# fogleman/sdf

Hardware: AMD Instinct MI355X
Metric: grid voxels/sec (sampled + meshed), canonical CSG example (higher is better)
Workload: dtype f64; 1 GPU; example @ samples=2**27 -> 512x512x512 grid, sparse=True, batch_size=32; batches=4096, skipped=2352, empty=120, nonempty=1624, triangles=2945152, parallelism=single GPU

## Files before the change

include/sdf_hip.h:

```cpp
#ifndef SDF_HIP_H
#define SDF_HIP_H

#include <stddef.h>
#include <stdint.h>

#ifdef __cplusplus
extern "C" {
#endif

#define SDF_ABI_VERSION 15

#define SDF_PRECISION_F64 0
#define SDF_PRECISION_F32 1

typedef struct sdf_ctx sdf_ctx;
typedef struct sdf_tape sdf_tape;
typedef struct sdf_mesh sdf_mesh;

typedef struct sdf_stats {
    int64_t n_batches;
    int64_t n_skipped;
    int64_t n_empty;
    int64_t n_nonempty;
    int64_t n_triangles;
    int64_t n_grid_voxels;
    int64_t n_eval_voxels;
    int64_t n_ambiguous_cells;
    int64_t n_work_begin;
    int64_t n_work_end;
    int64_t n_retries;
    double ms_prepass;
    double ms_mesh;
    double ms_emit;
    double ms_total;
    int64_t n_pruned_instrs;
    int64_t n_batch_instrs;
    int64_t n_sampled_voxels;
    double ms_mesh_device;
    double sclk_mhz;
    double t_mesh_first_us;
    double t_mesh_last_us;
    int64_t mesh_kernel;
} sdf_stats;

int sdf_abi_version(void);
const char *sdf_build_info(void);
const char *sdf_last_error(void);
int sdf_device_count(void);

int sdf_device_mem_info(int device, size_t *free_bytes, size_t *total_bytes);
int sdf_test_fail_alloc(int nth);

int sdf_ctx_create(int device, sdf_ctx **out);
int sdf_ctx_destroy(sdf_ctx *ctx);
int sdf_ctx_set_stream(sdf_ctx *ctx, void *hip_stream);
int sdf_ctx_set_prune(sdf_ctx *ctx, int enabled);
int sdf_ctx_set_cull(sdf_ctx *ctx, int enabled);
int sdf_ctx_set_twopass(sdf_ctx *ctx, int mode);
int sdf_ctx_set_defer(sdf_ctx *ctx, int on);
int sdf_ctx_set_cull_levels(sdf_ctx *ctx, int levels);
int sdf_ctx_set_tail_order(sdf_ctx *ctx, int on);
int sdf_ctx_synchronize(sdf_ctx *ctx);
int sdf_ctx_trim(sdf_ctx *ctx);

int sdf_tape_create(sdf_ctx *ctx, const uint32_t *code, uint32_t n_words, const double *consts,
                    uint32_t n_consts, uint32_t n_pslots, uint32_t n_dslots, sdf_tape **out);
int sdf_tape_set_prune_info(sdf_tape *tape, const uint16_t *rstart, const uint16_t *lstart, uint32_t n_instr);
int sdf_tape_destroy(sdf_tape *tape);

int sdf_eval_points(sdf_tape *tape, const void *d_points, int64_t n, int dim, void *d_out, int precision);
int sdf_eval_points_host(sdf_tape *tape, const double *h_points, int64_t n, int dim, double *h_out,
                         int precision);
int sdf_eval_grid_host(sdf_tape *tape, const double *X, int nx, const double *Y, int ny, const double *Z,
                       int nz, double *h_out, int precision);

int sdf_tape_extern_count(sdf_tape *tape);
int sdf_eval_extern_points_host(sdf_tape *tape, const double *h_points, int64_t n, int dim, double *h_ext_points,
                                int precision);
int sdf_eval_points_extern_host(sdf_tape *tape, const double *h_points, int64_t n, int dim, const double *h_ext_values,
                                double *h_out, int precision);
int sdf_mesh_level_set_host(sdf_ctx *ctx, const double *h_points, int64_t n_points, const int32_t *h_tris, int64_t n_tris,
                            double voxel_size, int half_width_voxels, int64_t out_ijk0[3], int64_t out_dims[3], float *h_out,
                            int64_t cap_voxels);
int sdf_distance_texture_host(sdf_ctx *ctx, const uint8_t *h_mask, int64_t rows, int64_t cols, double *h_out);
int sdf_render_host(sdf_tape *tape, const double *frame18, int width, int height, const double *params5, int max_steps, int refine,
                    double *h_depth, double *h_normal, int32_t *h_steps, uint8_t *h_status);
double sdf_render_last_kernel_ms(void);

typedef int (*sdf_field_fn)(void *user, const double *points, int64_t n, double *values);
int sdf_generate_field(sdf_ctx *ctx, sdf_field_fn field, void *user, const double *X, int nx, const double *Y, int ny,
                       const double *Z, int nz, int batch_size, int sparse, int64_t shard_index, int64_t shard_count,
                       sdf_mesh **out);

int sdf_estimate_bounds(sdf_tape *tape, double *h_out6, int precision);

int sdf_marching_cubes(sdf_ctx *ctx, const void *d_volume, int n0, int n1, int n2, void *d_out_tris,
                       int64_t cap_tris, int64_t *n_tris);
int sdf_marching_cubes_host(sdf_ctx *ctx, const float *h_volume, int n0, int n1, int n2, float *h_out_tris,
                            int64_t cap_tris, int64_t *n_tris);

int sdf_generate(sdf_tape *tape, const double *X, int nx, const double *Y, int ny, const double *Z, int nz,
                 int batch_size, int sparse, int64_t shard_index, int64_t shard_count, int precision,
                 sdf_mesh **out);
int sdf_generate_to_device(sdf_tape *tape, const double *X, int nx, const double *Y, int ny, const double *Z, int nz,
                           int batch_size, int sparse, int64_t shard_index, int64_t shard_count, int precision,
                           void *d_out, int64_t cap_tris, int *emitted, sdf_mesh **out);
int sdf_generate_to_device_async(sdf_tape *tape, const double *X, int nx, const double *Y, int ny, const double *Z, int nz,
                                 int batch_size, int sparse, int64_t shard_index, int64_t shard_count, int precision,
                                 void *d_out, int64_t cap_tris, sdf_mesh **out);
int sdf_mesh_wait(sdf_mesh *mesh, int *emitted);
int sdf_generate_records(sdf_tape *tape, const double *X, int nx, const double *Y, int ny, const double *Z, int nz,
                         int batch_size, int sparse, int precision, sdf_mesh **out);
size_t sdf_slab_bytes(int64_t cap_items, int64_t cap_tris);
int sdf_generate_compact_async(sdf_tape *tape, const double *X, int nx, const double *Y, int ny, const double *Z, int nz,
                               int batch_size, int sparse, int64_t shard_index, int64_t shard_count, int precision,
                               void *d_slab, int64_t cap_items, int64_t cap_tris, sdf_mesh **out);
int sdf_expand_slabs(sdf_ctx *ctx, const void *const *d_slabs, int n_slabs, int64_t cap_items, int64_t cap_tris,
                     void *d_out, int64_t cap_out_tris);
#define SDF_COMM_ID_BYTES 128
typedef struct sdf_comm sdf_comm;
typedef struct sdf_exchange sdf_exchange;
typedef struct sdf_exchange_stats {
    int64_t n_batches, n_skipped, n_empty, n_nonempty, n_triangles, n_grid_voxels, n_eval_voxels, n_ambiguous_cells,
        n_sampled_voxels, n_pruned_instrs;
    int64_t n_retries, chunks, world, slab_bytes;
    double ms_mesh, ms_exchange, ms_expand, ms_total;
    int64_t per_rank_triangles[64];
} sdf_exchange_stats;
int sdf_comm_available(void);
int sdf_comm_unique_id(void *out_id128);
int sdf_comm_create(sdf_ctx *ctx, const void *ids, int n_lanes, int rank, int world, sdf_comm **out);
int sdf_comm_destroy(sdf_comm *comm);
int sdf_generate_sharded_async(sdf_comm *comm, sdf_tape *tape, const double *X, int nx, const double *Y, int ny, const double *Z,
                               int nz, int batch_size, int sparse, int precision, int chunks, int lane, sdf_exchange **out);
int sdf_exchange_wait(sdf_exchange *x, void **d_soup, int64_t *n_tris);
int sdf_exchange_stats_get(sdf_exchange *x, sdf_exchange_stats *out);
int sdf_exchange_destroy(sdf_exchange *x);
int sdf_skip_kinds(sdf_tape *tape, const double *X, int nx, const double *Y, int ny, const double *Z, int nz, int batch_size,
                   int64_t b_begin, int64_t b_end, int precision, void *d_kinds);
int sdf_generate_from_kinds(sdf_tape *tape, const double *X, int nx, const double *Y, int ny, const double *Z, int nz,
                            int batch_size, int64_t shard_index, int64_t shard_count, int precision, const void *d_kinds,
                            sdf_mesh **out);
int sdf_memcpy_to_host(sdf_ctx *ctx, void *h_dst, const void *d_src, size_t bytes);
// ... 37 lines not shown
```

sdf_amd/csrc/sdf_device.h:

```cpp
#pragma once
#include <hip/hip_runtime.h>
#include <stdint.h>
#include <type_traits>

#include "sdf_interp.h"
#include "sdf_mc33.h"
#include "sdf_interval.h"
#include "sdf_slab.h"

namespace sdfk {

struct McTables {
    unsigned char ntri[256];
    unsigned char amb[256];
    signed char tri[256][16];
    signed char mc33[MC33_FLAT_SIZE];
};

struct MeshCounters {
    unsigned long long n_pruned;
    unsigned long long n_eval;
    unsigned int work_counter;
    unsigned int overflow;
    unsigned int n_empty, n_nonempty;
// ... 258 lines not shown
                                                           unsigned max_spins, unsigned long long first) {
    const int lane = threadIdx.x & 63;
    if (w == w_begin) return 0;
    unsigned long long acc = 0;
    int idx = w - 1;
    bool use_first = true;
    for (unsigned spins = 0; spins < max_spins;) {
        constexpr int NW = 4;
        unsigned long long sw[NW];
        const int nwin = use_first ? 1 : NW;
        if (use_first) sw[0] = first;
        else {
#pragma unroll
            for (int k = 0; k < NW; k++) {
                const int j = idx - 64 * k - lane;
                sw[k] = j >= w_begin ? __hip_atomic_load(&status[j], __ATOMIC_RELAXED, __HIP_MEMORY_SCOPE_AGENT)
                                     : MESH_FLAG_PFX;
            }
        }
        use_first = false;
        bool wait = false;
#pragma unroll
        for (int k = 0; k < NW; k++) {
            if (k >= nwin || wait) break;
            const unsigned flag = (unsigned)(sw[k] >> 62);
            const unsigned long long pending = __ballot(flag == 0), is_pfx = __ballot(flag == 2);
            if (is_pfx) {
                const int p = __ffsll((long long)is_pfx) - 1;
                if (pending & ((1ull << p) - 1ull)) { wait = true; break; }
                acc += lane <= p ? (sw[k] & MESH_VAL_MASK) : 0ull;
                const unsigned long long excl = wave_sum_u64(acc);
                if (lane == 0) __hip_atomic_store(&status[w], MESH_FLAG_PFX | (excl + total), __ATOMIC_RELAXED, __HIP_MEMORY_SCOPE_AGENT);
                return excl;
            }
            if (pending) { wait = true; break; }
            acc += sw[k] & MESH_VAL_MASK;
            idx -= 64;
        }
        if (wait) { __builtin_amdgcn_s_sleep(1); spins++; }
    }
    return max_spins < (1u << 24) ? MESH_NOT_READY : ~0ull;
}
#define MESH_SPIN_FOREVER (1u << 24)

__device__ __noinline__ void mc33_triangle(const float *corner, int s0, int s1, int i0, int i1, int i2,
                                           const signed char *tab, int j, float *o) {
    double lv[8];
    int off;
    mc33_load_cell(corner, s0, s1, lv);
    const int n = mc33_cell(lv, tab, &off);
    if (j >= n) { for (int q = 0; q < 9; q++) o[q] = 0.0f; return; }
    const signed char lew_edge[12] = {8, 5, 9, 4, 10, 7, 11, 6, 0, 1, 3, 2};
    for (int q = 0; q < 3; q++) {
        const int e = tab[off + 3 * j + 2 - q];
        if (e == 12) mc33_centre_vertex(lv, i0, i1, i2, o + 3 * q);
        else mc_vertex(corner, s0, s1, i0, i1, i2, lew_edge[e], o + 3 * q);
    }
}

struct TileTasks {
    int lx, ly, lz, lyz, nvox;
    float inv_lyz, inv_lz;
    bool regular;
    int ntask;
    __device__ __forceinline__ TileTasks(int lx_, int ly_, int lz_) : lx(lx_), ly(ly_), lz(lz_) {
        lyz = ly * lz; nvox = lx * lyz;
        inv_lyz = 1.0f / (float)lyz; inv_lz = 1.0f / (float)lz;
        regular = lx == 33 && ly == 33 && lz == 33;
        ntask = regular ? 563 : (nvox + 63) >> 6;
    }
    __device__ __forceinline__ bool sample(int task, int lane, int &ix, int &iy, int &iz) const {
        if (!regular) {
            const int i = min(task * 64 + lane, nvox - 1);
            ix = fast_div(i, inv_lyz); const int r = i - ix * lyz; iy = fast_div(r, inv_lz); iz = r - iy * lz;
            return task * 64 + lane < nvox;
        }
        if (task < 512) { ix = 4 * (task >> 6) + (lane >> 4); iy = 4 * ((task >> 3) & 7) + ((lane >> 2) & 3); iz = 4 * (task & 7) + (lane & 3); return true; }
        if (task < 530) { const int p = min((task - 512) * 64 + lane, 1088); ix = 32; iy = fast_div(p, 1.0f / 33.0f); iz = p - 33 * iy; return (task - 512) * 64 + lane < 1089; }
        if (task < 547) { const int p = min((task - 530) * 64 + lane, 1055); iy = 32; ix = fast_div(p, 1.0f / 33.0f); iz = p - 33 * ix; return (task - 530) * 64 + lane < 1056; }
        const int p = (task - 547) * 64 + lane; iz = 32; ix = p >> 5; iy = p & 31; return true;
    }
};

enum { CULL_UNIT_CAP = 3072, CULL_ULIST = 8, CULL_SBYTES = CULL_ULIST, CULL_SSTATE = CULL_ULIST + 2 * CULL_UNIT_CAP, CULL_COLINFO = CULL_SSTATE + 1024,
       CULL_RECORD = CULL_COLINFO + 1160,
       CULL_MSTATE = CULL_RECORD, CULL_GSTATE = CULL_MSTATE + 64, CULL_ELIST = CULL_GSTATE + 512, CULL_PACC = CULL_ELIST + 1024,
       CULL_SCRATCH = CULL_PACC + 64 };
static_assert(CULL_RECORD % 8 == 0 && CULL_SSTATE % 8 == 0 && CULL_COLINFO % 8 == 0, "the record is copied in words; its state rows are read as u64");
__device__ __forceinline__ bool cull_sample(const unsigned short *units, int task, int lane, int lx, int ly, int lz, int &ix, int &iy, int &iz) {
    const unsigned u = units[8 * task + (lane >> 3)];
    const int x = (int)((u >> 9) & 62u) + ((lane >> 2) & 1), y = (int)((u >> 4) & 62u) + ((lane >> 1) & 1), z = (int)((u << 1) & 62u) + (lane & 1);
    const bool ok = x < lx && y < ly && z < lz;
    ix = ok ? x : 0; iy = ok ? y : 0; iz = ok ? z : 0;
    return ok;
}
template <int BLOCK, bool FULL, bool RARE>
__device__ __forceinline__ int cull_tasks(const uint32_t *wcode, const double *consts, int n_instr_w, int lx, int ly, int lz,
                                       const double *axes, double *ia_state, int ia_bytes, unsigned char *scratch, int *wave_sums,
                                       int ia_np, int ia_nd, unsigned long long *prof = nullptr, int levels = 3) {
    const int tid = threadIdx.x;
    long long tprev = prof ? clock64() : 0;
    unsigned *pacc = reinterpret_cast<unsigned *>(scratch + CULL_PACC);
    if (prof && tid == 0) for (int k = 0; k < 12; k++) pacc[k] = 0;
#define SDF_CULL_PROF(K) do { if (prof && tid == 0) { const long long tn = clock64(); pacc[(K) - 16] += (unsigned)(tn - tprev); tprev = tn; } } while (0)
    const int c0 = lx - 1, c1 = ly - 1, c2 = lz - 1;
    const int per_pass = min(BLOCK, ia_bytes / ((6 * ia_np + 2 * ia_nd) * 8)) & ~63;
    if (c0 <= 0 || c1 <= 0 || c2 <= 0 || per_pass < 64) return -1;
    unsigned short *ulist = reinterpret_cast<unsigned short *>(scratch + CULL_ULIST);
    unsigned char *sstate = scratch + CULL_SBYTES;
    static_assert(2 * CULL_UNIT_CAP >= 4096, "the byte states lie over the unit list");
    unsigned char *mstate = scratch + CULL_MSTATE;
    unsigned char *gstate = scratch + CULL_GSTATE;
    unsigned short *elist = reinterpret_cast<unsigned short *>(scratch + CULL_ELIST);
    auto box_state = [&](int x0, int x1, int y0, int y1, int z0, int z1) -> unsigned char {
        Ival bx{axes[x0], axes[min(x1, c0)]}, by{axes[33 + y0], axes[33 + min(y1, c1)]}, bz{axes[66 + z0], axes[66 + min(z1, c2)]};
        if (bx.lo > bx.hi) { const double t = bx.lo; bx.lo = bx.hi; bx.hi = t; }
        if (by.lo > by.hi) { const double t = by.lo; by.lo = by.hi; by.hi = t; }
        if (bz.lo > bz.hi) { const double t = bz.lo; bz.lo = bz.hi; bz.hi = t; }
        if (ia::bad(bx) || ia::bad(by) || ia::bad(bz)) { bx = by = bz = ia::top(); }
        const Ival v = ia_run_tape<false, FULL, RARE>(wcode, consts, nullptr, nullptr, n_instr_w, bx, by, bz, true,
                                          IaShared{ia_state, ia_np, per_pass}, ia_nd, nullptr);
        return v.lo > 1e-30 ? 1 : (v.hi < -1e-30 ? 2 : 0);
    };
    int phase = 0, e0 = 0, nev = 0;
    for (;;) {
        if (phase == 1 && e0 >= nev) {
            __syncthreads();
            SDF_CULL_PROF(19);
            int nund = 0;
            for (int g0 = 0; levels >= 3 && g0 < 512; g0 += BLOCK) {
                const int gi = g0 + tid;
                const bool und = gi < 512 && gstate[gi] == 0;
                int n;
                const int pos = nund + block_exclusive_count<BLOCK>(und, wave_sums, n);
                if (und) elist[pos] = (unsigned short)gi;
                nund += n;
            }
            for (int h = tid; h < 4096; h += BLOCK) {
                const int h0 = h >> 8, h1 = (h >> 4) & 15, h2 = h & 15;
                const bool exists = 2 * h0 < c0 && 2 * h1 < c1 && 2 * h2 < c2;
                sstate[h] = exists ? gstate[((h0 >> 1) * 8 + (h1 >> 1)) * 8 + (h2 >> 1)] : 1;
            }
            __syncthreads();
            phase = 2; e0 = 0; nev = 8 * nund;
        }
        if (phase == 2 && e0 >= nev) break;
        const bool run = phase == 0 ? tid < 64 : (tid < per_pass && e0 + (tid & ~63) < nev);
        int target = 0, x0, y0, z0, ext;
        bool live;
        if (phase == 0) {
            const int m0 = tid >> 4, m1 = (tid >> 2) & 3, m2 = tid & 3;
            live = 8 * m0 < c0 && 8 * m1 < c1 && 8 * m2 < c2;
            x0 = live ? 8 * m0 : 0; y0 = live ? 8 * m1 : 0; z0 = live ? 8 * m2 : 0; ext = 8;
        } else if (phase == 1) {
            live = e0 + tid < nev;
            target = run ? (int)elist[min(e0 + tid, nev - 1)] : 0;
            x0 = 4 * (target >> 6); y0 = 4 * ((target >> 3) & 7); z0 = 4 * (target & 7); ext = 4;
        } else {
            const int e = min(e0 + tid, nev - 1);
            const int gq = run ? (int)elist[e >> 3] : 0, ch = e & 7;
            const int h0 = 2 * (gq >> 6) + (ch >> 2), h1 = 2 * ((gq >> 3) & 7) + ((ch >> 1) & 1), h2 = 2 * (gq & 7) + (ch & 1);
            live = e0 + tid < nev && 2 * h0 < c0 && 2 * h1 < c1 && 2 * h2 < c2;
            target = (h0 * 16 + h1) * 16 + h2;
            x0 = live ? 2 * h0 : 0; y0 = live ? 2 * h1 : 0; z0 = live ? 2 * h2 : 0; ext = 2;
        }
        if (run) {
            const unsigned char st = box_state(x0, x0 + ext, y0, y0 + ext, z0, z0 + ext);
            if (phase == 0) mstate[tid & 63] = live ? st : 1;
            else if (live) (phase == 1 ? gstate : sstate)[target] = st;
        }
        if (phase != 0) { if (prof && tid == 0) pacc[7]++; e0 += per_pass; continue; }
        SDF_CULL_PROF(17);
        __syncthreads();
        for (int g0 = 0; g0 < 512; g0 += BLOCK) {
            const int gi = g0 + tid;
            const int a0 = gi >> 6, a1 = (gi >> 3) & 7, a2 = gi & 7;
            const bool exists = gi < 512 && 4 * a0 < c0 && 4 * a1 < c1 && 4 * a2 < c2;
            const unsigned char ms = exists ? mstate[((a0 >> 1) * 4 + (a1 >> 1)) * 4 + (a2 >> 1)] : 1;
            if (gi < 512) gstate[gi] = ms;
            int n;
            const int pos = nev + block_exclusive_count<BLOCK>(ms == 0, wave_sums, n);
            if (ms == 0) elist[pos] = (unsigned short)gi;
            nev += n;
        }
        __syncthreads();
        SDF_CULL_PROF(18);
        if (prof && tid == 0) pacc[6] = (unsigned)nev;
        phase = 1; e0 = 0;
    }
    __syncthreads();
    SDF_CULL_PROF(20);
    unsigned short *ub = reinterpret_cast<unsigned short *>(scratch + CULL_GSTATE);
    for (int r = tid; r < 256; r += BLOCK) {
        const unsigned long long lo8 = *reinterpret_cast<const unsigned long long *>(sstate + 16 * r);
        const unsigned long long hi8 = *reinterpret_cast<const unsigned long long *>(sstate + 16 * r + 8);
        unsigned m = 0, pk = 0;
        SDF_UNROLL for (int k = 0; k < 8; k++) { m |= ((lo8 >> (8 * k)) & 255ull) == 0ull ? 1u << k : 0u; pk |= (unsigned)((lo8 >> (8 * k)) & 3ull) << (2 * k); }
        SDF_UNROLL for (int k = 0; k < 8; k++) { m |= ((hi8 >> (8 * k)) & 255ull) == 0ull ? 256u << k : 0u; pk |= (unsigned)((hi8 >> (8 * k)) & 3ull) << (2 * k + 16); }
        ub[r] = (unsigned short)m;
        reinterpret_cast<unsigned *>(scratch + CULL_SSTATE)[r] = pk;
    }
    __syncthreads();
    const int nu0 = (lx + 1) >> 1, nu1 = (ly + 1) >> 1, nu2 = (lz + 1) >> 1;
    int nlisted = 0;
    unsigned *colinfo = reinterpret_cast<unsigned *>(scratch + CULL_COLINFO);
    for (int q0 = 0; q0 < 17 * 17; q0 += BLOCK) {
        const int q = q0 + tid, u0 = q / 17, u1 = q - 17 * u0;
        unsigned um = 0;
        if (q < 17 * 17 && u0 < nu0 && u1 < nu1) {
            unsigned m = 0;
            for (int d0 = 0; d0 < 2; d0++)
                for (int d1 = 0; d1 < 2; d1++) {
                    const int h0 = u0 - d0, h1 = u1 - d1;
                    if (h0 >= 0 && h0 < 16 && h1 >= 0 && h1 < 16) m |= ub[h0 * 16 + h1];
                }
            um = (m | (m << 1)) & ((1u << nu2) - 1u);
        }
        int n;
        int pos = nlisted + block_exclusive_scan<BLOCK>(__popc(um), wave_sums, n);
        nlisted += n;
        if (q < 17 * 17) colinfo[q] = um | ((unsigned)min(pos, 32767) << 17);
        if (nlisted <= CULL_UNIT_CAP) {
            while (um) {
                const int u2 = __ffs((int)um) - 1;
                um &= um - 1u;
                ulist[pos++] = (unsigned short)((u0 << 10) | (u1 << 5) | u2);
            }
        }
    }
    SDF_CULL_PROF(24);
    if (nlisted > CULL_UNIT_CAP) { __syncthreads(); return -1; }
    if (tid < 8 && nlisted + tid < ((nlisted + 7) & ~7)) ulist[nlisted + tid] = 0xFFFFu;
    if (tid == 0) reinterpret_cast<unsigned short *>(scratch)[0] = (unsigned short)nlisted;
    __syncthreads();
    SDF_CULL_PROF(25);
#undef SDF_CULL_PROF
    return (nlisted + 7) >> 3;
}

#ifndef SDF_SOUP_NT
#define SDF_SOUP_NT 0
#endif
#if SDF_SOUP_NT
#define SDF_SOUP_STORE(PTR, VAL) __builtin_nontemporal_store((VAL), (PTR))
#else
#define SDF_SOUP_STORE(PTR, VAL) (*(PTR) = (VAL))
#endif

enum { MESH_SLOT_HDR = 1232, MESH_SLOT_COLINFO = 64, MESH_STAGE_BYTES = 32 * 9 * 4 };

template <typename T, bool FULL, int NP, int ND, int NS, int BLOCK, bool TWOPASS = false>
__global__ __launch_bounds__(BLOCK) void k_mesh(const uint32_t *__restrict__ code, const T *__restrict__ consts, MeshArgs a_byval) {
    typedef __attribute__((address_space(4))) const MeshArgs KArgs;
    static_assert(sizeof(const uint32_t *) + sizeof(const T *) == 16 && alignof(MeshArgs) <= 16, "MeshArgs sits at byte 16 of the kernel arguments");
    KArgs *ap = (KArgs *)((__attribute__((address_space(4))) const char *)__builtin_amdgcn_kernarg_segment_ptr() + 16);
    (void)a_byval;
#define KA (*ap)
#define SDF_SINK (Tri16Sink{KA.out, KA.raw, KA.raw_cap, &KA.ctr->n_raw})
    typedef Vec<T, NS> V;
    constexpr int RPT = 1024 / BLOCK;
    constexpr int MESH_CELL_CHUNKS = 2;
    extern __shared__ __attribute__((aligned(16))) unsigned char smem[];
    int *wave_sums = reinterpret_cast<int *>(smem);
    int *bcast = wave_sums + 16;
    unsigned char *ntri_lds = smem + MESH_LDS_NTRI;
    double *axes = reinterpret_cast<double *>(smem + MESH_LDS_AXES);
    float *vol = reinterpret_cast<float *>(smem + MESH_LDS_VOL);
    unsigned long long *bits = reinterpret_cast<unsigned long long *>(smem + KA.bits_off);
    unsigned *wlist = reinterpret_cast<unsigned *>(smem + KA.list_off);
    int tid = threadIdx.x;
#define SDF_FRESH() asm volatile("" : "+v"(tid))
    const GridDesc g = a_byval.g;
    unsigned short *tri_lds = reinterpret_cast<unsigned short *>(smem + MESH_LDS_TRI);

    if (tid < 256) ntri_lds[tid] = (unsigned char)(KA.mc->ntri[tid] | (KA.mc->amb[tid] << 7));
    if (!TWOPASS)
        for (int i = tid; i < 256 * 5; i += BLOCK) {
            const int cfg = i / 5, j = i - 5 * cfg;
            const signed char *t3 = &KA.mc->tri[cfg][3 * j];
            tri_lds[i] = (unsigned short)(((unsigned)t3[0] & 15u) | (((unsigned)t3[1] & 15u) << 4) | (((unsigned)t3[2] & 15u) << 8));
        }

    for (int i = tid; i < (int)((KA.list_off - KA.bits_off) >> 3); i += BLOCK) bits[i] = 0ull;
    const int work_begin = KA.ctr->work_begin, work_end = KA.ctr->work_end;
    if (KA.prof && tid == 0) KA.prof[64 + 4 * blockIdx.x] = wall_clock64();
// ... 683 lines not shown
```

sdf_amd/csrc/sdf_hip.hip:

```cpp
#include <hip/hip_runtime.h>

#include <algorithm>
#include <cmath>
#include <cstdio>
#include <cstdlib>
#include <cstring>

#include "mc_table.h"
#include "sdf_prune.h"
#include "sdf_plain.h"
#include "sdf_bounds.h"
#include "sdf_internal.h"

using namespace sdfk;


template <typename T, bool FULL>
__global__ __launch_bounds__(256) void k_eval_points(const uint32_t *__restrict__ code, const T *__restrict__ consts,
                                                     const double *__restrict__ pts, long long n, int dim,
                                                     double *__restrict__ out) {
    const long long i = (long long)blockIdx.x * blockDim.x + threadIdx.x;
    if (i >= n) return;
    const T x = (T)pts[i * dim], y = (T)pts[i * dim + 1], z = dim > 2 ? (T)pts[i * dim + 2] : T(0);
    out[i] = (double)run_tape1<T, FULL>(code, consts, x, y, z);
// ... 22 lines not shown
    const int iz = (int)(i % tl.n2), iy = (int)((i / tl.n2) % tl.n1), ix = (int)(i / ((long long)tl.n2 * tl.n1));
    const int *o = org + 3 * blockIdx.y;
    vol[tl.vol_off + i] = (float)run_tape1<T, FULL>(code, consts, (T)X[o[0] + ix], (T)Y[o[1] + iy], (T)Z[o[2] + iz]);
}

template <typename T, bool FULL>
__global__ __launch_bounds__(256) void k_eval_points_ext(const uint32_t *__restrict__ code, const T *__restrict__ consts,
                                                         const double *__restrict__ pts, long long n, int dim,
                                                         double *__restrict__ ext, int dump, double *__restrict__ out) {
    const long long i = (long long)blockIdx.x * blockDim.x + threadIdx.x;
    if (i >= n) return;
    const T x = (T)pts[i * dim], y = (T)pts[i * dim + 1], z = dim > 2 ? (T)pts[i * dim + 2] : T(0);
    const T v = run_tape1_ext<T, FULL>(code, consts, x, y, z, ExtIO{ext, n, i, dump != 0});
    if (!dump) out[i] = (double)v;
}


enum { SKIP_BATCHES_PER_BLOCK = 7 * (256 / 64) };
template <typename T, bool FULL, bool RARE>
__device__ __forceinline__ void skip_body(const uint32_t *__restrict__ code, const T *__restrict__ consts, GridDesc g,
                                              int nbatches, unsigned char *__restrict__ kinds, const PruneArgs &pa,
                                              const double *__restrict__ c64, const uint16_t *__restrict__ rstart,
                                              const uint16_t *__restrict__ lstart, double *prune_lds, int skip_b0) {
    if ((int)blockIdx.x >= pa.first_block) {
        prune_block<FULL, RARE>(code, c64, rstart, lstart, pa, g, nbatches, (int)blockIdx.x - pa.first_block, prune_lds);
        return;
    }
    const int lane = threadIdx.x & 63, slot = min(lane / 9, 6), l = lane - 9 * slot;
    const int b = skip_b0 + ((int)blockIdx.x * (256 / 64) + (int)(threadIdx.x >> 6)) * 7 + slot;
    const bool live = b < nbatches && l < 9;
    int ox = 0, oy = 0, oz = 0, lx = 1, ly = 1, lz = 1;
    if (b < nbatches) batch_origin(g, b, ox, oy, oz, lx, ly, lz);
    double x0 = 0, x1 = 0, y0 = 0, y1 = 0, z0 = 0, z1 = 0;
    if (b < nbatches) {
        x0 = g.X[ox]; x1 = g.X[ox + lx - 1]; y0 = g.Y[oy]; y1 = g.Y[oy + ly - 1]; z0 = g.Z[oz]; z1 = g.Z[oz + lz - 1];
    }
    const double cx = (x0 + x1) / 2, cy = (y0 + y1) / 2, cz = (z0 + z1) / 2;
    double px = cx, py = cy, pz = cz;
    if (l >= 1) { const int k = l - 1; px = (k & 4) ? x1 : x0; py = (k & 2) ? y1 : y0; pz = (k & 1) ? z1 : z0; }
    T v = T(0);
    if (live) v = run_tape1<T, FULL>(code, consts, (T)px, (T)py, (T)pz);
    const int base = 9 * slot;
    const T vc = __shfl(v, base, 64);
    const T v1 = __shfl(v, base + 1, 64);
    const bool pos = v1 > T(0);
    const bool ok = pos ? (v > T(0)) : (v < T(0));
    const unsigned long long m = __ballot(ok);
    const bool all_same = ((m >> (base + 1)) & 0xFFull) == 0xFFull;
    if (b < nbatches && l == 0) {
        const double r = fabs((double)vc);
        const double d = sqrt(((cx - x0) * (cx - x0) + (cy - y0) * (cy - y0)) + (cz - z0) * (cz - z0));
        const bool skip = !(r <= d) && all_same;
        kinds[b] = skip ? 0 : 255;
    }
}

template <typename T, bool FULL>
__global__ __launch_bounds__(256) void k_skip(const uint32_t *__restrict__ code, const T *__restrict__ consts, GridDesc g,
                                              int nbatches, unsigned char *__restrict__ kinds, PruneArgs pa,
                                              const double *__restrict__ c64, const uint16_t *__restrict__ rstart, const uint16_t *__restrict__ lstart,
                                              int skip_b0) {
    extern __shared__ double prune_lds[];
    skip_body<T, FULL, false>(code, consts, g, nbatches, kinds, pa, c64, rstart, lstart, prune_lds, skip_b0);
}
template <typename T, bool FULL>
__global__ __launch_bounds__(256) void k_skip_rare(const uint32_t *__restrict__ code, const T *__restrict__ consts, GridDesc g,
                                                   int nbatches, unsigned char *__restrict__ kinds, PruneArgs pa,
                                                   const double *__restrict__ c64, const uint16_t *__restrict__ rstart, const uint16_t *__restrict__ lstart,
                                                   int skip_b0) {
    extern __shared__ double prune_lds[];
    skip_body<T, FULL, true>(code, consts, g, nbatches, kinds, pa, c64, rstart, lstart, prune_lds, skip_b0);
}

template <bool FULL, bool RARE>
__global__ __launch_bounds__(PRUNE_BLOCK) void k_prune_list(const uint32_t *__restrict__ code, GridDesc g, int nbatches, PruneArgs pa,
                                                               const double *__restrict__ c64, const uint16_t *__restrict__ rstart,
                                                               const uint16_t *__restrict__ lstart) {
    extern __shared__ double prune_list_lds[];
    if ((long long)blockIdx.x * (PRUNE_BLOCK / 8) >= (long long)(pa.ctr->work_end - pa.ctr->work_begin)) return;
    prune_block<FULL, RARE>(code, c64, rstart, lstart, pa, g, nbatches, (int)blockIdx.x, prune_list_lds);
}

#define CULL_BLOCK 256
template <bool FULL, bool RARE, int CB = CULL_BLOCK>
__device__ __forceinline__ void cull_body(const uint32_t *__restrict__ code, const double *__restrict__ consts, GridDesc g,
                                                     const int *__restrict__ worklist, const MeshCounters *__restrict__ ctr,
                                                     int tape_stride, int n_instr, int ia_np, int ia_nd, int ia_bytes,
                                                     unsigned char *__restrict__ out, unsigned char *cull_smem, unsigned long long *prof,
                                                     int *__restrict__ order, int tail_max, int levels) {
    int *wave_sums = reinterpret_cast<int *>(cull_smem);
    double *axes = reinterpret_cast<double *>(cull_smem + 64);
    unsigned char *scratch = cull_smem + 896;
    double *ia_state = reinterpret_cast<double *>(cull_smem + 896 + CULL_SCRATCH);
    const int tid = threadIdx.x;
    const long long tstart = prof ? clock64() : 0;
    asm volatile("" :: "s"(g.X), "s"(g.Y), "s"(g.Z), "s"(g.nx), "s"(g.ny), "s"(g.nz), "s"(g.nby), "s"(g.nbz), "s"(g.bs));
    const int w = ctr->work_begin + (int)blockIdx.x;
    if (w >= ctr->work_end) return;
    long long t_ctr = 0, t_b = 0;
    if (prof) asm volatile("s_memtime %0\n\ts_waitcnt lgkmcnt(0)" : "=s"(t_ctr) : "s"(w) : "memory");
    const int b = __builtin_amdgcn_readfirstlane(worklist[w]);
    if (prof) asm volatile("s_memtime %0\n\ts_waitcnt lgkmcnt(0)" : "=s"(t_b) : "s"(b) : "memory");
    int ox, oy, oz, lx, ly, lz;
    batch_origin(g, b, ox, oy, oz, lx, ly, lz);
    long long t_org = 0;
    if (prof) asm volatile("s_memtime %0\n\ts_waitcnt lgkmcnt(0)" : "=s"(t_org) : "s"(ox), "s"(oy), "s"(oz), "s"(lx) : "memory");
    for (int i = tid; i < 99; i += CB) {
        const int ax = i < 33 ? 0 : (i < 66 ? 1 : 2), k = i - 33 * ax;
        const double *src = ax == 0 ? g.X + ox : (ax == 1 ? g.Y + oy : g.Z + oz);
        if (k < (ax == 0 ? lx : (ax == 1 ? ly : lz))) axes[i] = src[k];
    }
    long long t_ax = 0, t_bar = 0;
    if (prof) asm volatile("s_waitcnt vmcnt(0) lgkmcnt(0)\n\ts_memtime %0\n\ts_waitcnt lgkmcnt(0)" : "=s"(t_ax) : "s"(b) : "memory");
    __syncthreads();
    if (prof) asm volatile("s_memtime %0\n\ts_waitcnt lgkmcnt(0)" : "=s"(t_bar) : "s"(b) : "memory");
    const uint32_t *wcode = code + (size_t)b * (size_t)tape_stride * 2;
    const int n_instr_w = tape_stride ? (int)reinterpret_cast<const unsigned long long *>(wcode)[tape_stride - 1] : n_instr;
    long long tstart1 = 0;
    if (prof) asm volatile("s_waitcnt vmcnt(0) lgkmcnt(0)\n\ts_memtime %0\n\ts_waitcnt lgkmcnt(0)" : "=s"(tstart1) : "s"(n_instr_w) : "memory");
    const int ntl = cull_tasks<CB, FULL, RARE>(wcode, consts, n_instr_w, lx, ly, lz, axes, ia_state, ia_bytes, scratch, wave_sums, ia_np, ia_nd, prof, levels);
    const long long tw = prof ? clock64() : 0;
    if (tid == 0 && ntl < 0) reinterpret_cast<unsigned short *>(scratch)[0] = (unsigned short)0xFFFF;
    __syncthreads();
    {
        unsigned *rec = reinterpret_cast<unsigned *>(out + (size_t)w * CULL_RECORD);
        const unsigned *src = reinterpret_cast<const unsigned *>(scratch);
        const int nwords = ntl < 0 ? 1 : (CULL_ULIST + 16 * ntl + 3) >> 2;
        for (int i = tid; i < nwords; i += CB) rec[i] = src[i];
        if (ntl >= 0) for (int i = tid; i < (CULL_RECORD - CULL_SSTATE) / 4; i += CB) rec[CULL_SSTATE / 4 + i] = src[CULL_SSTATE / 4 + i];
    }
    if (order && tid == 0) {
        const int tail = min(tail_max, ctr->work_end - ctr->work_begin), tpos = w - (ctr->work_end - tail);
        if (tpos >= 0) order[tpos] = (ntl < 0 ? 563 : ntl) * max(n_instr_w, 1);
    }
    if (prof && tid == 0) {
        const unsigned *pacc = reinterpret_cast<const unsigned *>(scratch + CULL_PACC);
        atomicAdd(&prof[32 + (ntl < 0 ? 9 : min(ntl >> 6, 8))], 1ull);
        atomicAdd(&prof[16], (unsigned long long)(tstart1 - tstart));
        atomicAdd(&prof[26], (unsigned long long)(t_ctr - tstart));
        atomicAdd(&prof[27], (unsigned long long)(t_b - t_ctr));
        atomicAdd(&prof[28], (unsigned long long)(t_ax - t_org));
        atomicAdd(&prof[30], (unsigned long long)(t_org - t_b));
        atomicAdd(&prof[29], (unsigned long long)(t_bar - t_ax));
        atomicAdd(&prof[21], (unsigned long long)(clock64() - tw));
        for (int k = 1; k < 10; k++) if (k != 5) atomicAdd(&prof[16 + k], (unsigned long long)pacc[k]);
    }
}

template <bool FULL, bool RARE, int CB = CULL_BLOCK>
__global__ __launch_bounds__(CB) void k_cull(const uint32_t *__restrict__ code, const double *__restrict__ consts, GridDesc g,
                                                     const int *__restrict__ worklist, const MeshCounters *__restrict__ ctr,
                                                     int tape_stride, int n_instr, int ia_np, int ia_nd, int ia_bytes,
                                                     unsigned char *__restrict__ out, unsigned long long *prof,
                                                     int *__restrict__ order, int tail_max, int levels) {
    extern __shared__ __attribute__((aligned(16))) unsigned char cull_smem[];
    cull_body<FULL, RARE, CB>(code, consts, g, worklist, ctr, tape_stride, n_instr, ia_np, ia_nd, ia_bytes, out, cull_smem, prof, order, tail_max, levels);
}
__global__ __launch_bounds__(CULL_BLOCK) __attribute__((amdgpu_waves_per_eu(6, 8))) void k_cull_lean(const uint32_t *__restrict__ code, const double *__restrict__ consts, GridDesc g,
                                                     const int *__restrict__ worklist, const MeshCounters *__restrict__ ctr,
                                                     int tape_stride, int n_instr, int ia_np, int ia_nd, int ia_bytes,
                                                     unsigned char *__restrict__ out, unsigned long long *prof,
                                                     int *__restrict__ order, int tail_max, int levels) {
    extern __shared__ __attribute__((aligned(16))) unsigned char cull_smem[];
    cull_body<false, false>(code, consts, g, worklist, ctr, tape_stride, n_instr, ia_np, ia_nd, ia_bytes, out, cull_smem, prof, order, tail_max, levels);
}
__global__ __launch_bounds__(128) __attribute__((amdgpu_waves_per_eu(6, 8))) void k_cull_lean128(const uint32_t *__restrict__ code, const double *__restrict__ consts, GridDesc g,
                                                     const int *__restrict__ worklist, const MeshCounters *__restrict__ ctr,
                                                     int tape_stride, int n_instr, int ia_np, int ia_nd, int ia_bytes,
                                                     unsigned char *__restrict__ out, unsigned long long *prof,
                                                     int *__restrict__ order, int tail_max, int levels) {
    extern __shared__ __attribute__((aligned(16))) unsigned char cull_smem[];
    cull_body<false, false, 128>(code, consts, g, worklist, ctr, tape_stride, n_instr, ia_np, ia_nd, ia_bytes, out, cull_smem, prof, order, tail_max, levels);
}



static bool tape_needs_full(const uint32_t *code, uint32_t n_words, const double *consts) {
    auto trig_ease = [](int id) {
        return id == EASE_in_sine || id == EASE_out_sine || id == EASE_in_out_sine || id == EASE_in_expo ||
               id == EASE_out_expo || id == EASE_in_out_expo || id == EASE_in_elastic || id == EASE_out_elastic ||
               id == EASE_in_out_elastic;
    };
    for (uint32_t i = 0; i + 1 < n_words; i += 2) {
        const uint32_t op = code[i] & 255u;
        const double *c = consts + (code[i + 1] & 0xFFFFFFu) + 1;
        switch (op) {
        case OP_TWIST: case OP_BEND: case OP_BEND_RADIAL: case OP_WRAP_AROUND: case OP_CIRC_PREP: case OP_CIRC_SET:
        case OP_TRANS_RAD_PRE:
            return true;
        case OP_BEND_LINEAR: if (trig_ease((int)c[10])) return true; break;
        case OP_TRANS_LIN_PRE: if (trig_ease((int)c[7])) return true; break;
        case OP_EXTTO_PRE: if (trig_ease((int)c[1])) return true; break;
        default: break;
        }
    }
    return false;
}

static int validate_tape(const uint32_t *code, uint32_t n_words, uint32_t n_consts, uint32_t n_p, uint32_t n_d) {
    if (n_words < 2 || (n_words & 1)) return fail("tape: code must be a non-empty list of 2-word instructions");
    if (n_p > SDF_NP_SLOTS || n_d > SDF_ND_SLOTS) return fail("tape: model needs more register slots than this build provides");
    if ((code[n_words - 2] & 255u) != OP_END) return fail("tape: missing END");
    for (uint32_t i = 0; i < n_words; i += 2) {
        const uint32_t w0 = code[i], w1 = code[i + 1], op = w0 & 255u, post = (w0 >> 8) & 7u, sa = w0 >> 24, sb = w1 >> 24;
        if (op >= OP_COUNT) return fail("tape: unknown opcode");
        if (post > POST_BLEND) return fail("tape: unknown post-combine");
        if (w0 & 0x800000u) return fail("tape: reserved bit set");
        if ((w0 & 0x000800u) && ((w0 >> 12) & 7u) >= std::max(n_p, 1u)) return fail("tape: reload slot out of range");
        if ((w0 & 0x008000u) && ((w0 >> 16) & 7u) >= std::max(n_p, 1u)) return fail("tape: save slot out of range");
        if ((w0 & 0x080000u) && ((w0 >> 20) & 7u) >= std::max(n_d, 1u)) return fail("tape: push slot out of range");
        if (sa >= SDF_NP_SLOTS || sb >= SDF_NP_SLOTS) return fail("tape: slot out of range");
        if ((w1 & 0xFFFFFFu) >= n_consts) return fail("tape: constant offset out of range");
        if (op == OP_END && i != n_words - 2) return fail("tape: END before the last instruction");
    }
    return 0;
}

static int ctx_init(sdf_ctx *c);

extern "C" {

int sdf_abi_version(void) { return SDF_ABI_VERSION; }

#ifndef SDF_BUILD_INFO
#define SDF_BUILD_INFO "unknown toolchain (not built by csrc/build.sh)"
#endif
const char *sdf_build_info(void) { return SDF_BUILD_INFO; }

int sdf_device_count(void) {
    int n = 0;
    hipError_t e = hipGetDeviceCount(&n);
    if (e != hipSuccess) { g_err = std::string("hipGetDeviceCount: ") + hipGetErrorString(e); return 0; }
    return n;
}


int sdf_device_mem_info(int device, size_t *free_bytes, size_t *total_bytes) {
    if (!free_bytes || !total_bytes) return fail("sdf_device_mem_info: NULL argument");
    HIPCHK(set_device(device));
    HIPCHK(hipMemGetInfo(free_bytes, total_bytes));
    return 0;
}

int sdf_ctx_create(int device, sdf_ctx **out) {
    if (!out) return fail("sdf_ctx_create: out is NULL");
    int n = 0;
    HIPCHK(hipGetDeviceCount(&n));
    if (device < 0 || device >= n) return fail("sdf_ctx_create: no such device");
    HIPCHK(set_device(device));
    hipDeviceProp_t prop;
    HIPCHK(hipGetDeviceProperties(&prop, device));
    if (std::string(prop.gcnArchName).rfind("gfx950", 0) != 0)
        return fail(std::string("sdf_ctx_create: this library is built for gfx950 only, device is ") + prop.gcnArchName);
    sdf_ctx *c = new sdf_ctx();
    c->device = device;
    c->n_cu = prop.multiProcessorCount;
    c->lds_max = prop.sharedMemPerBlock;
    if (ctx_init(c)) {
        const std::string keep = g_err;
        sdf_ctx_destroy(c);
        g_err = keep;
        return 1;
    }
    *out = c;
    return 0;
}

static int ctx_init(sdf_ctx *c) {
    HIPCHK(hipStreamCreateWithFlags(&c->own_stream, hipStreamNonBlocking));
    c->stream = c->own_stream;
    for (auto &e : c->ev) HIPCHK(hipEventCreate(&e));
    HIPCHK(host_malloc(&c->h_stage, (size_t)SDF_CALL_SLOTS * SDF_STAGE_BYTES + 4096));
    for (auto &cs : c->slots) {
        HIPCHK(hipEventCreate(&cs.e0)); HIPCHK(hipEventCreate(&cs.e2)); HIPCHK(hipEventCreate(&cs.e3)); HIPCHK(hipEventCreate(&cs.e4));
        HIPCHK(hipEventCreateWithFlags(&cs.done, hipEventDisableTiming));
        HIPCHK(hipStreamCreateWithFlags(&cs.stream, hipStreamNonBlocking));
    }
    if (const char *e = getenv("SDF_SLOT_STREAMS")) c->slot_streams = atoi(e);
    if (const char *e = getenv("SDF_CULL_BLOCK")) c->cull_block = atoi(e);
    if (const char *e = getenv("SDF_TAIL_ORDER")) c->tail_order = atoi(e);
    if (const char *e = getenv("SDF_MESH_TWOPASS")) c->twopass = atoi(e);
    McTables t;
    memcpy(t.ntri, MC_NTRI, 256);
    memcpy(t.amb, MC_AMBIGUOUS, 256);
    memcpy(t.tri, MC_TRI, sizeof(t.tri));
    memcpy(t.mc33, MC33_FLAT, sizeof(t.mc33));
    if (c->mc.ensure(sizeof(t))) return 1;
    HIPCHK(hipMemcpy(c->mc.p, &t, sizeof(t), hipMemcpyHostToDevice));
    if (const char *e = getenv("SDF_BOUNDS_TAG0")) c->bounds_tag0 = (unsigned)atoi(e) & 0xFFFFu;
    if (const char *e = getenv("SDF_MESH_SLOTS")) c->mesh_slots = atoi(e);
    if (const char *e = getenv("SDF_PRUNE")) c->prune = atoi(e);
    if (const char *e = getenv("SDF_PARK")) c->parking = atoi(e);
    if (const char *e = getenv("SDF_PRUNE_LIST_MIN")) c->prune_list_min = std::max(atoi(e), 0);
    if (const char *e = getenv("SDF_CULL")) c->cull = atoi(e);
    if (const char *e = getenv("SDF_DEFER")) c->defer = atoi(e) ? 1 : 0;
    if (const char *e = getenv("SDF_CULL_LEVELS")) c->cull_levels = atoi(e);
    if (const char *e = getenv("SDF_PARK_SPINS")) c->park_spins = std::max(atoi(e), 1);
    if (const char *e = getenv("SDF_MESH_PROF")) { if (atoi(e) && c->prof.ensure(512 + 4096 * 32)) return 1; }
    return 0;
}

int sdf_ctx_destroy(sdf_ctx *c) {
    if (!c) return 0;
    (void)hipSetDevice(c->device);
    (void)stream_wait(c->stream);
    for (auto &cs : c->slots) { if (cs.stream) (void)stream_wait(cs.stream); cs.park.release(); }
    for (DevBuf *b : {&c->scratch_in, &c->scratch_out, &c->rows, &c->rows_off, &c->mc, &c->prof, &c->park, &c->ext, &c->field_vals,
                      &c->field_vol, &c->field_tiles, &c->bounds_work})
        b->release();
    for (auto &b : c->arena_pool) b.release();
    for (auto &b : c->counter_pool) b.release();
    g_pool.drop_device(c->device);
    for (auto &e : c->ev) if (e) (void)hipEventDestroy(e);
    for (auto &cs : c->slots) for (hipEvent_t e : {cs.e0, cs.e2, cs.e3, cs.e4, cs.done}) if (e) (void)hipEventDestroy(e);
    for (auto &cs : c->slots) if (cs.stream) (void)hipStreamDestroy(cs.stream);
    if (c->h_stage) (void)hipHostFree(c->h_stage);
    if (c->h_rec) (void)hipHostFree(c->h_rec);
    for (hipEvent_t e : c->rec_ev) if (e) (void)hipEventDestroy(e);
    if (c->own_stream) (void)hipStreamDestroy(c->own_stream);
    delete c;
    return 0;
}

int sdf_ctx_set_stream(sdf_ctx *c, void *s) {
    if (!c) return fail("sdf_ctx_set_stream: ctx is NULL");
    c->stream = s ? (hipStream_t)s : c->own_stream;
    return 0;
}

int sdf_ctx_set_prune(sdf_ctx *c, int enabled) {
    if (!c) return fail("sdf_ctx_set_prune: ctx is NULL");
    c->prune = enabled ? 1 : 0;
    return 0;
}

int sdf_ctx_set_cull(sdf_ctx *c, int enabled) {
    if (!c) return fail("sdf_ctx_set_cull: ctx is NULL");
    c->cull = enabled ? 1 : 0;
    return 0;
}

int sdf_ctx_set_defer(sdf_ctx *c, int on) {
    if (!c) return fail("sdf_ctx_set_defer: ctx is NULL");
    c->defer = on ? 1 : 0;
    return 0;
}
int sdf_ctx_set_cull_levels(sdf_ctx *c, int levels) {
    if (!c) return fail("sdf_ctx_set_cull_levels: ctx is NULL");
    if (levels != 0 && levels != 2 && levels != 3) return fail("sdf_ctx_set_cull_levels: 0 (the library's choice), 2 or 3");
    c->cull_levels = levels;
    return 0;
}

int sdf_ctx_set_tail_order(sdf_ctx *c, int on) {
    if (!c) return fail("sdf_ctx_set_tail_order: ctx is NULL");
    c->tail_order = on ? 1 : 0;
    return 0;
}
int sdf_ctx_set_twopass(sdf_ctx *c, int mode) {
    if (!c) return fail("sdf_ctx_set_twopass: ctx is NULL");
    c->twopass = mode < 0 ? -1 : (mode ? 1 : 0);
    return 0;
}

int sdf_ctx_trim(sdf_ctx *c) {
    if (!c) return fail("sdf_ctx_trim: ctx is NULL");
    HIPCHK(set_device(c->device));
    HIPCHK(stream_wait(c->stream));
    for (auto &cs : c->slots) if (cs.stream) HIPCHK(stream_wait(cs.stream));
    for (auto &b : c->arena_pool) b.release();
    c->arena_pool.clear();
    g_pool.drop_device(c->device);
    return 0;
}

int sdf_ctx_synchronize(sdf_ctx *c) {
    if (!c) return fail("sdf_ctx_synchronize: ctx is NULL");
    HIPCHK(set_device(c->device));
    HIPCHK(stream_wait(c->stream));
    for (auto &cs : c->slots) if (cs.stream) HIPCHK(stream_wait(cs.stream));
    return 0;
}

int sdf_tape_create(sdf_ctx *c, const uint32_t *code, uint32_t n_words, const double *consts, uint32_t n_consts,
                    uint32_t n_p, uint32_t n_d, sdf_tape **out) {
    if (!c || !code || !consts || !out) return fail("sdf_tape_create: NULL argument");
    if (validate_tape(code, n_words, n_consts, n_p, n_d)) return 1;
    HIPCHK(set_device(c->device));
    sdf_tape *t = new sdf_tape();
    struct Guard { sdf_tape *t; ~Guard() { if (t) { const std::string keep = g_err; sdf_tape_destroy(t); g_err = keep; } } } guard{t};
    t->ctx = c; t->n_words = n_words; t->n_consts = n_consts;
    t->full = tape_needs_full(code, n_words, consts);
    {
        unsigned long long h = 1469598103934665603ull;
        auto mix = [&](const void *p, size_t n) { const unsigned char *b = (const unsigned char *)p; for (size_t i = 0; i < n; i++) { h ^= b[i]; h *= 1099511628211ull; } };
        mix(code, (size_t)n_words * 4); mix(consts, (size_t)n_consts * 8); mix(&n_p, 4); mix(&n_d, 4);
        t->content_hash = h;
    }
    t->ia_complete = true;
    for (uint32_t i = 0; i < n_words; i += 2) {
        t->ia_complete = t->ia_complete && ia_has_form(code[i] & 255u);
        t->ia_rare = t->ia_rare || ia_is_rare_leaf(code[i] & 255u);
        if ((code[i] & 255u) == OP_L_EXTERN) {
            if ((code[i + 1] & 0xFFFFFFu) + 1 >= n_consts) return fail("tape: closure index out of the constant pool");
            const double k = consts[(code[i + 1] & 0xFFFFFFu) + 1];
            if (!(k >= 0.0 && k < 65536.0 && k == (double)(uint32_t)k)) return fail("tape: bad closure index");
            t->n_extern = std::max(t->n_extern, (uint32_t)k + 1u);
        }
    }
    t->n_p = n_p; t->n_d = n_d;
    std::vector<double> c64(consts, consts + n_consts);
    c64.push_back(0.0); c64.push_back(0.0);
    std::vector<float> c32(c64.size());
    for (size_t i = 0; i < c64.size(); i++) c32[i] = (float)c64[i];
    std::vector<uint32_t> pcode(code, code + n_words);
    pcode.push_back(code[n_words - 2]); pcode.push_back(code[n_words - 1]);
    HIPCHK(dev_malloc((void **)&t->d_code, pcode.size() * sizeof(uint32_t)));
    HIPCHK(dev_malloc((void **)&t->d_c64, c64.size() * sizeof(double)));
    HIPCHK(dev_malloc((void **)&t->d_c32, c32.size() * sizeof(float)));
    HIPCHK(hipMemcpy(t->d_code, pcode.data(), pcode.size() * sizeof(uint32_t), hipMemcpyHostToDevice));
    HIPCHK(hipMemcpy(t->d_c64, c64.data(), c64.size() * sizeof(double), hipMemcpyHostToDevice));
    HIPCHK(hipMemcpy(t->d_c32, c32.data(), c32.size() * sizeof(float), hipMemcpyHostToDevice));
    guard.t = nullptr;
    *out = t;
    return 0;
}

int sdf_tape_set_prune_info(sdf_tape *t, const uint16_t *rstart, const uint16_t *lstart, uint32_t n_instr) {
    if (!t || !rstart || !lstart) return fail("sdf_tape_set_prune_info: NULL argument");
    if (n_instr * 2 != t->n_words) return fail("sdf_tape_set_prune_info: one entry per instruction expected");
    for (uint32_t i = 0; i < n_instr; i++) {
        const bool none = rstart[i] == 0xFFFF || lstart[i] == 0xFFFF;
        if (!none && !(lstart[i] <= rstart[i] && rstart[i] <= i)) return fail("sdf_tape_set_prune_info: operand range out of order");
// ... 338 lines not shown
    return 0;
}

static int stage_axes(const GenCall &call, char *stage, double *dX, hipStream_t st) {
    const double *X = call.X, *Y = call.Y, *Z = call.Z;
    const int nx = call.nx, ny = call.ny, nz = call.nz;
    double *dY = dX + nx, *dZ = dY + ny;
    const size_t axis_bytes = (size_t)(nx + ny + nz) * 8;
    if (call.collected && axis_bytes > SDF_STAGE_BYTES - 256) return fail("sdf_generate_to_device_async: axes too long for the staging slot");
    if (axis_bytes <= SDF_STAGE_BYTES - 256) {
        double *hs = (double *)stage;
        memcpy(hs, X, (size_t)nx * 8); memcpy(hs + nx, Y, (size_t)ny * 8); memcpy(hs + nx + ny, Z, (size_t)nz * 8);
        HIPCHK(hipMemcpyAsync(dX, hs, axis_bytes, hipMemcpyHostToDevice, st));
    } else {
        HIPCHK(hipMemcpyAsync(dX, X, (size_t)nx * 8, hipMemcpyHostToDevice, st));
        HIPCHK(hipMemcpyAsync(dY, Y, (size_t)ny * 8, hipMemcpyHostToDevice, st));
        HIPCHK(hipMemcpyAsync(dZ, Z, (size_t)nz * 8, hipMemcpyHostToDevice, st));
    }
    return 0;
}

static int enqueue_prepass(const GenCall &call, sdf_mesh *m, int nb, int tape_stride, hipStream_t st) {
    sdf_tape *t = call.tape;
    sdf_ctx *c = t->ctx;
    const GridDesc &g = m->g;
    const int sparse = call.sparse, precision = call.precision;
    const bool pruning = tape_stride != 0;
    const uint32_t n_instr = t->n_words / 2;
    PruneArgs pa = {};
    pa.first_block = 0x7fffffff;
    const bool prune_listed = pruning && sparse && (nb >= c->prune_list_min || call.shard_count > 1);
    unsigned skip_blocks = (sparse && !call.d_kinds) ? (unsigned)((nb + SKIP_BATCHES_PER_BLOCK - 1) / SKIP_BATCHES_PER_BLOCK) : 0u, prune_blocks = 0;
    size_t prune_lds = 0;
    if (pruning) {
        if (m->prune.ensure((size_t)nb * 64) || m->tapes.ensure((size_t)nb * tape_stride * 8)) return 1;
        pa.n_instr = (int)n_instr; pa.n_p = std::max(t->n_p, 1u); pa.n_d = std::max(t->n_d, 1u);
        pa.masks_out = (uint32_t *)m->prune.p; pa.tapes_out = (unsigned long long *)m->tapes.p; pa.tape_stride = tape_stride;
        pa.zero_off = t->n_consts;
        prune_lds = prune_lds_bytes(pa.n_p, pa.n_d);
        if (!prune_listed) {
            pa.first_block = (int)skip_blocks;
            prune_blocks = (unsigned)(((long long)nb * 8 + PRUNE_BLOCK - 1) / PRUNE_BLOCK);
        }
    }
    if (skip_blocks + prune_blocks) {
        if (prune_lds > 32768 && prune_blocks) {
            const void *fn = t->ia_rare ? (t->full ? reinterpret_cast<const void *>(k_skip_rare<double, true>) : reinterpret_cast<const void *>(k_skip_rare<double, false>))
                                        : (t->full ? reinterpret_cast<const void *>(k_skip<double, true>) : reinterpret_cast<const void *>(k_skip<double, false>));
            HIPCHK(hipFuncSetAttribute(fn, hipFuncAttributeMaxDynamicSharedMemorySize, (int)prune_lds));
        }
        const size_t skip_lds = prune_blocks ? prune_lds : 0;
        if (t->ia_rare) LAUNCH_TAPE_ON(st, k_skip_rare, dim3(skip_blocks + prune_blocks), dim3(256), skip_lds, t, precision, g, nb, (unsigned char *)m->kinds.p, pa,
                                       (const double *)t->d_c64, (const uint16_t *)t->d_rstart, (const uint16_t *)t->d_lstart, 0);
        else LAUNCH_TAPE_ON(st, k_skip, dim3(skip_blocks + prune_blocks), dim3(256), skip_lds, t, precision, g, nb, (unsigned char *)m->kinds.p, pa,
                            (const double *)t->d_c64, (const uint16_t *)t->d_rstart, (const uint16_t *)t->d_lstart, 0);
    }
    if (!sparse) HIPCHK(hipMemsetAsync(m->kinds.p, 255, (size_t)nb, st));
    else if (call.d_kinds) HIPCHK(hipMemcpyAsync(m->kinds.p, call.d_kinds, (size_t)nb, hipMemcpyDeviceToDevice, st));
    launch_k_compact(dim3(1), dim3(1024), st, (const unsigned char *)m->kinds.p, nb, (int *)m->worklist.p,
                       (MeshCounters *)m->counters.p, (unsigned long long *)m->status.p, (long long)call.shard_index,
                       (long long)call.shard_count);
    HIPCHK(hipGetLastError());
    if (prune_listed) {
        pa.worklist = (const int *)m->worklist.p; pa.ctr = (const MeshCounters *)m->counters.p;
        auto kp = t->full ? (t->ia_rare ? k_prune_list<true, true> : k_prune_list<true, false>) : (t->ia_rare ? k_prune_list<false, true> : k_prune_list<false, false>);
        if (prune_lds > 32768) HIPCHK(hipFuncSetAttribute(reinterpret_cast<const void *>(kp), hipFuncAttributeMaxDynamicSharedMemorySize, (int)prune_lds));
        hipLaunchKernelGGL(kp, dim3((unsigned)(((long long)nb * 8 + PRUNE_BLOCK - 1) / PRUNE_BLOCK)), dim3(PRUNE_BLOCK), prune_lds, st,
                           (const uint32_t *)t->d_code, g, nb, pa, (const double *)t->d_c64, (const uint16_t *)t->d_rstart,
                           (const uint16_t *)t->d_lstart);
        HIPCHK(hipGetLastError());
    }
    return 0;
}

static int enqueue_cull(sdf_tape *t, sdf_mesh *m, int nb, int tape_stride, bool tail_order, int tail_max, hipStream_t st) {
    sdf_ctx *c = t->ctx;
    const GridDesc &g = m->g;
    const bool pruning = tape_stride != 0;
    const uint32_t n_instr = t->n_words / 2;
    if (c->prof.p) HIPCHK(hipMemsetAsync((unsigned char *)c->prof.p + 128, 0, 384, st));
    if (m->cull.ensure((size_t)nb * CULL_RECORD) || (tail_order && m->order.ensure(MESH_TAIL_MAX * sizeof(int)))) return 1;
    const int ia_np = (int)std::max(t->n_p, 1u), ia_nd = (int)std::max(t->n_d, 1u);
    auto kc = t->full ? (t->ia_rare ? k_cull<true, true> : k_cull<true, false>) : (t->ia_rare ? k_cull<false, true> : k_cull_lean);
    int cull_block = CULL_BLOCK;
    if (c->cull_block == 128 && kc == k_cull_lean) { kc = k_cull_lean128; cull_block = 128; }
    if (t->full && !t->ia_rare && c->cull_block != 256) {
        cull_block = c->cull_block == 64 ? 64 : 128;
        kc = cull_block == 64 ? k_cull<true, false, 64> : k_cull<true, false, 128>;
    }
    const int cull_levels = c->cull_levels ? c->cull_levels : (kc == k_cull_lean || kc == k_cull_lean128 ? 3 : 2);
    const size_t ia_bytes = std::min<size_t>((size_t)cull_block * (6 * ia_np + 2 * ia_nd) * 8, c->lds_max - 896 - CULL_SCRATCH);
    const size_t lds = 896 + CULL_SCRATCH + ia_bytes;
    if (lds > 32768) HIPCHK(hipFuncSetAttribute(reinterpret_cast<const void *>(kc), hipFuncAttributeMaxDynamicSharedMemorySize, (int)lds));
    hipLaunchKernelGGL(kc, dim3(nb), dim3(cull_block), lds, st,
                       pruning ? (const uint32_t *)m->tapes.p : (const uint32_t *)t->d_code, (const double *)t->d_c64, g,
                       (const int *)m->worklist.p, (const MeshCounters *)m->counters.p, pruning ? tape_stride : 0, (int)n_instr,
                       ia_np, ia_nd, (int)ia_bytes, (unsigned char *)m->cull.p, (unsigned long long *)c->prof.p,
                       tail_order ? (int *)m->order.p : (int *)nullptr, tail_max, cull_levels);
    HIPCHK(hipGetLastError());
    return 0;
}

static int first_soup_cap(sdf_tape *t, sdf_mesh *m, unsigned long long key, hipStream_t st, unsigned long long &cap, bool &quiet) {
    if (t->hint_key == key && t->hint_total_tris) {
        cap = t->hint_total_tris + t->hint_total_tris / 4 + 4096;
        return 0;
    }
    MeshCounters h;
    quiet = false;
    HIPCHK(hipMemcpyAsync(&h, m->counters.p, sizeof(h), hipMemcpyDeviceToHost, st));
    HIPCHK(stream_wait(st));
    const unsigned long long nshard0 = (unsigned long long)std::max(h.work_end - h.work_begin, 1);
    cap = std::max<unsigned long long>(4096ull * nshard0, 1ull << 16);
    size_t free_b = 0, total_b = 0;
    if (hipMemGetInfo(&free_b, &total_b) == hipSuccess)
        cap = std::min<unsigned long long>(cap, std::max<unsigned long long>(free_b / 2 / (72 + 40), 1ull << 16));
    return 0;
}

static int soup_target(const GenCall &call, sdf_mesh *m, int attempt, unsigned long long cap, bool &quiet, MeshArgs &a) {
    sdf_ctx *c = m->ctx;
    a.compact = 0; a.xf = nullptr; a.xf_cap = 0; a.raw = nullptr; a.raw_cap = 0;
    if (cap) {
        if (!m->out.p && !c->arena_pool.empty()) { m->out = c->arena_pool.back(); c->arena_pool.pop_back(); }
        if (m->out.bytes < (size_t)cap * 72) quiet = false;
        if (m->out.ensure((size_t)cap * 72)) {
            bool ok = false;
            for (int k = 0; k < 6 && !ok && attempt == 0 && cap > (1ull << 16); k++) {
                cap = std::max<unsigned long long>(cap / 4, 1ull << 16);
                ok = m->out.ensure((size_t)cap * 72) == 0;
            }
            if (!ok) return 1;
        }
        a.out = (double *)m->out.p; a.out_cap = m->out.bytes / 72;
    } else if (call.dest == GenCall::SLAB) {
        unsigned char *d_slab = (unsigned char *)call.d_out;
        const SlabLayout L(call.cap_items, call.cap_tris);
        a.out = reinterpret_cast<double *>(d_slab + L.tris_off); a.out_cap = (unsigned long long)call.cap_tris;
        a.compact = 1; a.xf = reinterpret_cast<double *>(d_slab + L.xf_off);
        a.raw = reinterpret_cast<float *>(d_slab + L.raw_off); a.raw_cap = L.raw_cap;
        a.xf_cap = (int)std::min<int64_t>(call.cap_items, 0x7fffffff);
    } else {
        a.out = (double *)call.d_out; a.out_cap = (unsigned long long)call.cap_tris;
    }
    return 0;
}

static int mesh_attempt(const GenCall &call, sdf_mesh *m, CallState &s, hipStream_t st, int attempt, unsigned long long soup_cap, bool quiet,
                        bool culling, int tail, int tape_stride) {
    sdf_tape *t = call.tape;
    sdf_ctx *c = t->ctx;
    CallSlot &cs = c->slots[s.slot];
    const int nb = s.nb;
    const uint32_t n_instr = s.n_instr;
    MeshArgs a;
    a.twopass = 0; a.desc = nullptr; a.cells = nullptr; a.tlist = nullptr; a.cells_cap = a.tlist_cap = 0; a.block_item = nullptr;
    a.order = tail ? (const int *)m->order.p : nullptr; a.tail = tail;
    if (soup_target(call, m, attempt, soup_cap, quiet, a)) return 1;
    if (attempt) {
        HIPCHK(hipMemsetAsync(m->counters.p, 0, MESH_COUNTERS_RESET_BYTES, st));
        HIPCHK(hipMemsetAsync(m->status.p, 0, (size_t)nb * 8, st));
    }
    a.g = m->g; a.worklist = (const int *)m->worklist.p;
    a.kinds = (unsigned char *)m->kinds.p; a.status = (unsigned long long *)m->status.p;
    a.ctr = (MeshCounters *)m->counters.p;
    a.mc = (const McTables *)c->mc.p;
    a.prof = (unsigned long long *)c->prof.p;
    const bool twopass = c->twopass >= 0 ? c->twopass != 0 : n_instr > 96;
    DevBuf &park = call.collected ? cs.park : c->park;
    const bool parks = c->parking && !twopass;
    if (parks && !park.p) { quiet = false; if (park.ensure((size_t)c->n_cu * MESH_PARK_DEPTH * SDF_PARK_TRIS * 36)) return 1; }
    a.park = parks ? (float *)park.p : nullptr; a.park_cap = a.park ? SDF_PARK_TRIS : 0;
    a.park_spins = (unsigned)c->park_spins;
    a.cull = culling ? (const unsigned char *)m->cull.p : nullptr;
    a.tape_stride = tape_stride;
    a.n_instr = (int)n_instr;
    if (twopass) {
        const size_t cap_t = (size_t)a.out_cap;
        if (m->desc.bytes < (size_t)nb * sizeof(ItemDesc) || m->cellrecs.bytes < cap_t * 36 || m->trilist.bytes < cap_t * 4) quiet = false;
        if (m->desc.ensure((size_t)nb * sizeof(ItemDesc)) || m->cellrecs.ensure(cap_t * 36) || m->trilist.ensure(cap_t * 4) ||
            m->blockidx.ensure(((cap_t + 255) / 256 + 2) * sizeof(int)))
            return 1;
        a.twopass = 1; a.desc = (ItemDesc *)m->desc.p; a.cells = (unsigned *)m->cellrecs.p; a.tlist = (unsigned *)m->trilist.p;
        a.block_item = (const int *)m->blockidx.p;
        a.cells_cap = a.tlist_cap = (unsigned long long)cap_t;
    }
    if (a.prof) {
        HIPCHK(hipMemsetAsync(a.prof, 0, 128, st));
        HIPCHK(hipMemsetAsync((unsigned char *)a.prof + 512, 0, 4096 * 32, st));
    }
    const int grid = std::min(nb, c->n_cu);
    s.own_start = attempt > 0 || a.prof || !quiet;
    if (s.own_start) HIPCHK(hipEventRecord(cs.e3, st));
    if (launch_mesh(t, tape_stride ? m->tapes.p : (const void *)t->d_code, call.precision, a, grid, call.bs, st)) return 1;
    if (a.twopass) {
        const unsigned long long emit_blocks = (a.out_cap + 255ull) / 256ull;
        if (emit_blocks > 0x7fffffffull) return fail("sdf_generate: soup capacity too large for one k_emit2 launch");
        launch_k_scan_items(dim3(1), dim3(1024), st, (const ItemDesc *)m->desc.p, (MeshCounters *)m->counters.p,
                           (unsigned long long *)m->status.p, (int *)m->blockidx.p, emit_blocks + 1ull);
        launch_k_emit2(dim3((unsigned)std::max<unsigned long long>(emit_blocks, 1ull)), dim3(256), st, a);
        HIPCHK(hipGetLastError());
    }
    HIPCHK(hipEventRecord(cs.e4, st));
    if (call.dest == GenCall::SLAB) {
        const unsigned pack_blocks = (unsigned)std::min<int64_t>(std::max<int64_t>((call.cap_items + 255) / 256, 1), 1024);
        HIPCHK((hipError_t)sdf_launch_pack_slab(pack_blocks, st, (const MeshCounters *)m->counters.p, (const unsigned long long *)m->status.p,
                                                (unsigned char *)call.d_out, (long long)call.cap_items, (long long)call.cap_tris));
    }
    MeshCounters *hp = (MeshCounters *)((char *)c->h_stage + (size_t)s.slot * SDF_STAGE_BYTES + SDF_STAGE_BYTES - 256);
    HIPCHK(hipMemcpyAsync(hp, m->counters.p, sizeof(MeshCounters), hipMemcpyDeviceToHost, st));
    return 0;
}

static int mesh_prof_report(sdf_ctx *c, int grid, float ms) {
    unsigned long long pc[64];
    HIPCHK(hipMemcpy(pc, c->prof.p, 512, hipMemcpyDeviceToHost));
    {
        std::vector<unsigned long long> tl((size_t)4 * grid);
        HIPCHK(hipMemcpy(tl.data(), (unsigned char *)c->prof.p + 512, tl.size() * 8, hipMemcpyDeviceToHost));
        unsigned long long t0 = ~0ull, t_end = 0;
        double s_out = 0, s_done = 0, mn_out = 1e30, mx_out = 0;
        for (int i = 0; i < grid; i++) t0 = std::min(t0, tl[4 * i]);
        for (int i = 0; i < grid; i++) {
            const double o = (double)(tl[4 * i + 1] - t0) * 0.01, d = (double)(tl[4 * i + 2] - t0) * 0.01;
            s_out += o; s_done += d; mn_out = std::min(mn_out, o); mx_out = std::max(mx_out, o); t_end = std::max(t_end, tl[4 * i + 2]);
        }
        double first_hi = 0;
        for (int i = 0; i < grid; i++) first_hi = std::max(first_hi, (double)(tl[4 * i] - t0) * 0.01);
        fprintf(stderr, "[k_mesh prof] %d workgroups (1 per CU), last of them started after %.1f us; out of work after min %.1f avg %.1f max %.1f us; done after avg %.1f, last %.1f us\n",
                grid, first_hi, mn_out, s_out / grid, mx_out, s_done / grid, (double)(t_end - t0) * 0.01);
    }
    fprintf(stderr, "[k_cull prof] work items by listed tasks (of 563; bins of 64, last: not culled): %llu %llu %llu %llu %llu %llu %llu %llu %llu | %llu\n",
            pc[32], pc[33], pc[34], pc[35], pc[36], pc[37], pc[38], pc[39], pc[40], pc[41]);
    fprintf(stderr, "[k_cull prof] cycles of thread 0, summed over the workgroups: start %llu boxes %llu list %llu groups %llu (%llu passes, %llu groups) tasks %llu record %llu\n",
            pc[16], pc[17], pc[18], pc[19], pc[23], pc[22], pc[20], pc[21]);
    fprintf(stderr, "[k_cull prof] task listing: which tasks %llu, scans %llu; start: range %llu batch %llu origin %llu axes %llu barrier %llu (rest: tape length)\n", pc[24], pc[25], pc[26], pc[27], pc[30], pc[28], pc[29]);
    fprintf(stderr, "[k_mesh prof] sampling: intervals %llu task list %llu interpreter %llu sign bits %llu\n", pc[8], pc[9], pc[10], pc[11]);
    fprintf(stderr, "[k_mesh prof] fine: atomic %llu barrier+rank %llu header %llu | rows %llu cells %llu | placing %llu look-back %llu | round end %llu\n",
            pc[42], pc[43], pc[44], pc[45], pc[46], pc[47], pc[48], pc[49]);
    fprintf(stderr, "[k_mesh prof] %.3f ms; cycles/WG-sum: grab %llu sample %llu count %llu (of which placing the parked batch %llu) list %llu emit %llu tail %llu; %llu batches parked, %llu written one batch later from their slot\n",
            ms, pc[0], pc[1], pc[2], pc[6], pc[3], pc[4], pc[5], pc[7], pc[12]);
    return 0;
}

int generate_impl(sdf_mesh *m, const GenCall &call) {
    sdf_tape *t = call.tape;
    sdf_ctx *c = t->ctx;
    const bool slab = call.dest == GenCall::SLAB;
    const int nx = call.nx, ny = call.ny, nz = call.nz;
    CallState s;
    if (take_slot(c, s.slot)) return 1;
    CallSlot &cs = c->slots[s.slot];
    const bool own_lane = call.collected && !slab && c->stream == c->own_stream && c->slot_streams;
    hipStream_t st = call.lane ? call.lane : (own_lane ? cs.stream : c->stream);
    m->stream = (own_lane || call.lane) ? st : nullptr;
    if (grid_batches(nx, ny, nz, call.bs, "sdf_generate", m->g, s.nb)) return 1;
    const int nb = s.nb;
    m->st.n_batches = nb;
    m->st.n_grid_voxels = (int64_t)nx * ny * nz;
    if (nb == 0) {
        if (slab) HIPCHK(hipMemsetAsync(call.d_out, 0, sizeof(SlabHeader), st));
        return 0;
    }

    if (m->axes.ensure((size_t)(nx + ny + nz) * 8) || m->kinds.ensure((size_t)nb) || m->worklist.ensure((size_t)nb * 4) ||
        m->status.ensure((size_t)nb * 8))
        return 1;
    if (!m->counters.p && !c->counter_pool.empty()) { m->counters = c->counter_pool.back(); c->counter_pool.pop_back(); }
    if (m->counters.ensure(sizeof(MeshCounters))) return 1;
    double *dX = (double *)m->axes.p;
    m->g.X = dX; m->g.Y = dX + nx; m->g.Z = dX + nx + ny;
    HIPCHK(hipEventRecord(cs.e0, st));
    if (stage_axes(call, (char *)c->h_stage + (size_t)s.slot * SDF_STAGE_BYTES, dX, st)) return 1;

    auto monotone = [](const double *a, int n) {
        bool up = true, down = true;
        for (int i = 1; i < n; i++) { up &= a[i - 1] <= a[i]; down &= a[i - 1] >= a[i]; }
        return up || down;
    };
    s.n_instr = t->n_words / 2;
    const bool intervals_ok = call.precision == SDF_PRECISION_F64 && monotone(call.X, nx) && monotone(call.Y, ny) && monotone(call.Z, nz);
    s.pruning = c->prune && t->d_rstart && s.n_instr <= 256 && intervals_ok && t->n_consts < 0xFFFFF0u;
    const int tape_stride = s.pruning ? (int)((s.n_instr + 2 + 7) & ~7u) : 0;
    if (enqueue_prepass(call, m, nb, tape_stride, st)) return 1;
    const bool culling = c->cull && intervals_ok && t->ia_complete && mesh_lds(call.bs, c->lds_max).list_off + CULL_RECORD <= c->lds_max;
    const int tail_max = std::min<int>(MESH_TAIL_MAX, std::min(nb, c->n_cu) - 1);
    const bool tail_order = culling && c->tail_order && tail_max >= 2 && !call.collected;
    s.key = grid_key(nx, ny, nz, call.bs, call.sparse, call.shard_index, call.shard_count);
    if (culling && enqueue_cull(t, m, nb, tape_stride, tail_order, tail_max, st)) return 1;
    HIPCHK(hipEventRecord(cs.e2, st));

    unsigned long long soup_cap = 0;
    bool quiet = true;
    if (call.dest == GenCall::SOUP && first_soup_cap(t, m, s.key, st, soup_cap, quiet)) return 1;
    for (int attempt = 0;; attempt++) {
        if (mesh_attempt(call, m, s, st, attempt, soup_cap, quiet, culling, tail_order ? tail_max : 0, tape_stride)) return 1;
        if (call.collected) {
            HIPCHK(hipEventRecord(cs.done, st));
            cs.busy = true; cs.owner = m;
            sdf_mesh::Pending &pd = m->pend;
            pd.active = true; pd.call = call; pd.got = s;
            pd.axes.assign(call.X, call.X + nx); pd.axes.insert(pd.axes.end(), call.Y, call.Y + ny); pd.axes.insert(pd.axes.end(), call.Z, call.Z + nz);
            pd.call.X = pd.axes.data(); pd.call.Y = pd.call.X + nx; pd.call.Z = pd.call.Y + ny;
            return 0;
        }
        HIPCHK(stream_wait(st));
        MeshCounters h;
        const int rc = finish_call(m, call, s, slab, h);
        if (c->prof.p && mesh_prof_report(c, std::min(nb, c->n_cu), m->st.ms_mesh)) return 1;
        m->st.n_retries = attempt;
        if (rc) return 1;
        if (slab) {
            const SlabLayout L(call.cap_items, call.cap_tris);
            const bool raw_over = (long long)h.n_raw > L.raw_cap;
            m->n_raw = (long long)h.n_raw;
            m->rec_overflow = (h.overflow & 1u) != 0 || raw_over || (long long)(h.work_end - h.work_begin) > (long long)call.cap_items;
            m->rec_need_tris = std::max<long long>((long long)h.total, raw_over ? (long long)h.n_raw * SLAB_RAW_DIV : 0ll);
            m->emitted_to = nullptr;
            return 0;
// ... 378 lines not shown
```

sdf_amd/csrc/sdf_internal.h:

```cpp
#pragma once
#include <cstdint>
#include <map>

#include "../../include/sdf_hip.h"
#include "sdf_device.h"
#include "sdf_runtime.h"

using sdfk::DevBuf;
using sdfk::GridDesc;

#define SDF_STAGE_BYTES (1u << 20)
#ifndef SDF_CALL_SLOTS
#define SDF_CALL_SLOTS 8
#endif
struct CallSlot {
    hipEvent_t e0 = nullptr, e2 = nullptr, e3 = nullptr, e4 = nullptr;
    hipEvent_t done = nullptr;
    bool busy = false;
    struct sdf_mesh *owner = nullptr;
    hipStream_t stream = nullptr;
    DevBuf park;
};
#define SDF_BATCH_SIZE_MAX 512
#define SDF_PARK_TRIS 8192

struct sdf_ctx {
    int device = 0;
    hipStream_t own_stream = nullptr, stream = nullptr;
    hipEvent_t ev[8] = {};
    int n_cu = 256;
    size_t lds_max = 0;
    DevBuf scratch_in, scratch_out, rows, rows_off, mc;
    DevBuf ext;
    DevBuf field_vals, field_vol, field_tiles;
    DevBuf prof;
    int prune = 1;
    int parking = 1;
    int cull = 1;
    int prune_list_min = 8192;
    int park_spins = 1;
    DevBuf park;
    int mesh_slots = -1;
    std::vector<DevBuf> arena_pool;
    std::vector<DevBuf> counter_pool;
    void *h_stage = nullptr;
    CallSlot slots[SDF_CALL_SLOTS];
    unsigned slot_seq = 0;
    int slot_streams = 1;
    int cull_block = 0;
    int tail_order = 1;
    int twopass = -1;
    int defer = 1;
    int cull_levels = 0;
    DevBuf bounds_work;
    unsigned bounds_tag = 0, bounds_tag0 = 0;
    struct RecHint { unsigned long long tris = 0, raw = 0; };
    std::map<std::pair<unsigned long long, unsigned long long>, RecHint> rec_hints;
    void *h_rec = nullptr;
    size_t h_rec_bytes = 0;
    std::vector<hipEvent_t> rec_ev;
};

struct sdf_tape {
    sdf_ctx *ctx = nullptr;
    uint32_t *d_code = nullptr;
    double *d_c64 = nullptr;
    float *d_c32 = nullptr;
    uint32_t n_words = 0, n_consts = 0;
    bool full = false;
    uint32_t n_p = 0, n_d = 0;
    uint16_t *d_rstart = nullptr, *d_lstart = nullptr;
    bool ia_complete = false;
    bool ia_rare = false;
    uint32_t n_extern = 0;
    unsigned long long hint_key = 0, hint_total_tris = 0;
    unsigned long long content_hash = 0;
};

struct GenCall {
    sdf_tape *tape = nullptr;
    const double *X = nullptr, *Y = nullptr, *Z = nullptr;
    int nx = 0, ny = 0, nz = 0, bs = 0, sparse = 0, precision = 0;
    int64_t shard_index = 0, shard_count = 1;
    enum Dest { SOUP, CALLER, SLAB } dest = SOUP;
    void *d_out = nullptr;
    int64_t cap_tris = 0, cap_items = 0;
    bool collected = false;
    hipStream_t lane = nullptr;
    const unsigned char *d_kinds = nullptr;
};
struct CallState { int slot = 0, nb = 0; bool pruning = false, own_start = false; uint32_t n_instr = 0; unsigned long long key = 0; };

struct sdf_mesh {
    sdf_ctx *ctx = nullptr;
    sdf_stats st = {};
    GridDesc g = {};
    DevBuf axes, kinds, worklist, status, out, prune, tapes, cull, order;
    DevBuf desc, cellrecs, trilist;
    DevBuf blockidx;
    bool pruned = false;
    hipStream_t stream = nullptr;
    DevBuf counters;
    int work_begin = 0, work_end = 0;
    void *emitted_to = nullptr;
    struct Pending {
        bool active = false;
        GenCall call;
        std::vector<double> axes;
        CallState got;
    } pend;
    double *weld_pts = nullptr;
    long long *weld_inv = nullptr;
    long long weld_n = -1;
    double *nrm = nullptr;
    bool nrm_valid = false;
    unsigned long long nrm_model = 0;
    double nrm_eps = 0.0;
    long long nrm_flat = 0;
    bool records = false;
    DevBuf slab;
    long long slab_items = 0, slab_tris = 0, n_raw = 0;
    bool rec_overflow = false;
    long long rec_need_tris = 0;
};

inline long long grid_desc(int nx, int ny, int nz, int bs, GridDesc &g) {
    g = GridDesc{};
    g.nx = nx; g.ny = ny; g.nz = nz; g.bs = bs;
    if (bs < 1) return 0;
    g.nbx = (nx + bs - 1) / bs; g.nby = (ny + bs - 1) / bs; g.nbz = (nz + bs - 1) / bs;
    return (long long)g.nbx * g.nby * g.nbz;
}

inline GenCall gen_call(sdf_tape *t, const double *X, int nx, const double *Y, int ny, const double *Z, int nz, int bs, int sparse,
                        int64_t shard_index, int64_t shard_count, int precision) {
// ... 16 lines not shown
```

sdf_amd/csrc/sdf_interval.h:

```cpp
#pragma once
#include <hip/hip_runtime.h>
#include <stdint.h>

#include "opcodes.h"

#define SDF_IA __host__ __device__ __forceinline__

namespace sdfk {

#if defined(__HIP_DEVICE_COMPILE__)
__device__ __forceinline__ void ia_sincos(double x, double *s, double *c) { sincos64(x, *s, *c); }
__device__ __forceinline__ double ia_atan2(double y, double x) { return atan2_64(y, x); }
#else
inline void ia_sincos(double x, double *s, double *c) { *s = sin(x); *c = cos(x); }
inline double ia_atan2(double y, double x) { return atan2(y, x); }
#endif

struct Ival {
    double lo, hi;
};

namespace ia {

SDF_IA Ival top() { return Ival{-__builtin_inf(), __builtin_inf()}; }
// ... 100 lines not shown
    d = a = top();
    if (!finite_(x) || !finite_(y) || !(da > 0.0) || !(da < 7.0)) return;
    d = pad(len2(x, y), 1e-12, 1e-300);
    if (bad(d)) { d = top(); return; }
    d.lo = fmax(d.lo, 0.0);
    a = Ival{0.0, da};
    if (x.lo <= 0.0 && y.lo <= 0.0 && y.hi >= 0.0) return;
    const double t0 = ia_atan2(y.lo, x.lo), t1 = ia_atan2(y.lo, x.hi), t2 = ia_atan2(y.hi, x.lo), t3 = ia_atan2(y.hi, x.hi);
    const double tl = fmin(fmin(t0, t1), fmin(t2, t3)) - 1e-12, th = fmax(fmax(t0, t1), fmax(t2, t3)) + 1e-12;
    if (!(tl <= th)) return;
    const double kl = floor(tl / da), kh = floor(th / da);
    if (kl != kh) return;
    const double lo = tl - kl * da, hi = th - kl * da;
    if (!(lo > 1e-9) || !(da - hi > 1e-9)) return;
    a = Ival{lo - 1e-12, hi + 1e-12};
}
SDF_IA Ival atan2_range(const Ival &x, const Ival &y) {
    const double pi = 3.141592653589793;
    if (!finite_(x) || !finite_(y)) return top();
    if (x.lo <= 0.0 && y.lo <= 0.0 && y.hi >= 0.0) return Ival{-pi, pi};
    const double t0 = ia_atan2(y.lo, x.lo), t1 = ia_atan2(y.lo, x.hi), t2 = ia_atan2(y.hi, x.lo), t3 = ia_atan2(y.hi, x.hi);
    const double tl = fmin(fmin(t0, t1), fmin(t2, t3)) - 1e-12, th = fmax(fmax(t0, t1), fmax(t2, t3)) + 1e-12;
    if (!(tl <= th)) return Ival{-pi, pi};
    return Ival{fmax(tl, -pi), fmin(th, pi)};
}
SDF_IA void circ_set(const Ival &d, const Ival &a, double delta, Ival &x, Ival &y) {
    x = y = top();
    if (!finite_(d) || !finite_(a) || delta != delta) return;
    Ival sn, cs;
    sincos_range(subc(a, delta), sn, cs);
    x = mul(cs, d);
    y = mul(sn, d);
}
SDF_IA double ease_value(int id, double t, bool &known) {
    double u, v;
    known = true;
    switch (id) {
    case EASE_linear: return t;
    case EASE_in_quad: return t * t;
    case EASE_out_quad: return -t * (t - 2.0);
    case EASE_in_out_quad: u = 2.0 * t - 1.0; return t < 0.5 ? 2.0 * t * t : -0.5 * (u * (u - 2.0) - 1.0);
    case EASE_in_cubic: return t * t * t;
    case EASE_out_cubic: u = t - 1.0; return u * u * u + 1.0;
    case EASE_in_out_cubic: u = t * 2.0; v = u - 2.0; return u < 1.0 ? 0.5 * u * u * u : 0.5 * (v * v * v + 2.0);
    case EASE_in_quart: return t * t * t * t;
    case EASE_out_quart: u = t - 1.0; return -(u * u * u * u - 1.0);
    case EASE_in_out_quart: u = t * 2.0; v = u - 2.0; return u < 1.0 ? 0.5 * u * u * u * u : -0.5 * (v * v * v * v - 2.0);
    case EASE_in_quint: return t * t * t * t * t;
    case EASE_out_quint: u = t - 1.0; return u * u * u * u * u + 1.0;
    case EASE_in_out_quint: u = t * 2.0; v = u - 2.0; return u < 1.0 ? 0.5 * u * u * u * u * u : 0.5 * (v * v * v * v * v + 2.0);
    case EASE_in_circ: return -1.0 * (sqrt(fmax(1.0 - t * t, 0.0)) - 1.0);
    case EASE_out_circ: u = t - 1.0; return sqrt(fmax(1.0 - u * u, 0.0));
    case EASE_in_out_circ:
        u = t * 2.0; v = u - 2.0;
        return u < 1.0 ? -0.5 * (sqrt(fmax(1.0 - u * u, 0.0)) - 1.0) : 0.5 * (sqrt(fmax(1.0 - v * v, 0.0)) + 1.0);
    case EASE_in_square: return t < 1.0 ? 0.0 : 1.0;
    case EASE_out_square: return t > 0.0 ? 1.0 : 0.0;
    case EASE_in_out_square: return t < 0.5 ? 0.0 : 1.0;
    default: known = false; return 0.0;
    }
}
SDF_IA Ival ease01(int id, const Ival &t) {
    if (bad(t) || t.lo < 0.0 || t.hi > 1.0) return top();
    bool k0, k1;
    const double a = ease_value(id, t.lo, k0), b = ease_value(id, t.hi, k1);
    if (!k0 || !k1 || a != a || b != b) return top();
    return Ival{fmin(a, b) - 1e-12, fmax(a, b) + 1e-12};
}

}

enum { PRUNE_BLOCK = 256 };
struct IaShared {
    double *base;
    int n_p;
    int stride;
#if defined(__HIP_DEVICE_COMPILE__)
    __device__ __forceinline__ static int lane_slot() { return (int)threadIdx.x; }
#elif defined(SDF_HOST_SIMT)
    static int lane_slot() { return sdf_host_simt_tid(); }
#else
    static int lane_slot() { return 0; }
#endif
    SDF_IA double &ps(uint32_t slot, int k) { return base[(slot * 6 + k) * stride + lane_slot()]; }
    SDF_IA double &ds(uint32_t slot, int k) { return base[(n_p * 6 + slot * 2 + k) * stride + lane_slot()]; }
};
__host__ __device__ inline size_t prune_lds_bytes(int n_p, int n_d) { return (size_t)(6 * n_p + 2 * n_d) * PRUNE_BLOCK * 8; }


__host__ __device__ inline bool ia_has_form(uint32_t op) {
    switch (op) {
    case OP_END: case OP_L_SPHERE: case OP_L_PLANE: case OP_L_BOX: case OP_L_ROUNDED_BOX: case OP_L_TORUS: case OP_L_CYLINDER:
    case OP_L_ROUNDED_CYLINDER: case OP_L_CAPSULE: case OP_L_OCTAHEDRON: case OP_L_CIRCLE: case OP_L_LINE: case OP_L_RECTANGLE:
    case OP_L_WIREFRAME_BOX: case OP_L_CAPPED_CYLINDER: case OP_L_ROUNDED_CONE: case OP_L_ELLIPSOID: case OP_L_TETRAHEDRON:
    case OP_L_DODECAHEDRON: case OP_L_ICOSAHEDRON: case OP_L_ROUNDED_RECTANGLE: case OP_L_EQUILATERAL_TRIANGLE: case OP_L_HEXAGON:
    case OP_L_ROUNDED_X: case OP_L_VESICA: case OP_L_CAPPED_CONE: case OP_L_PYRAMID: case OP_L_POLYGON: case OP_L_TEXTURE2D:
    case OP_L_GRID3D:
    case OP_COMB: case OP_TRANSLATE: case OP_SCALE: case OP_ROTATE: case OP_ELONGATE: case OP_TRANSLATE2: case OP_SCALE2:
    case OP_ROTATE2: case OP_ELONGATE2: case OP_REVOLVE: case OP_SETZ0: case OP_SAVE_P: case OP_LOAD_P: case OP_PUSH_D: case OP_NOP:
    case OP_NEG: case OP_ADDC: case OP_SUBC: case OP_MULC: case OP_SHELL: case OP_ADD_DS: case OP_EXT_PRE: case OP_EXT_POST:
    case OP_REP_PREP: case OP_REP_SET: case OP_CIRC_PREP: case OP_CIRC_SET: case OP_BEND_LINEAR:
    case OP_TWIST: case OP_BEND: case OP_BEND_RADIAL: case OP_TRANS_LIN_PRE: case OP_TRANS_RAD_PRE: case OP_TRANS_MIX:
    case OP_EXTTO_PRE: case OP_EXTTO_MIX: case OP_SLICE_POST: case OP_WRAP_AROUND:
        return true;
    default: return false;
    }
}

SDF_IA Ival ia_box_like(const Ival &qx, const Ival &qy, const Ival &qz) {
    using namespace ia;
    const Ival mx = max_(max_(qx, qy), qz);
    return add(len3(maxc(qx, 0.0), maxc(qy, 0.0), maxc(qz, 0.0)), minc(mx, 0.0));
}

SDF_IA Ival ia_leaf(uint32_t op, const double *c, const Ival &x, const Ival &y, const Ival &z) {
    using namespace ia;
    switch (op) {
    case OP_L_SPHERE: return subc(len3(subc(x, c[1]), subc(y, c[2]), subc(z, c[3])), c[0]);
    case OP_L_PLANE: return dot3c(csub(c[3], x), csub(c[4], y), csub(c[5], z), c[0], c[1], c[2]);
    case OP_L_BOX:
        return ia_box_like(subc(abs_(subc(x, c[0])), c[3]), subc(abs_(subc(y, c[1])), c[4]), subc(abs_(subc(z, c[2])), c[5]));
    case OP_L_ROUNDED_BOX:
        return subc(ia_box_like(addc(subc(abs_(x), c[0]), c[3]), addc(subc(abs_(y), c[1]), c[3]), addc(subc(abs_(z), c[2]), c[3])), c[3]);
    case OP_L_TORUS: return subc(len2(subc(len2(x, y), c[0]), z), c[1]);
    case OP_L_CYLINDER: return subc(len2(x, y), c[0]);
    case OP_L_ROUNDED_CYLINDER: {
        const Ival d0 = addc(subc(len2(x, y), c[0]), c[1]), d1 = addc(subc(abs_(z), c[2]), c[1]);
        return subc(add(minc(max_(d0, d1), 0.0), len2(maxc(d0, 0.0), maxc(d1, 0.0))), c[1]);
    }
    case OP_L_CAPSULE: {
        const Ival pax = subc(x, c[0]), pay = subc(y, c[1]), paz = subc(z, c[2]);
        const Ival h = clip01(divc(dot3c(pax, pay, paz, c[3], c[4], c[5]), c[6]));
        return subc(len3(sub(pax, mulc(h, c[3])), sub(pay, mulc(h, c[4])), sub(paz, mulc(h, c[5]))), c[7]);
    }
    case OP_L_OCTAHEDRON: return mulc(subc(add(add(abs_(x), abs_(y)), abs_(z)), c[0]), c[1]);
    case OP_L_CIRCLE: return subc(len2(subc(x, c[1]), subc(y, c[2])), c[0]);
    case OP_L_LINE: return dot2c(csub(c[2], x), csub(c[3], y), c[0], c[1]);
    case OP_L_RECTANGLE: {
        const Ival qx = subc(abs_(subc(x, c[0])), c[2]), qy = subc(abs_(subc(y, c[1])), c[3]);
        return add(len2(maxc(qx, 0.0), maxc(qy, 0.0)), minc(max_(qx, qy), 0.0));
    }
    default: return top();

    }
}

SDF_IA bool ia_is_rare_leaf(uint32_t op) {
    switch (op) {
    case OP_L_WIREFRAME_BOX: case OP_L_CAPPED_CYLINDER: case OP_L_ROUNDED_CONE: case OP_L_ELLIPSOID: case OP_L_TETRAHEDRON:
    case OP_L_DODECAHEDRON: case OP_L_ICOSAHEDRON: case OP_L_ROUNDED_RECTANGLE: case OP_L_EQUILATERAL_TRIANGLE: case OP_L_HEXAGON:
    case OP_L_ROUNDED_X: case OP_L_VESICA: case OP_L_CAPPED_CONE: case OP_L_PYRAMID: case OP_L_POLYGON: case OP_L_TEXTURE2D:
    case OP_L_GRID3D:
        return true;
    default: return false;
    }
}
__host__ __device__ __attribute__((noinline)) inline Ival ia_leaf_rare(uint32_t op, const double *c, const Ival &x, const Ival &y, const Ival &z) {
    using namespace ia;
    switch (op) {
    case OP_L_WIREFRAME_BOX: {
        const double t2 = c[3];
        const Ival px = subc(subc(abs_(x), c[0]), t2), py = subc(subc(abs_(y), c[1]), t2), pz = subc(subc(abs_(z), c[2]), t2);
        const Ival qx = subc(abs_(addc(px, t2)), t2), qy = subc(abs_(addc(py, t2)), t2), qz = subc(abs_(addc(pz, t2)), t2);
        const Ival g0 = add(len3(maxc(px, 0.0), maxc(qy, 0.0), maxc(qz, 0.0)), minc(max_(px, max_(qy, qz)), 0.0));
        const Ival g1 = add(len3(maxc(qx, 0.0), maxc(py, 0.0), maxc(qz, 0.0)), minc(max_(qx, max_(py, qz)), 0.0));
        const Ival g2 = add(len3(maxc(qx, 0.0), maxc(qy, 0.0), maxc(pz, 0.0)), minc(max_(qx, max_(qy, pz)), 0.0));
        return min_(min_(g0, g1), g2);
    }
    case OP_L_CAPPED_CYLINDER: {
        const double bax = c[3], bay = c[4], baz = c[5], baba = c[6];
        if (!(baba > 0.0)) return top();
        const Ival pax = subc(x, c[0]), pay = subc(y, c[1]), paz = subc(z, c[2]);
        const Ival paba = dot3c(pax, pay, paz, bax, bay, baz);
        const Ival xx = subc(len3(sub(mulc(pax, baba), mulc(paba, bax)), sub(mulc(pay, baba), mulc(paba, bay)),
                                  sub(mulc(paz, baba), mulc(paba, baz))), c[8]);
        const Ival yy = subc(abs_(subc(paba, c[9])), c[9]);
        const Ival x2 = sqr(xx), y2 = mulc(sqr(yy), baba);
        const Ival zero = pt(0.0);
        const Ival din = neg(min_(x2, y2));
        const Ival dout = add(sel_gt(xx, zero, x2, zero), sel_gt(yy, zero, y2, zero));
        const Ival d = sel_gt(zero, max_(xx, yy), din, dout);
        if (bad(d)) return top();
        const double lo = (d.lo > 0.0 ? 1.0 : (d.lo < 0.0 ? -1.0 : 0.0)) * sqrt(fabs(d.lo)) / baba;
        const double hi = (d.hi > 0.0 ? 1.0 : (d.hi < 0.0 ? -1.0 : 0.0)) * sqrt(fabs(d.hi)) / baba;
        return wide(lo, hi);
    }
    case OP_L_ROUNDED_CONE: {
        const double r1 = c[0], r2 = c[1], h = c[2], b = c[3], a = c[4], ah = c[5];
        const Ival qx = len2(x, y), qy = z;
        const Ival k = dot2c(qx, qy, -b, a);
        const Ival c1 = subc(len2(qx, qy), r1), c2 = subc(len2(qx, subc(qy, h)), r2), c3 = subc(dot2c(qx, qy, a, b), r1);
        if (bad(k) || ah != ah) return top();
        Ival r{0.0, 0.0};
        bool any = false;
        if (k.lo < 0.0) { r = c1; any = true; }
        if (k.hi >= 0.0) {
            if (k.hi > ah) { r = any ? hull(r, c2) : c2; any = true; }
            if (fmax(k.lo, 0.0) <= ah) { r = any ? hull(r, c3) : c3; any = true; }
        }
        return any ? fix(r) : top();
    }
    case OP_L_ELLIPSOID: {
        const Ival k0 = len3(divc(x, c[0]), divc(y, c[1]), divc(z, c[2]));
        const Ival k1 = len3(divc(x, c[3]), divc(y, c[4]), divc(z, c[5]));
        return div_pos(mul(k0, subc(k0, 1.0)), k1);
    }
    case OP_L_TETRAHEDRON:
        return divc(subc(max_(sub(abs_(add(x, y)), z), add(abs_(sub(x, y)), z)), c[0]), c[1]);
    case OP_L_DODECAHEDRON: case OP_L_ICOSAHEDRON: {
        const double r = c[0], X = c[1], Y = c[2], Z = c[3];
        const Ival ax = abs_(divc(x, r)), ay = abs_(divc(y, r)), az = abs_(divc(z, r));
        const Ival a = dot3c(ax, ay, az, X, Y, Z), b = dot3c(ax, ay, az, Z, X, Y), cc = dot3c(ax, ay, az, Y, Z, X);
        const Ival m = subc(max_(max_(a, b), cc), X);
        if (op == OP_L_DODECAHEDRON) return mulc(m, r);
        return mulc(max_(m, subc(dot3c(ax, ay, az, c[4], c[4], c[4]), X)), r);
    }
    case OP_L_ROUNDED_RECTANGLE: {
        if (bad(x) || bad(y)) return top();
        const bool xt = x.hi > 0.0, xf = !(x.lo > 0.0), yt = y.hi > 0.0, yf = !(y.lo > 0.0);
        double rl = __builtin_inf(), rh = -__builtin_inf();
        if (xt && yt) { rl = fmin(rl, c[2]); rh = fmax(rh, c[2]); }
        if (xt && yf) { rl = fmin(rl, c[3]); rh = fmax(rh, c[3]); }
        if (xf && yf) { rl = fmin(rl, c[4]); rh = fmax(rh, c[4]); }
        if (xf && yt) { rl = fmin(rl, c[5]); rh = fmax(rh, c[5]); }
        if (!(rl <= rh)) return top();
        const Ival r{rl, rh};
        const Ival qx = add(subc(abs_(x), c[0]), r), qy = add(subc(abs_(y), c[1]), r);
// ... 75 lines not shown
        const Ival ti = addc(mulc(u, c[4]), c[6]), tj = addc(mulc(vv, c[5]), c[7]);
        const Ival qx = subc(abs_(subc(x, c[10])), c[12]), qy = subc(abs_(subc(y, c[11])), c[13]);
        const Ival q = add(len2(maxc(qx, 0.0), maxc(qy, 0.0)), minc(max_(qx, qy), 0.0));
        if (bad(ti) || bad(tj) || !finite_(ti) || !finite_(tj)) return top();
        const double wi = (double)(tw - 1), hj = (double)(th - 1);
        if (ti.hi < 0.0 || ti.lo >= wi || tj.hi < 0.0 || tj.lo >= hj) return q;
        const int i0 = (int)floor(fmax(ti.lo, 0.0)), i1 = (int)fmin(floor(fmin(ti.hi, wi)) + 1.0, wi);
        const int j0 = (int)floor(fmax(tj.lo, 0.0)), j1 = (int)fmin(floor(fmin(tj.hi, hj)) + 1.0, hj);
        if ((long long)(i1 - i0 + 1) * (long long)(j1 - j0 + 1) > 1024) return top();
        double lo = __builtin_inf(), hi = -__builtin_inf();
        for (int j = j0; j <= j1; j++)
            for (int i = i0; i <= i1; i++) { const double p = tex[(size_t)j * tw + i]; lo = fmin(lo, p); hi = fmax(hi, p); if (p != p) return top(); }
        if (!(lo <= hi)) return top();
        const Ival d = pad(Ival{lo, hi}, 1e-12, 1e-300);
        const bool all_inside = ti.lo >= 0.0 && ti.hi < wi && tj.lo >= 0.0 && tj.hi < hj;
        return all_inside ? d : hull(d, q);
    }
    case OP_L_GRID3D: {
        const int n[3] = {(int)c[0], (int)c[1], (int)c[2]};
        const double bg = c[3];
        if (n[0] < 2 || n[1] < 2 || n[2] < 2 || bad(x) || bad(y) || bad(z) || !(bg == bg)) return top();
        const Ival e = ia_box_like(subc(abs_(subc(x, c[4])), c[7]), subc(abs_(subc(y, c[5])), c[8]), subc(abs_(subc(z, c[6])), c[9]));
        if (bad(e)) return top();
        if (e.lo > bg) return e;
        const double *g[3] = {c + 10, c + 10 + n[0], c + 10 + n[0] + n[1]};
        const double *vox = c + 10 + n[0] + n[1] + n[2];
        const Ival *pv[3] = {&x, &y, &z};
        int i0[3], i1[3];
        bool oob = false;
        for (int a = 0; a < 3; a++) {
            const double plo = pv[a]->lo, phi = pv[a]->hi;
            int lo = 0, hi = n[a];
            while (lo < hi) { const int mid = (lo + hi) >> 1; if (g[a][mid] < plo) lo = mid + 1; else hi = mid; }
            i0[a] = lo - 1 < 0 ? 0 : (lo - 1 > n[a] - 2 ? n[a] - 2 : lo - 1);
            lo = 0; hi = n[a];
            while (lo < hi) { const int mid = (lo + hi) >> 1; if (g[a][mid] < phi) lo = mid + 1; else hi = mid; }
            i1[a] = (lo - 1 < 0 ? 0 : (lo - 1 > n[a] - 2 ? n[a] - 2 : lo - 1)) + 1;
            oob = oob || plo < g[a][0] || phi > g[a][n[a] - 1];
        }
        if ((long long)(i1[0] - i0[0] + 1) * (long long)(i1[1] - i0[1] + 1) * (long long)(i1[2] - i0[2] + 1) > 4096) return top();
        double lo = __builtin_inf(), hi = -__builtin_inf();
        for (int i = i0[0]; i <= i1[0]; i++)
            for (int j = i0[1]; j <= i1[1]; j++)
                for (int k = i0[2]; k <= i1[2]; k++) {
                    const double p = vox[((size_t)i * n[1] + j) * n[2] + k];
                    if (p != p) return top();
                    lo = fmin(lo, p); hi = fmax(hi, p);
                }
        if (!(lo <= hi)) return top();
        Ival d = pad(Ival{lo, hi}, 1e-12, 1e-300);
        if (oob) d = hull(d, pt(bg));
        return e.hi <= bg ? d : hull(e, d);
    }
    case OP_L_POLYGON: {
        const int np_ = (int)c[0];
        const double *pv = c + 1;
        if (np_ < 1 || bad(x) || bad(y) || !finite_(x) || !finite_(y)) return top();
        Ival d = add(sqr(subc(x, pv[0])), sqr(subc(y, pv[1])));
        double sgn = 1.0;
        double scale2 = x.hi * x.hi + y.hi * y.hi + x.lo * x.lo + y.lo * y.lo;
        for (int i = 0; i < np_; i++) {
            const int j = (i + np_ - 1) % np_;
            const double vix = pv[2 * i], viy = pv[2 * i + 1], vjx = pv[2 * j], vjy = pv[2 * j + 1];
            const double ex = vjx - vix, ey = vjy - viy;
            const Ival wx = subc(x, vix), wy = subc(y, viy);
            const double ee = fma(ey, ey, ex * ex);
            const Ival cl = clip01(divc(dot2c(wx, wy, ex, ey), ee));
            const Ival bx = sub(wx, mulc(cl, ex)), by = sub(wy, mulc(cl, ey));
            d = min_(d, add(sqr(bx), sqr(by)));
            const double pwx = x.lo - vix, pwy = y.lo - viy;
            const bool c1 = y.lo >= viy, c2 = y.lo < vjy, c3 = ex * pwy > ey * pwx;
            if ((c1 && c2 && c3) || (!c1 && !c2 && !c3)) sgn = -sgn;
            scale2 += vix * vix + viy * viy;
        }
        const Ival r = sqrt_(d);
        if (bad(d) || bad(r) || !(scale2 == scale2)) return top();
        if (d.lo > 1e-24 * (1.0 + scale2)) return sgn > 0.0 ? r : neg(r);
        return Ival{-r.hi, r.hi};
    }
    default: return top();
    }
}

SDF_IA Ival ia_post(uint32_t post, const Ival &d1, const Ival &d2, double K) {
    using namespace ia;
    switch (post) {
    case POST_SET: return d2;
    case POST_UNION: return min_(d1, d2);
    case POST_DIFF: return max_(d1, neg(d2));
    case POST_INTER: return max_(d1, d2);
    case POST_BLEND: return add(mulc(d2, K), mulc(d1, 1.0 - K));
    default: break;
    }
    if (!(K > 0.0) || bad(d1) || bad(d2)) return top();
    const Ival e = post == POST_SDIFF ? neg(d2) : d2;
    const Ival ad = abs_(sub(e, d1));
    const double tmin = fmin(ad.lo / K, 1.0), tmax = fmin(ad.hi / K, 1.0);
    const double cmax = 0.25 * K * (1.0 - tmin) * (1.0 - tmin), cmin = 0.25 * K * (1.0 - tmax) * (1.0 - tmax);
    Ival r = post == POST_SUNION ? min_(d1, e) : max_(d1, e);
    if (post == POST_SUNION) { r.lo -= cmax; r.hi -= cmin; } else { r.lo += cmin; r.hi += cmax; }
    const double m = 1e-9 * (fabs(r.lo) + fabs(r.hi) + K);
    return fix(Ival{r.lo - m, r.hi + m});
}

SDF_IA int ia_decide(uint32_t post, const Ival &left, const Ival &right, double K) {
    using namespace ia;
    switch (post) {
    case POST_UNION: return right.lo > left.hi ? 1 : (left.lo > right.hi ? 2 : 0);
    case POST_INTER: return right.hi < left.lo ? 1 : (left.hi < right.lo ? 2 : 0);
    case POST_DIFF: return -right.lo < left.lo ? 1 : (left.hi < -right.hi ? 2 : 0);
    case POST_SUNION: case POST_SINTER: case POST_SDIFF: {
        if (!(K > 0.0) || !finite_(left) || !finite_(right)) return 0;
        Ival e;
        if (post == POST_SUNION) e = addc(divc(mulc(sub(right, left), 0.5), K), 0.5);
        else if (post == POST_SINTER) e = csub(0.5, divc(mulc(sub(right, left), 0.5), K));
        else e = csub(0.5, divc(mulc(add(right, left), 0.5), K));
        if (bad(e) || !(e.hi <= 0.0)) return 0;
        return post == POST_SDIFF ? 1 : 2;
    }
    default: return 0;
    }
}

__device__ __forceinline__ void mask_set_range(uint32_t *m, int a, int b) {
    for (int k = 0; k < 8; k++) {
        const int lo = a - 32 * k, hi = b - 32 * k;
        if (hi < 0 || lo > 31) continue;
        m[k] |= (0xFFFFFFFFu >> (31 - (hi > 31 ? 31 : hi))) & (0xFFFFFFFFu << (lo < 0 ? 0 : lo));
    }
}

__device__ __forceinline__ void mask_set_bit(uint32_t *m, int i) {
    for (int k = 0; k < 8; k++) if ((i >> 5) == k) m[k] |= 1u << (i & 31);
}
__device__ __forceinline__ uint32_t mask_word(const uint32_t *m, int idx) {
    uint32_t r = 0;
    for (int k = 0; k < 8; k++) r = idx == k ? m[k] : r;
    return r;
}

SDF_IA void ia_keep_bit(uint32_t *m, int i) {
    for (int k = 0; k < 8; k++) if ((i >> 5) == k) m[k] |= 1u << (i & 31);
}

template <bool DECIDE, bool FULL, bool RARE>
SDF_IA Ival ia_run_tape(const uint32_t *__restrict__ code, const double *__restrict__ consts,
                        const uint16_t *__restrict__ rstart, const uint16_t *__restrict__ lstart, int n_instr,
                        Ival x, Ival y, Ival z, bool live, IaShared sh, int n_d, uint32_t *masks) {
    using namespace ia;
#if defined(__HIP_DEVICE_COMPILE__)
    const int lane = threadIdx.x & 63, gbase = lane & ~7;
#endif
    Ival acc = pt(0.0);
    for (int i = 0; i < sh.n_p; i++)
        for (int k = 0; k < 6; k++) sh.ps(i, k) = 0.0;
    for (int i = 0; i < n_d; i++) { sh.ds(i, 0) = 0.0; sh.ds(i, 1) = 0.0; }
    uint32_t keep[8] = {0, 0, 0, 0, 0, 0, 0, 0};
    auto psave = [&](uint32_t k) {
        sh.ps(k, 0) = x.lo; sh.ps(k, 1) = x.hi; sh.ps(k, 2) = y.lo; sh.ps(k, 3) = y.hi; sh.ps(k, 4) = z.lo; sh.ps(k, 5) = z.hi;
    };
    auto pload = [&](uint32_t k) {
        x = Ival{sh.ps(k, 0), sh.ps(k, 1)}; y = Ival{sh.ps(k, 2), sh.ps(k, 3)}; z = Ival{sh.ps(k, 4), sh.ps(k, 5)};
    };
    auto dsave = [&](uint32_t k, const Ival &v) { sh.ds(k, 0) = v.lo; sh.ds(k, 1) = v.hi; };
    auto dload = [&](uint32_t k) { return Ival{sh.ds(k, 0), sh.ds(k, 1)}; };
    for (int ip = 0; ip < n_instr; ip++) {
        const uint32_t w0 = code[2 * ip], w1 = code[2 * ip + 1];
        const uint32_t op = w0 & 255u, post = (w0 >> 8) & 7u, sa = (w0 >> 24) & 7u;
        const double *c = consts + (w1 & 0xFFFFFFu) + 1;
        if (op == OP_END) break;
        if (w0 & 0x000800u) pload((w0 >> 12) & 7u);
        if (w0 & 0x008000u) psave((w0 >> 16) & 7u);
        if (w0 & 0x080000u) dsave((w0 >> 20) & 7u, acc);
        const bool is_leaf = op >= OP_L_SPHERE && op < OP_COMB;
        if (is_leaf || op == OP_COMB) {
            const Ival left = is_leaf ? acc : dload(sa);
            Ival right = acc;
            if (is_leaf) {
                if (RARE && ia_is_rare_leaf(op)) right = ia_leaf_rare(op, c, x, y, z);
                else right = ia_leaf(op, c, x, y, z);
            }
            int rs = 0xFFFF, ls = 0xFFFF;
            if constexpr (DECIDE) { rs = rstart[ip]; ls = lstart[ip]; }
#if defined(__HIP_DEVICE_COMPILE__)
            if (DECIDE && rs != 0xFFFF && ls != 0xFFFF && rs <= ip && ls <= rs) {
                const int d = live ? ia_decide(post, left, right, c[-1]) : 3;
                const unsigned long long b1 = __ballot(d == 1 || d == 3), b2 = __ballot(d == 2 || d == 3);
                if (((b1 >> gbase) & 0xFFull) == 0xFFull) {
                    if (post < POST_SUNION) mask_set_range(masks, rs, ip);
                    else {
                        if (rs < ip) mask_set_range(masks, rs, ip - 1);
                        mask_set_bit(masks + 8, ip);
                    }
                } else if (((b2 >> gbase) & 0xFFull) == 0xFFull && rs > ls) {
                    mask_set_range(masks, ls, rs - 1);
                    mask_set_bit(masks + 8, ip);
                }
            }
#endif
            acc = ia_post(post, left, right, c[-1]);
            continue;
        }
        switch (op) {
        case OP_TRANSLATE: x = subc(x, c[0]); y = subc(y, c[1]); z = subc(z, c[2]); break;
        case OP_SCALE: x = divc(x, c[0]); y = divc(y, c[1]); z = divc(z, c[2]); break;
        case OP_ROTATE: {
            const Ival nx = dot3c(x, y, z, c[0], c[3], c[6]);
            const Ival ny = dot3c(x, y, z, c[1], c[4], c[7]);
            const Ival nz = dot3c(x, y, z, c[2], c[5], c[8]);
            x = nx; y = ny; z = nz; break; }
        case OP_ELONGATE: {
            const Ival qx = subc(abs_(x), c[0]), qy = subc(abs_(y), c[1]), qz = subc(abs_(z), c[2]);
            dsave(sa, minc(max_(qx, max_(qy, qz)), 0.0));
            x = maxc(qx, 0.0); y = maxc(qy, 0.0); z = maxc(qz, 0.0); break; }
        case OP_TRANSLATE2: x = subc(x, c[0]); y = subc(y, c[1]); break;
        case OP_SCALE2: x = divc(x, c[0]); y = divc(y, c[1]); break;
        case OP_ROTATE2: {
            const Ival nx = dot2c(x, y, c[0], c[2]), ny = dot2c(x, y, c[1], c[3]);
            x = nx; y = ny; break; }
        case OP_ELONGATE2: {
            const Ival qx = subc(abs_(x), c[0]), qy = subc(abs_(y), c[1]);
            dsave(sa, minc(max_(qx, qy), 0.0));
            x = maxc(qx, 0.0); y = maxc(qy, 0.0); break; }
        case OP_REVOLVE: { const Ival nx = subc(len2(x, y), c[0]); y = z; x = nx; z = pt(0.0); break; }
        case OP_SETZ0: z = pt(0.0); break;
        case OP_SAVE_P: psave(sa); if constexpr (DECIDE) ia_keep_bit(keep, ip); break;
        case OP_LOAD_P: pload(sa); if constexpr (DECIDE) ia_keep_bit(keep, ip); break;
        case OP_PUSH_D: dsave(sa, acc); break;
        case OP_NOP: break;
        case OP_NEG: acc = neg(acc); break;
        case OP_ADDC: acc = addc(acc, c[0]); break;
        case OP_SUBC: acc = subc(acc, c[0]); break;
        case OP_MULC: acc = mulc(acc, c[0]); break;
        case OP_SHELL: acc = subc(abs_(acc), c[0]); break;
        case OP_ADD_DS: acc = add(acc, dload(sa)); break;
        case OP_EXT_PRE: dsave(sa, subc(abs_(z), c[0])); break;
        case OP_EXT_POST: {
            const Ival w = dload(sa);
            acc = add(minc(max_(acc, w), 0.0), len2(maxc(acc, 0.0), maxc(w, 0.0))); break; }
        case OP_BEND_LINEAR: {
            const Ival tt = ease01((int)c[10], clip01(divc(dot3c(subc(x, c[0]), subc(y, c[1]), subc(z, c[2]), c[3], c[4], c[5]), c[6])));
            x = add(x, mulc(tt, c[7])); y = add(y, mulc(tt, c[8])); z = add(z, mulc(tt, c[9])); break; }
        case OP_REP_PREP: {
            const int dim = (int)c[0];
            Ival idx[3] = {pt(0.0), pt(0.0), pt(0.0)};
            const Ival pp[3] = {x, y, z};
            for (int i = 0; i < 3; i++) {
                if (i >= dim) continue;
                const double s = c[1 + i];
                Ival r = s != 0.0 ? rint_(divc(pp[i], s)) : pt(0.0);
                if (c[4] != 0.0) r = clipc(r, -c[5 + i], c[5 + i]);
                idx[i] = r;
            }
            sh.ps(sa, 0) = idx[0].lo; sh.ps(sa, 1) = idx[0].hi; sh.ps(sa, 2) = idx[1].lo; sh.ps(sa, 3) = idx[1].hi;
            sh.ps(sa, 4) = idx[2].lo; sh.ps(sa, 5) = idx[2].hi; break; }
        case OP_REP_SET: {
            const uint32_t sb = (w1 >> 24) & 7u;
            const Ival ax{sh.ps(sa, 0), sh.ps(sa, 1)}, ay{sh.ps(sa, 2), sh.ps(sa, 3)}, az{sh.ps(sa, 4), sh.ps(sa, 5)};
            const Ival bx{sh.ps(sb, 0), sh.ps(sb, 1)}, by{sh.ps(sb, 2), sh.ps(sb, 3)}, bz{sh.ps(sb, 4), sh.ps(sb, 5)};
            x = sub(ax, mulc(addc(bx, c[3]), c[0]));
            y = sub(ay, mulc(addc(by, c[4]), c[1]));
            z = sub(az, mulc(addc(bz, c[5]), c[2])); break; }
        case OP_TRANS_LIN_PRE:
            dsave(sa, ease01((int)c[7], clip01(divc(dot3c(subc(x, c[0]), subc(y, c[1]), subc(z, c[2]), c[3], c[4], c[5]), c[6])))); break;
        case OP_TRANS_MIX: {
            const uint32_t sb = (w1 >> 24) & 7u;
            const Ival tt = dload(sa), dd = dload(sb);
            acc = add(mul(tt, acc), mul(csub(1.0, tt), dd)); break; }
        case OP_EXTTO_PRE:
            dsave(sa, ease01((int)c[1], addc(clipc(divc(z, c[0]), -0.5, 0.5), 0.5))); break;
        case OP_EXTTO_MIX: {
            const uint32_t sb = (w1 >> 24) & 7u;
            const Ival dd1 = dload(sb), tt = dload(sa);
            acc = add(dd1, mul(sub(acc, dd1), tt)); break; }
        case OP_SLICE_POST: {
            const Ival A = dload(sa), B = neg(acc);
            if (bad(A) || bad(B)) acc = top();
            else if (A.hi <= 0.0) acc = B;
            else if (A.lo > 0.0) acc = A;
            else acc = Ival{fmin(A.lo, B.lo), fmax(A.hi, B.hi)};
            break; }
        case OP_TWIST: case OP_BEND: case OP_BEND_RADIAL: case OP_TRANS_RAD_PRE: case OP_WRAP_AROUND:
            if constexpr (FULL) {
                if (op == OP_WRAP_AROUND) {
                    const double pi = 3.141592653589793;
                    Ival r = finite_(x) && finite_(y) ? pad(len2(x, y), 1e-12, 1e-300) : top();
                    if (!bad(r)) r.lo = fmax(r.lo, 0.0);
                    const Ival d = subc(r, c[9]);
                    const Ival u = divc(addc(atan2_range(x, y), pi), 2.0 * pi);
                    const Ival tt = bad(u) ? top() : ease01((int)c[10], Ival{fmax(u.lo, 0.0), fmin(u.hi, 1.0)});
                    const Ival nx = add(addc(mulc(tt, c[3]), c[0]), mulc(d, c[6])), ny = add(addc(mulc(tt, c[4]), c[1]), mulc(d, c[7]));
                    x = nx; y = ny;
                } else
                if (op == OP_TWIST || op == OP_BEND) {
                    Ival sn, cs;
                    sincos_range(mulc(op == OP_TWIST ? z : x, c[0]), sn, cs);
                    const Ival nx = sub(mul(cs, x), mul(sn, y)), ny = add(mul(sn, x), mul(cs, y));
                    x = nx; y = ny;
                } else {
                    Ival r = finite_(x) && finite_(y) ? pad(len2(x, y), 1e-12, 1e-300) : top();
                    if (!bad(r)) r.lo = fmax(r.lo, 0.0);
                    const Ival tt = clip01(divc(subc(r, c[0]), c[1]));
                    if (op == OP_BEND_RADIAL) z = sub(z, mulc(ease01((int)c[3], tt), c[2]));
                    else dsave(sa, ease01((int)c[2], tt));
                }
                break;
            }
            [[fallthrough]];
        case OP_CIRC_PREP: case OP_CIRC_SET:
            if constexpr (FULL) {
                if (op == OP_CIRC_PREP) {
                    Ival d, a;
                    circ_prep(x, y, c[0], d, a);
                    sh.ps(sa, 0) = d.lo; sh.ps(sa, 1) = d.hi; sh.ps(sa, 2) = a.lo; sh.ps(sa, 3) = a.hi;
                    sh.ps(sa, 4) = z.lo; sh.ps(sa, 5) = z.hi;
                } else {
                    const Ival d{sh.ps(sa, 0), sh.ps(sa, 1)}, a{sh.ps(sa, 2), sh.ps(sa, 3)};
                    circ_set(d, a, c[0], x, y);
                    z = Ival{sh.ps(sa, 4), sh.ps(sa, 5)};
                }
                break;
            }
            [[fallthrough]];
        default:
            x = y = z = top(); acc = top();
            for (int k = 0; k < n_d; k++) dsave(k, top());
            if (op == OP_REP_PREP || op == OP_CIRC_PREP) psave(sa);
            break;
        }
    }
    if constexpr (DECIDE)
        for (int k = 0; k < 8; k++) masks[k] &= ~keep[k];
    return acc;
}

__device__ __forceinline__ int compact_tape(const unsigned long long *__restrict__ code64, int n_instr, const uint32_t *masks,
                                            unsigned long long *__restrict__ out, bool store, uint32_t zero_off) {
    const unsigned long long PREFIX = 0x00FFF800ull, POSTM = 0x700ull;
    const unsigned long long ADD0 = ((unsigned long long)zero_off << 32) | OP_ADDC;
    int n = 0;
    auto put = [&](unsigned long long w) { if (store) out[n] = w; n++; };
    uint32_t skip_w = 0, force_w = 0;
    for (int ip = 0; ip < n_instr; ip++) {
        const unsigned long long w = code64[ip];
        const uint32_t op = (uint32_t)w & 255u, post = ((uint32_t)w >> 8) & 7u;
        if ((ip & 31) == 0) { skip_w = mask_word(masks, ip >> 5); force_w = mask_word(masks + 8, ip >> 5); }
        const bool skip = skip_w & 1u, forced = force_w & 1u;
        skip_w >>= 1; force_w >>= 1;
        if (skip) {
            if (w & PREFIX) put((w & PREFIX) | OP_NOP);
        } else if (!forced) {
            put(w);
        } else if (post == POST_SDIFF) {
            put((w & PREFIX) | ADD0);
        } else if (op == OP_COMB) {
            if (post == POST_DIFF) put((w & PREFIX) | OP_NEG);
            else if (post >= POST_SUNION) put((w & PREFIX) | ADD0);
            else if (w & PREFIX) put((w & PREFIX) | OP_NOP);
        } else {
            put(w & ~POSTM);
            if (post == POST_DIFF) put(OP_NEG);
            else if (post >= POST_SUNION) put(ADD0);
        }
    }
    return n;
}

}
```

sdf_amd/engine.py:

```python
import ctypes
import os
import threading
import weakref

import numpy as np

from . import tape as _tape

_HERE = os.path.dirname(os.path.abspath(__file__))
LIB_PATH = os.environ.get('SDF_HIP_LIB') or os.path.join(_HERE, 'csrc', 'libsdf_hip.so')

PRECISION_F64 = 0
PRECISION_F32 = 1

_c_i64 = ctypes.c_int64
_vp = ctypes.c_void_p
_f64p = ctypes.POINTER(ctypes.c_double)
_f32p = ctypes.POINTER(ctypes.c_float)
_u32p = ctypes.POINTER(ctypes.c_uint32)
_u8p = ctypes.POINTER(ctypes.c_uint8)


class SdfExchangeStats(ctypes.Structure):
    _fields_ = [(k, ctypes.c_int64) for k in ('n_batches', 'n_skipped', 'n_empty', 'n_nonempty', 'n_triangles', 'n_grid_voxels',
                                               'n_eval_voxels', 'n_ambiguous_cells', 'n_sampled_voxels', 'n_pruned_instrs',
                                               'n_retries', 'chunks', 'world', 'slab_bytes')] + \
               [(k, ctypes.c_double) for k in ('ms_mesh', 'ms_exchange', 'ms_expand', 'ms_total')] + \
               [('per_rank_triangles', ctypes.c_int64 * 64)]


class SdfMoments(ctypes.Structure):
    _fields_ = [('sums', ctypes.c_double * 11), ('origin', ctypes.c_double * 3), ('box_lo', ctypes.c_double * 3),
                ('box_hi', ctypes.c_double * 3), ('n_triangles', _c_i64), ('n_zero_area', _c_i64), ('n_nonfinite', _c_i64)]


CENSUS_FIELDS = ('vertices', 'faces', 'collapsed', 'edges', 'paired', 'boundary', 'misoriented', 'nonmanifold', 'euler', 'closed',
                 'oriented')


class SdfEdgeCensus(ctypes.Structure):
    _fields_ = [(k, _c_i64) for k in CENSUS_FIELDS]


class SdfStats(ctypes.Structure):
    _fields_ = [
        ('n_batches', _c_i64), ('n_skipped', _c_i64), ('n_empty', _c_i64), ('n_nonempty', _c_i64),
        ('n_triangles', _c_i64), ('n_grid_voxels', _c_i64), ('n_eval_voxels', _c_i64),
        ('n_ambiguous_cells', _c_i64), ('n_work_begin', _c_i64), ('n_work_end', _c_i64),
        ('n_retries', _c_i64),
        ('ms_prepass', ctypes.c_double), ('ms_mesh', ctypes.c_double), ('ms_emit', ctypes.c_double),
        ('ms_total', ctypes.c_double), ('n_pruned_instrs', _c_i64), ('n_batch_instrs', _c_i64),
        ('n_sampled_voxels', _c_i64), ('ms_mesh_device', ctypes.c_double), ('sclk_mhz', ctypes.c_double),
        ('t_mesh_first_us', ctypes.c_double), ('t_mesh_last_us', ctypes.c_double), ('mesh_kernel', ctypes.c_int64),
    ]


ABI = {
    'sdf_abi_version': (ctypes.c_int, []),
    'sdf_build_info': (ctypes.c_char_p, []),
    'sdf_last_error': (ctypes.c_char_p, []),
    'sdf_device_count': (ctypes.c_int, []),
    'sdf_device_mem_info': (ctypes.c_int, [ctypes.c_int, ctypes.POINTER(ctypes.c_size_t), ctypes.POINTER(ctypes.c_size_t)]),
    'sdf_test_fail_alloc': (ctypes.c_int, [ctypes.c_int]),
    'sdf_ctx_create': (ctypes.c_int, [ctypes.c_int, ctypes.POINTER(_vp)]),
    'sdf_ctx_destroy': (ctypes.c_int, [_vp]),
    'sdf_ctx_set_stream': (ctypes.c_int, [_vp, _vp]),
    'sdf_ctx_set_prune': (ctypes.c_int, [_vp, ctypes.c_int]),
    'sdf_ctx_set_cull': (ctypes.c_int, [_vp, ctypes.c_int]),
    'sdf_ctx_set_twopass': (ctypes.c_int, [_vp, ctypes.c_int]),
    'sdf_ctx_set_tail_order': (ctypes.c_int, [_vp, ctypes.c_int]),
    'sdf_ctx_set_defer': (ctypes.c_int, [_vp, ctypes.c_int]),
    'sdf_ctx_set_cull_levels': (ctypes.c_int, [_vp, ctypes.c_int]),
    'sdf_ctx_synchronize': (ctypes.c_int, [_vp]),
    'sdf_ctx_trim': (ctypes.c_int, [_vp]),
    'sdf_tape_create': (ctypes.c_int, [_vp, _u32p, ctypes.c_uint32, _f64p, ctypes.c_uint32,
                                       ctypes.c_uint32, ctypes.c_uint32, ctypes.POINTER(_vp)]),
    'sdf_tape_set_prune_info': (ctypes.c_int, [_vp, ctypes.POINTER(ctypes.c_uint16), ctypes.POINTER(ctypes.c_uint16),
                                               ctypes.c_uint32]),
    'sdf_tape_destroy': (ctypes.c_int, [_vp]),
    'sdf_eval_points': (ctypes.c_int, [_vp, _vp, _c_i64, ctypes.c_int, _vp, ctypes.c_int]),
    'sdf_eval_points_host': (ctypes.c_int, [_vp, _f64p, _c_i64, ctypes.c_int, _f64p, ctypes.c_int]),
    'sdf_eval_grid_host': (ctypes.c_int, [_vp, _f64p, ctypes.c_int, _f64p, ctypes.c_int, _f64p,
                                          ctypes.c_int, _f64p, ctypes.c_int]),
    'sdf_estimate_bounds': (ctypes.c_int, [_vp, _f64p, ctypes.c_int]),
    'sdf_tape_extern_count': (ctypes.c_int, [_vp]),
    'sdf_eval_extern_points_host': (ctypes.c_int, [_vp, _f64p, _c_i64, ctypes.c_int, _f64p, ctypes.c_int]),
    'sdf_eval_points_extern_host': (ctypes.c_int, [_vp, _f64p, _c_i64, ctypes.c_int, _f64p, _f64p, ctypes.c_int]),
    'sdf_generate_field': (ctypes.c_int, [_vp, _vp, _vp, _f64p, ctypes.c_int, _f64p, ctypes.c_int, _f64p, ctypes.c_int,
                                          ctypes.c_int, ctypes.c_int, _c_i64, _c_i64, ctypes.POINTER(_vp)]),
    'sdf_marching_cubes': (ctypes.c_int, [_vp, _vp, ctypes.c_int, ctypes.c_int, ctypes.c_int, _vp,
                                          _c_i64, ctypes.POINTER(_c_i64)]),
    'sdf_marching_cubes_host': (ctypes.c_int, [_vp, _f32p, ctypes.c_int, ctypes.c_int, ctypes.c_int,
                                               _f32p, _c_i64, ctypes.POINTER(_c_i64)]),
    'sdf_mesh_level_set_host': (ctypes.c_int, [_vp, _f64p, _c_i64, ctypes.POINTER(ctypes.c_int32), _c_i64, ctypes.c_double,
                                               ctypes.c_int, ctypes.POINTER(_c_i64), ctypes.POINTER(_c_i64), _f32p, _c_i64]),
    'sdf_distance_texture_host': (ctypes.c_int, [_vp, _u8p, _c_i64, _c_i64, _f64p]),
    'sdf_render_host': (ctypes.c_int, [_vp, _f64p, ctypes.c_int, ctypes.c_int, _f64p, ctypes.c_int, ctypes.c_int, _f64p, _f64p,
                                       ctypes.POINTER(ctypes.c_int32), _u8p]),
    'sdf_render_last_kernel_ms': (ctypes.c_double, []),
    'sdf_generate': (ctypes.c_int, [_vp, _f64p, ctypes.c_int, _f64p, ctypes.c_int, _f64p, ctypes.c_int,
                                    ctypes.c_int, ctypes.c_int, _c_i64, _c_i64, ctypes.c_int,
                                    ctypes.POINTER(_vp)]),
    'sdf_generate_to_device': (ctypes.c_int, [_vp, _f64p, ctypes.c_int, _f64p, ctypes.c_int, _f64p, ctypes.c_int,
                                              ctypes.c_int, ctypes.c_int, _c_i64, _c_i64, ctypes.c_int, _vp, _c_i64,
                                              ctypes.POINTER(ctypes.c_int), ctypes.POINTER(_vp)]),
    'sdf_generate_to_device_async': (ctypes.c_int, [_vp, _f64p, ctypes.c_int, _f64p, ctypes.c_int, _f64p, ctypes.c_int,
                                                    ctypes.c_int, ctypes.c_int, ctypes.c_int64, ctypes.c_int64,
                                                    ctypes.c_int, _vp, ctypes.c_int64, ctypes.POINTER(_vp)]),
    'sdf_mesh_wait': (ctypes.c_int, [_vp, ctypes.POINTER(ctypes.c_int)]),
    'sdf_generate_records': (ctypes.c_int, [_vp, _f64p, ctypes.c_int, _f64p, ctypes.c_int, _f64p, ctypes.c_int,
                                            ctypes.c_int, ctypes.c_int, ctypes.c_int, ctypes.POINTER(_vp)]),
    'sdf_slab_bytes': (ctypes.c_size_t, [_c_i64, _c_i64]),
    'sdf_generate_compact_async': (ctypes.c_int, [_vp, _f64p, ctypes.c_int, _f64p, ctypes.c_int, _f64p, ctypes.c_int,
                                                  ctypes.c_int, ctypes.c_int, _c_i64, _c_i64, ctypes.c_int, _vp, _c_i64,
                                                  _c_i64, ctypes.POINTER(_vp)]),
    'sdf_expand_slabs': (ctypes.c_int, [_vp, ctypes.POINTER(_vp), ctypes.c_int, _c_i64, _c_i64, _vp, _c_i64]),
    'sdf_comm_available': (ctypes.c_int, []),
    'sdf_comm_unique_id': (ctypes.c_int, [_vp]),
    'sdf_comm_create': (ctypes.c_int, [_vp, _vp, ctypes.c_int, ctypes.c_int, ctypes.c_int, ctypes.POINTER(_vp)]),
    'sdf_comm_destroy': (ctypes.c_int, [_vp]),
    'sdf_generate_sharded_async': (ctypes.c_int, [_vp, _vp, _f64p, ctypes.c_int, _f64p, ctypes.c_int, _f64p, ctypes.c_int,
                                                  ctypes.c_int, ctypes.c_int, ctypes.c_int, ctypes.c_int, ctypes.c_int,
                                                  ctypes.POINTER(_vp)]),
    'sdf_exchange_wait': (ctypes.c_int, [_vp, ctypes.POINTER(_vp), ctypes.POINTER(_c_i64)]),
    'sdf_exchange_stats_get': (ctypes.c_int, [_vp, ctypes.POINTER(SdfExchangeStats)]),
    'sdf_exchange_destroy': (ctypes.c_int, [_vp]),
    'sdf_skip_kinds': (ctypes.c_int, [_vp, _f64p, ctypes.c_int, _f64p, ctypes.c_int, _f64p, ctypes.c_int, ctypes.c_int, _c_i64,
                                      _c_i64, ctypes.c_int, _vp]),
    'sdf_generate_from_kinds': (ctypes.c_int, [_vp, _f64p, ctypes.c_int, _f64p, ctypes.c_int, _f64p, ctypes.c_int, ctypes.c_int,
                                               _c_i64, _c_i64, ctypes.c_int, _vp, ctypes.POINTER(_vp)]),
    'sdf_memcpy_to_host': (ctypes.c_int, [_vp, _vp, _vp, ctypes.c_size_t]),
    'sdf_mesh_stats': (ctypes.c_int, [_vp, ctypes.POINTER(SdfStats)]),
    'sdf_mesh_triangles': (_c_i64, [_vp]),
    'sdf_mesh_emit_device': (ctypes.c_int, [_vp, _vp]),
    'sdf_mesh_emit_host': (ctypes.c_int, [_vp, _f64p]),
    'sdf_mesh_emit_host_workers': (ctypes.c_int, [_vp, _f64p, ctypes.c_int]),
    'sdf_mesh_emit_host_range': (ctypes.c_int, [_vp, _c_i64, _c_i64, _f64p]),
    'sdf_mesh_batch_offsets': (ctypes.c_int, [_vp, ctypes.POINTER(_c_i64)]),
    'sdf_mesh_emit_stl_host': (ctypes.c_int, [_vp, _vp]),
    'sdf_mesh_adopt_soup': (ctypes.c_int, [_vp, _vp, _c_i64, ctypes.POINTER(_vp)]),
    'sdf_mesh_weld': (ctypes.c_int, [_vp, ctypes.POINTER(ctypes.c_int64)]),
    'sdf_mesh_weld_fetch': (ctypes.c_int, [_vp, _f64p, ctypes.POINTER(ctypes.c_int64)]),
    'sdf_mesh_vertex_normals': (ctypes.c_int, [_vp, _vp, ctypes.c_double, _f64p, ctypes.POINTER(ctypes.c_int64)]),
    'sdf_mesh_normals_last_kernel_ms': (ctypes.c_double, []),
    'sdf_mesh_emit_ply_host': (ctypes.c_int, [_vp, ctypes.c_int, _vp, _vp]),
    'sdf_mesh_moments': (ctypes.c_int, [_vp, _f64p, ctypes.POINTER(SdfMoments)]),
    'sdf_mesh_edge_census': (ctypes.c_int, [_vp, ctypes.POINTER(SdfEdgeCensus)]),
    'sdf_mesh_measure_last_kernel_ms': (ctypes.c_double, []),
    'sdf_host_alloc': (ctypes.c_int, [ctypes.c_size_t, ctypes.POINTER(_vp)]),
    'sdf_host_free': (ctypes.c_int, [_vp]),
    'sdf_mesh_kinds': (ctypes.c_int, [_vp, _u8p]),
    'sdf_mesh_prune_masks': (ctypes.c_int, [_vp, _u32p]),
    'sdf_mesh_destroy': (ctypes.c_int, [_vp]),
}
ABI_VERSION = 15


def build_info():
    return load_library().sdf_build_info().decode()


def _strip_c_comments(text):
    out, i, n = [], 0, len(text)
    while i < n:
        ch = text[i]
        if ch in '"\'':
            j = i + 1
            while j < n and text[j] != ch:
                j += 2 if text[j] == '\\' else 1
            out.append(text[i:j + 1]); i = j + 1
        elif text.startswith('//', i):
            j = text.find('\n', i)
            i = n if j < 0 else j
        elif text.startswith('/*', i):
            j = text.find('*/', i + 2)
            i = n if j < 0 else j + 2
        else:
            out.append(ch); i += 1
    return ''.join(out)


def source_id():
    import glob
    import hashlib
    import re
    h = hashlib.sha256()
    here = os.path.dirname(os.path.abspath(__file__))
    d = os.path.join(here, 'csrc')
    files = sorted(glob.glob(os.path.join(d, '*'))) + [os.path.join(os.path.dirname(here), 'include', 'sdf_hip.h')]
    for f in files:
        ext = f.rsplit('.', 1)[-1]
        if os.path.isfile(f) and ext in ('h', 'hip', 'inc', 'sh'):
            text = open(f, encoding='utf-8', errors='replace').read()
            if ext == 'sh':
                text = re.sub(r'(?m)^\s*#(?!!).*$', '', text)
            else:
                text = _strip_c_comments(text)
            text = '\n'.join(ln.rstrip() for ln in text.split('\n') if ln.strip())
            h.update(os.path.basename(f).encode()); h.update(text.encode())
    return h.hexdigest()[:16]

_lib = None
_lib_lock = threading.Lock()


class SdfHipError(RuntimeError):
    pass


FIELD_FN = ctypes.CFUNCTYPE(ctypes.c_int, _vp, _f64p, _c_i64, _f64p)


def call_closure(fn, P):
    v = np.asarray(fn(P), dtype=np.float64).reshape(-1)
    if v.shape[0] != len(P):
        raise ValueError('a user SDF returned %d values for %d points' % (v.shape[0], len(P)))
    return v


def load_library(path=None):
    global _lib
    with _lib_lock:
        if _lib is not None and path is None:
            return _lib
        p = path or LIB_PATH
        if not os.path.exists(p):
            raise SdfHipError(
                '%s is missing: build the HIP extension first '
                '(python -c "import __graft_entry__ as g; g.build()"); sdf_amd has no CPU path' % p)
        lib = ctypes.CDLL(p)
        for name, (rt, at) in ABI.items():
            fn = getattr(lib, name)
            fn.restype = rt
            fn.argtypes = at
        if lib.sdf_abi_version() != ABI_VERSION:
            raise SdfHipError('libsdf_hip.so ABI %d != binding %d' % (lib.sdf_abi_version(), ABI_VERSION))
        if path is None:
            _lib = lib
# ... 239 lines not shown
        d.update(batches=st.n_batches, skipped=st.n_skipped, empty=st.n_empty, nonempty=st.n_nonempty, triangles=st.n_triangles,
                 payload='16-byte triangle records (local coordinates) + per-batch transform', exchange='rccl (native)')
        return DeviceSoup(self.comm.engine, p.value, n.value, keep=self), d

    def close(self):
        self._fin()


class Comm:

    @staticmethod
    def available(lib):
        if lib.sdf_comm_available():
            return True, ''
        return False, (lib.sdf_last_error() or b'').decode(errors='replace')

    @staticmethod
    def unique_ids(lib, n_lanes=2):
        buf = ctypes.create_string_buffer(COMM_ID_BYTES * n_lanes)
        for l in range(n_lanes):
            _check(lib, lib.sdf_comm_unique_id(ctypes.cast(ctypes.byref(buf, COMM_ID_BYTES * l), _vp)))
        return buf.raw

    def __init__(self, eng, ids, rank, world):
        self.engine, self.rank, self.world = eng, int(rank), int(world)
        self.n_lanes = len(ids) // COMM_ID_BYTES
        self.handle = _vp()
        raw = ctypes.create_string_buffer(bytes(ids), len(ids))
        _check(eng.lib, eng.lib.sdf_comm_create(eng.ctx, ctypes.cast(raw, _vp), self.n_lanes, self.rank, self.world,
                                                ctypes.byref(self.handle)))
        self._fin = weakref.finalize(self, eng.lib.sdf_comm_destroy, self.handle)
        self._live = weakref.WeakSet()

    def submit(self, sdf, X, Y, Z, batch_size=32, sparse=True, chunks=1, lane=0):
        eng = self.engine
        dt = eng.tape_for(sdf)
        if dt.tape.externs:
            raise ValueError('a model with user closures is sharded through the host protocol (sdf_amd.dist with HostCodec)')
        X, Y, Z = (np.ascontiguousarray(a, dtype=np.float64) for a in (X, Y, Z))
        h = _vp()
        _check(eng.lib, eng.lib.sdf_generate_sharded_async(self.handle, dt.handle, _dp(X, _f64p), len(X), _dp(Y, _f64p), len(Y),
                                                           _dp(Z, _f64p), len(Z), int(batch_size), 1 if sparse else 0,
                                                           eng.precision, int(chunks), int(lane), ctypes.byref(h)))
        return Exchange(self, h, dt)

    def close(self):
        for x in list(self._live):
            x.close()
        self._fin()


class Engine:

    def __init__(self, device=0):
        self.lib = load_library()
        n = self.lib.sdf_device_count()
        if n <= 0:
            raise SdfHipError('no HIP device visible (sdf_amd has no CPU path): %s'
                              % (self.lib.sdf_last_error() or b'').decode())
        self.device = device
        self.ctx = _vp()
        _check(self.lib, self.lib.sdf_ctx_create(device, ctypes.byref(self.ctx)))
        self._fin = weakref.finalize(self, self.lib.sdf_ctx_destroy, self.ctx)
        self.precision = PRECISION_F64
        self._tapes = weakref.WeakValueDictionary()

    def set_stream(self, stream_ptr):
        _check(self.lib, self.lib.sdf_ctx_set_stream(self.ctx, _vp(stream_ptr)))

    def set_prune(self, enabled):
        _check(self.lib, self.lib.sdf_ctx_set_prune(self.ctx, int(bool(enabled))))

    def set_cull(self, enabled):
        _check(self.lib, self.lib.sdf_ctx_set_cull(self.ctx, int(bool(enabled))))

    def set_tail_order(self, on):
        _check(self.lib, self.lib.sdf_ctx_set_tail_order(self.ctx, int(bool(on))))

    def set_defer(self, on):
        _check(self.lib, self.lib.sdf_ctx_set_defer(self.ctx, int(bool(on))))

    def set_cull_levels(self, levels):
        _check(self.lib, self.lib.sdf_ctx_set_cull_levels(self.ctx, int(levels)))

    def set_twopass(self, mode):
        _check(self.lib, self.lib.sdf_ctx_set_twopass(self.ctx, int(mode)))

    def synchronize(self):
        _check(self.lib, self.lib.sdf_ctx_synchronize(self.ctx))

    def trim(self):
        _check(self.lib, self.lib.sdf_ctx_trim(self.ctx))

    def tape_for(self, sdf):
        if isinstance(sdf, DeviceTape):
            return sdf
        t = sdf if isinstance(sdf, _tape.Tape) else _tape.lower(sdf)
        key = (t.code.tobytes(), t.consts.tobytes(), tuple(id(fn) for fn, _ in t.externs))
        dt = self._tapes.get(key)
        if dt is None:
            dt = DeviceTape(self, t)
            self._tapes[key] = dt
        return dt

    def eval_points(self, sdf, pts):
        dt = self.tape_for(sdf)
        pts = np.ascontiguousarray(pts, dtype=np.float64)
        if pts.ndim != 2 or pts.shape[1] not in (2, 3):
            raise ValueError('points must be (N,2) or (N,3)')
        if dt.tape.externs:
            return self._eval_points_hybrid(dt, pts)
        out = np.empty(len(pts), np.float64)
        if len(pts):
            _check(self.lib, self.lib.sdf_eval_points_host(dt.handle, _dp(pts, _f64p), len(pts), pts.shape[1],
                                                           _dp(out, _f64p), self.precision))
        return out

    def _eval_points_hybrid(self, dt, pts):
        ext = dt.tape.externs
        n, dim = pts.shape
        if n == 0:
            return np.empty(0, np.float64)
        if dt.tape.n_instr == 2:
            return call_closure(ext[0][0], pts.copy())
        epts = np.empty((len(ext), n, 3), np.float64)
        _check(self.lib, self.lib.sdf_eval_extern_points_host(dt.handle, _dp(pts, _f64p), n, dim, _dp(epts, _f64p),
                                                              self.precision))
        vals = np.empty((len(ext), n), np.float64)
        for k, (fn, d) in enumerate(ext):
            vals[k] = call_closure(fn, np.ascontiguousarray(epts[k, :, :d]))
        out = np.empty(n, np.float64)
        _check(self.lib, self.lib.sdf_eval_points_extern_host(dt.handle, _dp(pts, _f64p), n, dim, _dp(vals, _f64p),
                                                              _dp(out, _f64p), self.precision))
        return out

    def estimate_bounds(self, sdf):
        dt = self.tape_for(sdf)
        if dt.tape.externs:
            return None
        out = np.zeros(6, np.float64)
        lib = self.lib
        if lib.sdf_estimate_bounds(dt.handle, _dp(out, _f64p), self.precision) != 0:
            msg = (lib.sdf_last_error() or b'').decode()
            if msg.startswith('zero-size array'):
                raise ValueError(msg)
            if 'barrier' in msg:
                return None
            raise SdfHipError(msg)
        return (tuple(out[:3]), tuple(out[3:]))

    def eval_grid(self, sdf, X, Y, Z):
        dt = self.tape_for(sdf)
        X, Y, Z = (np.ascontiguousarray(a, dtype=np.float64) for a in (X, Y, Z))
        if dt.tape.externs:
            G = np.stack(np.meshgrid(X, Y, Z, indexing='ij'), axis=-1).reshape(-1, 3)
            return self._eval_points_hybrid(dt, np.ascontiguousarray(G)).reshape(len(X), len(Y), len(Z))
        out = np.empty((len(X), len(Y), len(Z)), np.float64)
        if out.size:
            _check(self.lib, self.lib.sdf_eval_grid_host(dt.handle, _dp(X, _f64p), len(X), _dp(Y, _f64p), len(Y),
                                                         _dp(Z, _f64p), len(Z), _dp(out, _f64p), self.precision))
        return out

    def marching_cubes(self, volume):
        vol = np.ascontiguousarray(volume, dtype=np.float32)
        if vol.ndim != 3:
            raise ValueError('Input volume should be a 3D numpy array.')
# ... 211 lines not shown
```

Measured before the change: 625.1 billion voxels/s.

## Evaluate multiple cull boxes per thread and pack sub-box states as 2-bit words

Generalizes the interval-arithmetic tape interpreter to evaluate NB boxes per thread (ia_run_tape_nb), with per-box shared-state stride. Adds 2-box cull kernels that can be selected through a new ctx setting or env var. Sub-box cull states are now kept as packed 2-bit fields, written with workgroup-scope atomic ORs, instead of a byte array that was repacked afterwards. This is meant to raise ILP in the cull interpreter and cut LDS traffic and repacking work. The cost is more register pressure and halved per-pass shared capacity when NB=2.

```diff
diff --git a/include/sdf_hip.h b/include/sdf_hip.h
--- a/include/sdf_hip.h
+++ b/include/sdf_hip.h
@@ -8,7 +8,7 @@
 extern "C" {
 #endif
 
-#define SDF_ABI_VERSION 15
+#define SDF_ABI_VERSION 16
 
 #define SDF_PRECISION_F64 0
 #define SDF_PRECISION_F32 1
@@ -59,6 +59,7 @@
 int sdf_ctx_set_twopass(sdf_ctx *ctx, int mode);
 int sdf_ctx_set_defer(sdf_ctx *ctx, int on);
 int sdf_ctx_set_cull_levels(sdf_ctx *ctx, int levels);
+int sdf_ctx_set_cull_boxes(sdf_ctx *ctx, int boxes);
 int sdf_ctx_set_tail_order(sdf_ctx *ctx, int on);
 int sdf_ctx_synchronize(sdf_ctx *ctx);
 int sdf_ctx_trim(sdf_ctx *ctx);
diff --git a/sdf_amd/csrc/sdf_device.h b/sdf_amd/csrc/sdf_device.h
--- a/sdf_amd/csrc/sdf_device.h
+++ b/sdf_amd/csrc/sdf_device.h
@@ -364,7 +364,7 @@
     }
 };
 
-enum { CULL_UNIT_CAP = 3072, CULL_ULIST = 8, CULL_SBYTES = CULL_ULIST, CULL_SSTATE = CULL_ULIST + 2 * CULL_UNIT_CAP, CULL_COLINFO = CULL_SSTATE + 1024,
+enum { CULL_UNIT_CAP = 3072, CULL_ULIST = 8, CULL_SSTATE = CULL_ULIST + 2 * CULL_UNIT_CAP, CULL_COLINFO = CULL_SSTATE + 1024,
        CULL_RECORD = CULL_COLINFO + 1160,
        CULL_MSTATE = CULL_RECORD, CULL_GSTATE = CULL_MSTATE + 64, CULL_ELIST = CULL_GSTATE + 512, CULL_PACC = CULL_ELIST + 1024,
        CULL_SCRATCH = CULL_PACC + 64 };
@@ -376,7 +376,8 @@
     ix = ok ? x : 0; iy = ok ? y : 0; iz = ok ? z : 0;
     return ok;
 }
-template <int BLOCK, bool FULL, bool RARE>
+__device__ __forceinline__ void cull_or_bits(unsigned *p, unsigned v) { __hip_atomic_fetch_or(p, v, __ATOMIC_RELAXED, __HIP_MEMORY_SCOPE_WORKGROUP); }
+template <int BLOCK, bool FULL, bool RARE, int NB = 1>
 __device__ __forceinline__ int cull_tasks(const uint32_t *wcode, const double *consts, int n_instr_w, int lx, int ly, int lz,
                                        const double *axes, double *ia_state, int ia_bytes, unsigned char *scratch, int *wave_sums,
                                        int ia_np, int ia_nd, unsigned long long *prof = nullptr, int levels = 3) {
@@ -386,23 +387,26 @@
     if (prof && tid == 0) for (int k = 0; k < 12; k++) pacc[k] = 0;
 #define SDF_CULL_PROF(K) do { if (prof && tid == 0) { const long long tn = clock64(); pacc[(K) - 16] += (unsigned)(tn - tprev); tprev = tn; } } while (0)
     const int c0 = lx - 1, c1 = ly - 1, c2 = lz - 1;
-    const int per_pass = min(BLOCK, ia_bytes / ((6 * ia_np + 2 * ia_nd) * 8)) & ~63;
+    const int per_pass = min(BLOCK, ia_bytes / ((6 * ia_np + 2 * ia_nd) * 8 * NB)) & ~63;
     if (c0 <= 0 || c1 <= 0 || c2 <= 0 || per_pass < 64) return -1;
     unsigned short *ulist = reinterpret_cast<unsigned short *>(scratch + CULL_ULIST);
-    unsigned char *sstate = scratch + CULL_SBYTES;
-    static_assert(2 * CULL_UNIT_CAP >= 4096, "the byte states lie over the unit list");
+    unsigned *pk = reinterpret_cast<unsigned *>(scratch + CULL_SSTATE);
     unsigned char *mstate = scratch + CULL_MSTATE;
     unsigned char *gstate = scratch + CULL_GSTATE;
     unsigned short *elist = reinterpret_cast<unsigned short *>(scratch + CULL_ELIST);
-    auto box_state = [&](int x0, int x1, int y0, int y1, int z0, int z1) -> unsigned char {
-        Ival bx{axes[x0], axes[min(x1, c0)]}, by{axes[33 + y0], axes[33 + min(y1, c1)]}, bz{axes[66 + z0], axes[66 + min(z1, c2)]};
-        if (bx.lo > bx.hi) { const double t = bx.lo; bx.lo = bx.hi; bx.hi = t; }
-        if (by.lo > by.hi) { const double t = by.lo; by.lo = by.hi; by.hi = t; }
-        if (bz.lo > bz.hi) { const double t = bz.lo; bz.lo = bz.hi; bz.hi = t; }
-        if (ia::bad(bx) || ia::bad(by) || ia::bad(bz)) { bx = by = bz = ia::top(); }
-        const Ival v = ia_run_tape<false, FULL, RARE>(wcode, consts, nullptr, nullptr, n_instr_w, bx, by, bz, true,
-                                          IaShared{ia_state, ia_np, per_pass}, ia_nd, nullptr);
-        return v.lo > 1e-30 ? 1 : (v.hi < -1e-30 ? 2 : 0);
+    auto box_states = [&](const int (&x0)[NB], const int (&y0)[NB], const int (&z0)[NB], int ext, unsigned char (&st)[NB]) {
+        Ival bx[NB], by[NB], bz[NB], v[NB];
+        SDF_UNROLL for (int b = 0; b < NB; b++) {
+            bx[b] = Ival{axes[x0[b]], axes[min(x0[b] + ext, c0)]}; by[b] = Ival{axes[33 + y0[b]], axes[33 + min(y0[b] + ext, c1)]};
+            bz[b] = Ival{axes[66 + z0[b]], axes[66 + min(z0[b] + ext, c2)]};
+            if (bx[b].lo > bx[b].hi) { const double t = bx[b].lo; bx[b].lo = bx[b].hi; bx[b].hi = t; }
+            if (by[b].lo > by[b].hi) { const double t = by[b].lo; by[b].lo = by[b].hi; by[b].hi = t; }
+            if (bz[b].lo > bz[b].hi) { const double t = bz[b].lo; bz[b].lo = bz[b].hi; bz[b].hi = t; }
+            if (ia::bad(bx[b]) || ia::bad(by[b]) || ia::bad(bz[b])) { bx[b] = by[b] = bz[b] = ia::top(); }
+        }
+        ia_run_tape_nb<false, FULL, RARE, NB>(wcode, consts, nullptr, nullptr, n_instr_w, bx, by, bz, true,
+                                              IaShared{ia_state, ia_np, NB * per_pass}, per_pass, ia_nd, nullptr, v);
+        SDF_UNROLL for (int b = 0; b < NB; b++) st[b] = v[b].lo > 1e-30 ? 1 : (v[b].hi < -1e-30 ? 2 : 0);
     };
     int phase = 0, e0 = 0, nev = 0;
     for (;;) {
@@ -418,40 +422,58 @@
                 if (und) elist[pos] = (unsigned short)gi;
                 nund += n;
             }
-            for (int h = tid; h < 4096; h += BLOCK) {
-                const int h0 = h >> 8, h1 = (h >> 4) & 15, h2 = h & 15;
-                const bool exists = 2 * h0 < c0 && 2 * h1 < c1 && 2 * h2 < c2;
-                sstate[h] = exists ? gstate[((h0 >> 1) * 8 + (h1 >> 1)) * 8 + (h2 >> 1)] : 1;
+            SDF_CULL_PROF(26);
+            const int n2 = (c2 + 1) >> 1;
+            const unsigned inside = n2 >= 16 ? 0xFFFFFFFFu : (1u << (2 * n2)) - 1u;
+            for (int r = tid; r < 256; r += BLOCK) {
+                const int h0 = r >> 4, h1 = r & 15;
+                unsigned long long x = *reinterpret_cast<const unsigned long long *>(gstate + ((h0 >> 1) * 8 + (h1 >> 1)) * 8) & 0x0303030303030303ull;
+                x = (x | (x >> 6)) & 0x000F000F000F000Full; x = (x | (x >> 12)) & 0x000000FF000000FFull; x = (x | (x >> 24)) & 0xFFFFull;
+                unsigned y = (unsigned)x;
+                y = (y | (y << 8)) & 0x00FF00FFu; y = (y | (y << 4)) & 0x0F0F0F0Fu; y = (y | (y << 2)) & 0x33333333u;
+                y |= y << 2;
+                pk[r] = 2 * h0 < c0 && 2 * h1 < c1 ? (y & inside) | (0x55555555u & ~inside) : 0x55555555u;
             }
             __syncthreads();
+            SDF_CULL_PROF(27);
             phase = 2; e0 = 0; nev = 8 * nund;
         }
         if (phase == 2 && e0 >= nev) break;
         const bool run = phase == 0 ? tid < 64 : (tid < per_pass && e0 + (tid & ~63) < nev);
-        int target = 0, x0, y0, z0, ext;
-        bool live;
+        int target[NB], x0[NB], y0[NB], z0[NB], ext;
+        bool live[NB];
         if (phase == 0) {
             const int m0 = tid >> 4, m1 = (tid >> 2) & 3, m2 = tid & 3;
-            live = 8 * m0 < c0 && 8 * m1 < c1 && 8 * m2 < c2;
-            x0 = live ? 8 * m0 : 0; y0 = live ? 8 * m1 : 0; z0 = live ? 8 * m2 : 0; ext = 8;
+            live[0] = 8 * m0 < c0 && 8 * m1 < c1 && 8 * m2 < c2;
+            x0[0] = live[0] ? 8 * m0 : 0; y0[0] = live[0] ? 8 * m1 : 0; z0[0] = live[0] ? 8 * m2 : 0; ext = 8; target[0] = 0;
+            SDF_UNROLL for (int b = 1; b < NB; b++) { live[b] = false; target[b] = 0; x0[b] = x0[0]; y0[b] = y0[0]; z0[b] = z0[0]; }
         } else if (phase == 1) {
-            live = e0 + tid < nev;
-            target = run ? (int)elist[min(e0 + tid, nev - 1)] : 0;
-            x0 = 4 * (target >> 6); y0 = 4 * ((target >> 3) & 7); z0 = 4 * (target & 7); ext = 4;
+            ext = 4;
+            SDF_UNROLL for (int b = 0; b < NB; b++) {
+                const int e = e0 + b * per_pass + tid;
+                live[b] = e < nev;
+                target[b] = run ? (int)elist[min(e, nev - 1)] : 0;
+                x0[b] = 4 * (target[b] >> 6); y0[b] = 4 * ((target[b] >> 3) & 7); z0[b] = 4 * (target[b] & 7);
+            }
         } else {
-            const int e = min(e0 + tid, nev - 1);
-            const int gq = run ? (int)elist[e >> 3] : 0, ch = e & 7;
-            const int h0 = 2 * (gq >> 6) + (ch >> 2), h1 = 2 * ((gq >> 3) & 7) + ((ch >> 1) & 1), h2 = 2 * (gq & 7) + (ch & 1);
-            live = e0 + tid < nev && 2 * h0 < c0 && 2 * h1 < c1 && 2 * h2 < c2;
-            target = (h0 * 16 + h1) * 16 + h2;
-            x0 = live ? 2 * h0 : 0; y0 = live ? 2 * h1 : 0; z0 = live ? 2 * h2 : 0; ext = 2;
+            ext = 2;
+            SDF_UNROLL for (int b = 0; b < NB; b++) {
+                const int e = min(e0 + b * per_pass + tid, nev - 1);
+                const int gq = run ? (int)elist[e >> 3] : 0, ch = e & 7;
+                const int h0 = 2 * (gq >> 6) + (ch >> 2), h1 = 2 * ((gq >> 3) & 7) + ((ch >> 1) & 1), h2 = 2 * (gq & 7) + (ch & 1);
+                live[b] = e0 + b * per_pass + tid < nev && 2 * h0 < c0 && 2 * h1 < c1 && 2 * h2 < c2;
+                target[b] = (h0 * 16 + h1) * 16 + h2;
+                x0[b] = live[b] ? 2 * h0 : 0; y0[b] = live[b] ? 2 * h1 : 0; z0[b] = live[b] ? 2 * h2 : 0;
+            }
         }
         if (run) {
-            const unsigned char st = box_state(x0, x0 + ext, y0, y0 + ext, z0, z0 + ext);
-            if (phase == 0) mstate[tid & 63] = live ? st : 1;
-            else if (live) (phase == 1 ? gstate : sstate)[target] = st;
-        }
-        if (phase != 0) { if (prof && tid == 0) pacc[7]++; e0 += per_pass; continue; }
+            unsigned char st[NB];
+            box_states(x0, y0, z0, ext, st);
+            if (phase == 0) mstate[tid & 63] = live[0] ? st[0] : 1;
+            else if (phase == 1) { SDF_UNROLL for (int b = 0; b < NB; b++) if (live[b]) gstate[target[b]] = st[b]; }
+            else { SDF_UNROLL for (int b = 0; b < NB; b++) if (live[b] && st[b]) cull_or_bits(pk + (target[b] >> 4), (unsigned)st[b] << (2 * (target[b] & 15))); }
+        }
+        if (phase != 0) { if (prof && tid == 0) pacc[7]++; e0 += NB * per_pass; continue; }
         SDF_CULL_PROF(17);
         __syncthreads();
         for (int g0 = 0; g0 < 512; g0 += BLOCK) {
@@ -474,15 +496,12 @@
     SDF_CULL_PROF(20);
     unsigned short *ub = reinterpret_cast<unsigned short *>(scratch + CULL_GSTATE);
     for (int r = tid; r < 256; r += BLOCK) {
-        const unsigned long long lo8 = *reinterpret_cast<const unsigned long long *>(sstate + 16 * r);
-        const unsigned long long hi8 = *reinterpret_cast<const unsigned long long *>(sstate + 16 * r + 8);
-        unsigned m = 0, pk = 0;
-        SDF_UNROLL for (int k = 0; k < 8; k++) { m |= ((lo8 >> (8 * k)) & 255ull) == 0ull ? 1u << k : 0u; pk |= (unsigned)((lo8 >> (8 * k)) & 3ull) << (2 * k); }
-        SDF_UNROLL for (int k = 0; k < 8; k++) { m |= ((hi8 >> (8 * k)) & 255ull) == 0ull ? 256u << k : 0u; pk |= (unsigned)((hi8 >> (8 * k)) & 3ull) << (2 * k + 16); }
-        ub[r] = (unsigned short)m;
-        reinterpret_cast<unsigned *>(scratch + CULL_SSTATE)[r] = pk;
+        unsigned z = ~(pk[r] | (pk[r] >> 1)) & 0x55555555u;
+        z = (z | (z >> 1)) & 0x33333333u; z = (z | (z >> 2)) & 0x0F0F0F0Fu; z = (z | (z >> 4)) & 0x00FF00FFu; z = (z | (z >> 8)) & 0xFFFFu;
+        ub[r] = (unsigned short)z;
     }
     __syncthreads();
+    SDF_CULL_PROF(16);
     const int nu0 = (lx + 1) >> 1, nu1 = (ly + 1) >> 1, nu2 = (lz + 1) >> 1;
     int nlisted = 0;
     unsigned *colinfo = reinterpret_cast<unsigned *>(scratch + CULL_COLINFO);
diff --git a/sdf_amd/csrc/sdf_hip.hip b/sdf_amd/csrc/sdf_hip.hip
--- a/sdf_amd/csrc/sdf_hip.hip
+++ b/sdf_amd/csrc/sdf_hip.hip
@@ -128,7 +128,7 @@
 }
 
 #define CULL_BLOCK 256
-template <bool FULL, bool RARE, int CB = CULL_BLOCK>
+template <bool FULL, bool RARE, int CB = CULL_BLOCK, int NB = 1>
 __device__ __forceinline__ void cull_body(const uint32_t *__restrict__ code, const double *__restrict__ consts, GridDesc g,
                                                      const int *__restrict__ worklist, const MeshCounters *__restrict__ ctr,
                                                      int tape_stride, int n_instr, int ia_np, int ia_nd, int ia_bytes,
@@ -164,7 +164,7 @@
     const int n_instr_w = tape_stride ? (int)reinterpret_cast<const unsigned long long *>(wcode)[tape_stride - 1] : n_instr;
     long long tstart1 = 0;
     if (prof) asm volatile("s_waitcnt vmcnt(0) lgkmcnt(0)\n\ts_memtime %0\n\ts_waitcnt lgkmcnt(0)" : "=s"(tstart1) : "s"(n_instr_w) : "memory");
-    const int ntl = cull_tasks<CB, FULL, RARE>(wcode, consts, n_instr_w, lx, ly, lz, axes, ia_state, ia_bytes, scratch, wave_sums, ia_np, ia_nd, prof, levels);
+    const int ntl = cull_tasks<CB, FULL, RARE, NB>(wcode, consts, n_instr_w, lx, ly, lz, axes, ia_state, ia_bytes, scratch, wave_sums, ia_np, ia_nd, prof, levels);
     const long long tw = prof ? clock64() : 0;
     if (tid == 0 && ntl < 0) reinterpret_cast<unsigned short *>(scratch)[0] = (unsigned short)0xFFFF;
     __syncthreads();
@@ -190,6 +190,7 @@
         atomicAdd(&prof[29], (unsigned long long)(t_bar - t_ax));
         atomicAdd(&prof[21], (unsigned long long)(clock64() - tw));
         for (int k = 1; k < 10; k++) if (k != 5) atomicAdd(&prof[16 + k], (unsigned long long)pacc[k]);
+        atomicAdd(&prof[50], (unsigned long long)pacc[10]); atomicAdd(&prof[51], (unsigned long long)pacc[11]); atomicAdd(&prof[52], (unsigned long long)pacc[0]);
     }
 }
 
@@ -217,6 +218,23 @@
                                                      int *__restrict__ order, int tail_max, int levels) {
     extern __shared__ __attribute__((aligned(16))) unsigned char cull_smem[];
     cull_body<false, false, 128>(code, consts, g, worklist, ctr, tape_stride, n_instr, ia_np, ia_nd, ia_bytes, out, cull_smem, prof, order, tail_max, levels);
+}
+
+__global__ __launch_bounds__(128) __attribute__((amdgpu_waves_per_eu(3, 4))) void k_cull_lean128x2(const uint32_t *__restrict__ code, const double *__restrict__ consts, GridDesc g,
+                                                     const int *__restrict__ worklist, const MeshCounters *__restrict__ ctr,
+                                                     int tape_stride, int n_instr, int ia_np, int ia_nd, int ia_bytes,
+                                                     unsigned char *__restrict__ out, unsigned long long *prof,
+                                                     int *__restrict__ order, int tail_max, int levels) {
+    extern __shared__ __attribute__((aligned(16))) unsigned char cull_smem[];
+    cull_body<false, false, 128, 2>(code, consts, g, worklist, ctr, tape_stride, n_instr, ia_np, ia_nd, ia_bytes, out, cull_smem, prof, order, tail_max, levels);
+}
+__global__ __launch_bounds__(256) __attribute__((amdgpu_waves_per_eu(3, 4))) void k_cull_lean256x2(const uint32_t *__restrict__ code, const double *__restrict__ consts, GridDesc g,
+                                                     const int *__restrict__ worklist, const MeshCounters *__restrict__ ctr,
+                                                     int tape_stride, int n_instr, int ia_np, int ia_nd, int ia_bytes,
+                                                     unsigned char *__restrict__ out, unsigned long long *prof,
+                                                     int *__restrict__ order, int tail_max, int levels) {
+    extern __shared__ __attribute__((aligned(16))) unsigned char cull_smem[];
+    cull_body<false, false, 256, 2>(code, consts, g, worklist, ctr, tape_stride, n_instr, ia_np, ia_nd, ia_bytes, out, cull_smem, prof, order, tail_max, levels);
 }
 
 
@@ -341,6 +359,7 @@
     if (const char *e = getenv("SDF_CULL")) c->cull = atoi(e);
     if (const char *e = getenv("SDF_DEFER")) c->defer = atoi(e) ? 1 : 0;
     if (const char *e = getenv("SDF_CULL_LEVELS")) c->cull_levels = atoi(e);
+    if (const char *e = getenv("SDF_CULL_BOXES")) c->cull_boxes = atoi(e);
     if (const char *e = getenv("SDF_PARK_SPINS")) c->park_spins = std::max(atoi(e), 1);
     if (const char *e = getenv("SDF_MESH_PROF")) { if (atoi(e) && c->prof.ensure(512 + 4096 * 32)) return 1; }
     return 0;
@@ -395,6 +414,12 @@
     if (!c) return fail("sdf_ctx_set_cull_levels: ctx is NULL");
     if (levels != 0 && levels != 2 && levels != 3) return fail("sdf_ctx_set_cull_levels: 0 (the library's choice), 2 or 3");
     c->cull_levels = levels;
+    return 0;
+}
+int sdf_ctx_set_cull_boxes(sdf_ctx *c, int boxes) {
+    if (!c) return fail("sdf_ctx_set_cull_boxes: ctx is NULL");
+    if (boxes < 0 || boxes > 2) return fail("sdf_ctx_set_cull_boxes: 0 (the library's choice), 1 or 2");
+    c->cull_boxes = boxes;
     return 0;
 }
 
@@ -899,14 +924,21 @@
     if (m->cull.ensure((size_t)nb * CULL_RECORD) || (tail_order && m->order.ensure(MESH_TAIL_MAX * sizeof(int)))) return 1;
     const int ia_np = (int)std::max(t->n_p, 1u), ia_nd = (int)std::max(t->n_d, 1u);
     auto kc = t->full ? (t->ia_rare ? k_cull<true, true> : k_cull<true, false>) : (t->ia_rare ? k_cull<false, true> : k_cull_lean);
-    int cull_block = CULL_BLOCK;
-    if (c->cull_block == 128 && kc == k_cull_lean) { kc = k_cull_lean128; cull_block = 128; }
+    int cull_block = CULL_BLOCK, cull_boxes = 1;
+    const bool lean = kc == k_cull_lean;
+    if (c->cull_block == 128 && lean) { kc = k_cull_lean128; cull_block = 128; }
+    if (lean && c->cull_boxes == 2) {
+        const int cb2 = c->cull_block == 256 ? 256 : 128;
+        if ((size_t)cb2 * 2 * (6 * ia_np + 2 * ia_nd) * 8 <= c->lds_max - 896 - CULL_SCRATCH) {
+            kc = cb2 == 256 ? k_cull_lean256x2 : k_cull_lean128x2; cull_block = cb2; cull_boxes = 2;
+        }
+    }
     if (t->full && !t->ia_rare && c->cull_block != 256) {
         cull_block = c->cull_block == 64 ? 64 : 128;
         kc = cull_block == 64 ? k_cull<true, false, 64> : k_cull<true, false, 128>;
     }
-    const int cull_levels = c->cull_levels ? c->cull_levels : (kc == k_cull_lean || kc == k_cull_lean128 ? 3 : 2);
-    const size_t ia_bytes = std::min<size_t>((size_t)cull_block * (6 * ia_np + 2 * ia_nd) * 8, c->lds_max - 896 - CULL_SCRATCH);
+    const int cull_levels = c->cull_levels ? c->cull_levels : (lean ? 3 : 2);
+    const size_t ia_bytes = std::min<size_t>((size_t)cull_block * cull_boxes * (6 * ia_np + 2 * ia_nd) * 8, c->lds_max - 896 - CULL_SCRATCH);
     const size_t lds = 896 + CULL_SCRATCH + ia_bytes;
     if (lds > 32768) HIPCHK(hipFuncSetAttribute(reinterpret_cast<const void *>(kc), hipFuncAttributeMaxDynamicSharedMemorySize, (int)lds));
     hipLaunchKernelGGL(kc, dim3(nb), dim3(cull_block), lds, st,
@@ -1052,6 +1084,7 @@
     fprintf(stderr, "[k_cull prof] cycles of thread 0, summed over the workgroups: start %llu boxes %llu list %llu groups %llu (%llu passes, %llu groups) tasks %llu record %llu\n",
             pc[16], pc[17], pc[18], pc[19], pc[23], pc[22], pc[20], pc[21]);
     fprintf(stderr, "[k_cull prof] task listing: which tasks %llu, scans %llu; start: range %llu batch %llu origin %llu axes %llu barrier %llu (rest: tape length)\n", pc[24], pc[25], pc[26], pc[27], pc[30], pc[28], pc[29]);
+    fprintf(stderr, "[k_cull prof] of `tasks`: listing the undecided groups %llu, sub-group set-up %llu (the rest: the sub-groups' interval runs); of `which tasks`: packing the states %llu\n", pc[50], pc[51], pc[52]);
     fprintf(stderr, "[k_mesh prof] sampling: intervals %llu task list %llu interpreter %llu sign bits %llu\n", pc[8], pc[9], pc[10], pc[11]);
     fprintf(stderr, "[k_mesh prof] fine: atomic %llu barrier+rank %llu header %llu | rows %llu cells %llu | placing %llu look-back %llu | round end %llu\n",
             pc[42], pc[43], pc[44], pc[45], pc[46], pc[47], pc[48], pc[49]);
diff --git a/sdf_amd/csrc/sdf_internal.h b/sdf_amd/csrc/sdf_internal.h
--- a/sdf_amd/csrc/sdf_internal.h
+++ b/sdf_amd/csrc/sdf_internal.h
@@ -51,6 +51,7 @@
     int tail_order = 1;
     int twopass = -1;
     int defer = 1;
+    int cull_boxes = 0;
     int cull_levels = 0;
     DevBuf bounds_work;
     unsigned bounds_tag = 0, bounds_tag0 = 0;
diff --git a/sdf_amd/csrc/sdf_interval.h b/sdf_amd/csrc/sdf_interval.h
--- a/sdf_amd/csrc/sdf_interval.h
+++ b/sdf_amd/csrc/sdf_interval.h
@@ -206,8 +206,8 @@
 #else
     static int lane_slot() { return 0; }
 #endif
-    SDF_IA double &ps(uint32_t slot, int k) { return base[(slot * 6 + k) * stride + lane_slot()]; }
-    SDF_IA double &ds(uint32_t slot, int k) { return base[(n_p * 6 + slot * 2 + k) * stride + lane_slot()]; }
+    SDF_IA double &ps(uint32_t slot, int k, int off = 0) { return base[(slot * 6 + k) * stride + lane_slot() + off]; }
+    SDF_IA double &ds(uint32_t slot, int k, int off = 0) { return base[(n_p * 6 + slot * 2 + k) * stride + lane_slot() + off]; }
 };
 __host__ __device__ inline size_t prune_lds_bytes(int n_p, int n_d) { return (size_t)(6 * n_p + 2 * n_d) * PRUNE_BLOCK * 8; }
 
@@ -237,36 +237,52 @@
     return add(len3(maxc(qx, 0.0), maxc(qy, 0.0), maxc(qz, 0.0)), minc(mx, 0.0));
 }
 
-SDF_IA Ival ia_leaf(uint32_t op, const double *c, const Ival &x, const Ival &y, const Ival &z) {
+#define SDF_IA_BOXES _Pragma("unroll") for (int b = 0; b < NB; b++)
+
+template <int NB>
+SDF_IA void ia_leaf_nb(uint32_t op, const double *c, const Ival (&x)[NB], const Ival (&y)[NB], const Ival (&z)[NB], Ival (&r)[NB]) {
     using namespace ia;
     switch (op) {
-    case OP_L_SPHERE: return subc(len3(subc(x, c[1]), subc(y, c[2]), subc(z, c[3])), c[0]);
-    case OP_L_PLANE: return dot3c(csub(c[3], x), csub(c[4], y), csub(c[5], z), c[0], c[1], c[2]);
+    case OP_L_SPHERE: SDF_IA_BOXES r[b] = subc(len3(subc(x[b], c[1]), subc(y[b], c[2]), subc(z[b], c[3])), c[0]); break;
+    case OP_L_PLANE: SDF_IA_BOXES r[b] = dot3c(csub(c[3], x[b]), csub(c[4], y[b]), csub(c[5], z[b]), c[0], c[1], c[2]); break;
     case OP_L_BOX:
-        return ia_box_like(subc(abs_(subc(x, c[0])), c[3]), subc(abs_(subc(y, c[1])), c[4]), subc(abs_(subc(z, c[2])), c[5]));
+        SDF_IA_BOXES r[b] = ia_box_like(subc(abs_(subc(x[b], c[0])), c[3]), subc(abs_(subc(y[b], c[1])), c[4]), subc(abs_(subc(z[b], c[2])), c[5]));
+        break;
     case OP_L_ROUNDED_BOX:
-        return subc(ia_box_like(addc(subc(abs_(x), c[0]), c[3]), addc(subc(abs_(y), c[1]), c[3]), addc(subc(abs_(z), c[2]), c[3])), c[3]);
-    case OP_L_TORUS: return subc(len2(subc(len2(x, y), c[0]), z), c[1]);
-    case OP_L_CYLINDER: return subc(len2(x, y), c[0]);
-    case OP_L_ROUNDED_CYLINDER: {
-        const Ival d0 = addc(subc(len2(x, y), c[0]), c[1]), d1 = addc(subc(abs_(z), c[2]), c[1]);
-        return subc(add(minc(max_(d0, d1), 0.0), len2(maxc(d0, 0.0), maxc(d1, 0.0))), c[1]);
-    }
-    case OP_L_CAPSULE: {
-        const Ival pax = subc(x, c[0]), pay = subc(y, c[1]), paz = subc(z, c[2]);
-        const Ival h = clip01(divc(dot3c(pax, pay, paz, c[3], c[4], c[5]), c[6]));
-        return subc(len3(sub(pax, mulc(h, c[3])), sub(pay, mulc(h, c[4])), sub(paz, mulc(h, c[5]))), c[7]);
-    }
-    case OP_L_OCTAHEDRON: return mulc(subc(add(add(abs_(x), abs_(y)), abs_(z)), c[0]), c[1]);
-    case OP_L_CIRCLE: return subc(len2(subc(x, c[1]), subc(y, c[2])), c[0]);
-    case OP_L_LINE: return dot2c(csub(c[2], x), csub(c[3], y), c[0], c[1]);
-    case OP_L_RECTANGLE: {
-        const Ival qx = subc(abs_(subc(x, c[0])), c[2]), qy = subc(abs_(subc(y, c[1])), c[3]);
-        return add(len2(maxc(qx, 0.0), maxc(qy, 0.0)), minc(max_(qx, qy), 0.0));
-    }
-    default: return top();
-
-    }
+        SDF_IA_BOXES r[b] = subc(ia_box_like(addc(subc(abs_(x[b]), c[0]), c[3]), addc(subc(abs_(y[b]), c[1]), c[3]), addc(subc(abs_(z[b]), c[2]), c[3])), c[3]);
+        break;
+    case OP_L_TORUS: SDF_IA_BOXES r[b] = subc(len2(subc(len2(x[b], y[b]), c[0]), z[b]), c[1]); break;
+    case OP_L_CYLINDER: SDF_IA_BOXES r[b] = subc(len2(x[b], y[b]), c[0]); break;
+    case OP_L_ROUNDED_CYLINDER:
+        SDF_IA_BOXES {
+            const Ival d0 = addc(subc(len2(x[b], y[b]), c[0]), c[1]), d1 = addc(subc(abs_(z[b]), c[2]), c[1]);
+            r[b] = subc(add(minc(max_(d0, d1), 0.0), len2(maxc(d0, 0.0), maxc(d1, 0.0))), c[1]);
+        }
+        break;
+    case OP_L_CAPSULE:
+        SDF_IA_BOXES {
+            const Ival pax = subc(x[b], c[0]), pay = subc(y[b], c[1]), paz = subc(z[b], c[2]);
+            const Ival h = clip01(divc(dot3c(pax, pay, paz, c[3], c[4], c[5]), c[6]));
+            r[b] = subc(len3(sub(pax, mulc(h, c[3])), sub(pay, mulc(h, c[4])), sub(paz, mulc(h, c[5]))), c[7]);
+        }
+        break;
+    case OP_L_OCTAHEDRON: SDF_IA_BOXES r[b] = mulc(subc(add(add(abs_(x[b]), abs_(y[b])), abs_(z[b])), c[0]), c[1]); break;
+    case OP_L_CIRCLE: SDF_IA_BOXES r[b] = subc(len2(subc(x[b], c[1]), subc(y[b], c[2])), c[0]); break;
+    case OP_L_LINE: SDF_IA_BOXES r[b] = dot2c(csub(c[2], x[b]), csub(c[3], y[b]), c[0], c[1]); break;
+    case OP_L_RECTANGLE:
+        SDF_IA_BOXES {
+            const Ival qx = subc(abs_(subc(x[b], c[0])), c[2]), qy = subc(abs_(subc(y[b], c[1])), c[3]);
+            r[b] = add(len2(maxc(qx, 0.0), maxc(qy, 0.0)), minc(max_(qx, qy), 0.0));
+        }
+        break;
+    default: SDF_IA_BOXES r[b] = top(); break;
+    }
+}
+SDF_IA Ival ia_leaf(uint32_t op, const double *c, const Ival &x, const Ival &y, const Ival &z) {
+    const Ival x1[1] = {x}, y1[1] = {y}, z1[1] = {z};
+    Ival r[1];
+    ia_leaf_nb<1>(op, c, x1, y1, z1, r);
+    return r[0];
 }
 
 SDF_IA bool ia_is_rare_leaf(uint32_t op) {
@@ -508,16 +524,8 @@
     }
 }
 
-SDF_IA Ival ia_post(uint32_t post, const Ival &d1, const Ival &d2, double K) {
+SDF_IA Ival ia_post_smooth(uint32_t post, const Ival &d1, const Ival &d2, double K) {
     using namespace ia;
-    switch (post) {
-    case POST_SET: return d2;
-    case POST_UNION: return min_(d1, d2);
-    case POST_DIFF: return max_(d1, neg(d2));
-    case POST_INTER: return max_(d1, d2);
-    case POST_BLEND: return add(mulc(d2, K), mulc(d1, 1.0 - K));
-    default: break;
-    }
     if (!(K > 0.0) || bad(d1) || bad(d2)) return top();
     const Ival e = post == POST_SDIFF ? neg(d2) : d2;
     const Ival ad = abs_(sub(e, d1));
@@ -527,6 +535,30 @@
     if (post == POST_SUNION) { r.lo -= cmax; r.hi -= cmin; } else { r.lo += cmin; r.hi += cmax; }
     const double m = 1e-9 * (fabs(r.lo) + fabs(r.hi) + K);
     return fix(Ival{r.lo - m, r.hi + m});
+}
+
+SDF_IA Ival ia_post(uint32_t post, const Ival &d1, const Ival &d2, double K) {
+    using namespace ia;
+    switch (post) {
+    case POST_SET: return d2;
+    case POST_UNION: return min_(d1, d2);
+    case POST_DIFF: return max_(d1, neg(d2));
+    case POST_INTER: return max_(d1, d2);
+    case POST_BLEND: return add(mulc(d2, K), mulc(d1, 1.0 - K));
+    default: return ia_post_smooth(post, d1, d2, K);
+    }
+}
+template <int NB>
+SDF_IA void ia_post_nb(uint32_t post, const Ival (&d1)[NB], const Ival (&d2)[NB], double K, Ival (&r)[NB]) {
+    using namespace ia;
+    switch (post) {
+    case POST_SET: SDF_IA_BOXES r[b] = d2[b]; break;
+    case POST_UNION: SDF_IA_BOXES r[b] = min_(d1[b], d2[b]); break;
+    case POST_DIFF: SDF_IA_BOXES r[b] = max_(d1[b], neg(d2[b])); break;
+    case POST_INTER: SDF_IA_BOXES r[b] = max_(d1[b], d2[b]); break;
+    case POST_BLEND: SDF_IA_BOXES r[b] = add(mulc(d2[b], K), mulc(d1[b], 1.0 - K)); break;
+    default: SDF_IA_BOXES r[b] = ia_post_smooth(post, d1[b], d2[b], K); break;
+    }
 }
 
 SDF_IA int ia_decide(uint32_t post, const Ival &left, const Ival &right, double K) {
@@ -569,27 +601,35 @@
     for (int k = 0; k < 8; k++) if ((i >> 5) == k) m[k] |= 1u << (i & 31);
 }
 
-template <bool DECIDE, bool FULL, bool RARE>
-SDF_IA Ival ia_run_tape(const uint32_t *__restrict__ code, const double *__restrict__ consts,
-                        const uint16_t *__restrict__ rstart, const uint16_t *__restrict__ lstart, int n_instr,
-                        Ival x, Ival y, Ival z, bool live, IaShared sh, int n_d, uint32_t *masks) {
+template <bool DECIDE, bool FULL, bool RARE, int NB>
+SDF_IA void ia_run_tape_nb(const uint32_t *__restrict__ code, const double *__restrict__ consts,
+                           const uint16_t *__restrict__ rstart, const uint16_t *__restrict__ lstart, int n_instr,
+                           Ival (&x)[NB], Ival (&y)[NB], Ival (&z)[NB], bool live, IaShared sh, int box_stride, int n_d, uint32_t *masks,
+                           Ival (&acc)[NB]) {
     using namespace ia;
+    static_assert(!DECIDE || NB == 1, "the lanes of a batch agree on ONE box each");
 #if defined(__HIP_DEVICE_COMPILE__)
     const int lane = threadIdx.x & 63, gbase = lane & ~7;
 #endif
-    Ival acc = pt(0.0);
+    SDF_IA_BOXES acc[b] = pt(0.0);
     for (int i = 0; i < sh.n_p; i++)
-        for (int k = 0; k < 6; k++) sh.ps(i, k) = 0.0;
-    for (int i = 0; i < n_d; i++) { sh.ds(i, 0) = 0.0; sh.ds(i, 1) = 0.0; }
+        for (int k = 0; k < 6; k++) { SDF_IA_BOXES sh.ps(i, k, b * box_stride) = 0.0; }
+    for (int i = 0; i < n_d; i++) { SDF_IA_BOXES { sh.ds(i, 0, b * box_stride) = 0.0; sh.ds(i, 1, b * box_stride) = 0.0; } }
     uint32_t keep[8] = {0, 0, 0, 0, 0, 0, 0, 0};
     auto psave = [&](uint32_t k) {
-        sh.ps(k, 0) = x.lo; sh.ps(k, 1) = x.hi; sh.ps(k, 2) = y.lo; sh.ps(k, 3) = y.hi; sh.ps(k, 4) = z.lo; sh.ps(k, 5) = z.hi;
+        SDF_IA_BOXES {
+            const int o = b * box_stride;
+            sh.ps(k, 0, o) = x[b].lo; sh.ps(k, 1, o) = x[b].hi; sh.ps(k, 2, o) = y[b].lo; sh.ps(k, 3, o) = y[b].hi; sh.ps(k, 4, o) = z[b].lo; sh.ps(k, 5, o) = z[b].hi;
+        }
     };
     auto pload = [&](uint32_t k) {
-        x = Ival{sh.ps(k, 0), sh.ps(k, 1)}; y = Ival{sh.ps(k, 2), sh.ps(k, 3)}; z = Ival{sh.ps(k, 4), sh.ps(k, 5)};
+        SDF_IA_BOXES {
+            const int o = b * box_stride;
+            x[b] = Ival{sh.ps(k, 0, o), sh.ps(k, 1, o)}; y[b] = Ival{sh.ps(k, 2, o), sh.ps(k, 3, o)}; z[b] = Ival{sh.ps(k, 4, o), sh.ps(k, 5, o)};
+        }
     };
-    auto dsave = [&](uint32_t k, const Ival &v) { sh.ds(k, 0) = v.lo; sh.ds(k, 1) = v.hi; };
-    auto dload = [&](uint32_t k) { return Ival{sh.ds(k, 0), sh.ds(k, 1)}; };
+    auto dsave = [&](uint32_t k, int b, const Ival &v) { sh.ds(k, 0, b * box_stride) = v.lo; sh.ds(k, 1, b * box_stride) = v.hi; };
+    auto dload = [&](uint32_t k, int b) { return Ival{sh.ds(k, 0, b * box_stride), sh.ds(k, 1, b * box_stride)}; };
     for (int ip = 0; ip < n_instr; ip++) {
         const uint32_t w0 = code[2 * ip], w1 = code[2 * ip + 1];
         const uint32_t op = w0 & 255u, post = (w0 >> 8) & 7u, sa = (w0 >> 24) & 7u;
@@ -597,20 +637,20 @@
         if (op == OP_END) break;
         if (w0 & 0x000800u) pload((w0 >> 12) & 7u);
         if (w0 & 0x008000u) psave((w0 >> 16) & 7u);
-        if (w0 & 0x080000u) dsave((w0 >> 20) & 7u, acc);
+        if (w0 & 0x080000u) { SDF_IA_BOXES dsave((w0 >> 20) & 7u, b, acc[b]); }
         const bool is_leaf = op >= OP_L_SPHERE && op < OP_COMB;
         if (is_leaf || op == OP_COMB) {
-            const Ival left = is_leaf ? acc : dload(sa);
-            Ival right = acc;
+            Ival left[NB], right[NB];
+            SDF_IA_BOXES { left[b] = is_leaf ? acc[b] : dload(sa, b); right[b] = acc[b]; }
             if (is_leaf) {
-                if (RARE && ia_is_rare_leaf(op)) right = ia_leaf_rare(op, c, x, y, z);
-                else right = ia_leaf(op, c, x, y, z);
+                if (RARE && ia_is_rare_leaf(op)) { SDF_IA_BOXES right[b] = ia_leaf_rare(op, c, x[b], y[b], z[b]); }
+                else ia_leaf_nb<NB>(op, c, x, y, z, right);
             }
             int rs = 0xFFFF, ls = 0xFFFF;
             if constexpr (DECIDE) { rs = rstart[ip]; ls = lstart[ip]; }
 #if defined(__HIP_DEVICE_COMPILE__)
             if (DECIDE && rs != 0xFFFF && ls != 0xFFFF && rs <= ip && ls <= rs) {
-                const int d = live ? ia_decide(post, left, right, c[-1]) : 3;
+                const int d = live ? ia_decide(post, left[0], right[0], c[-1]) : 3;
                 const unsigned long long b1 = __ballot(d == 1 || d == 3), b2 = __ballot(d == 2 || d == 3);
                 if (((b1 >> gbase) & 0xFFull) == 0xFFull) {
                     if (post < POST_SUNION) mask_set_range(masks, rs, ip);
@@ -624,111 +664,153 @@
                 }
             }
 #endif
-            acc = ia_post(post, left, right, c[-1]);
+            ia_post_nb<NB>(post, left, right, c[-1], acc);
             continue;
         }
         switch (op) {
-        case OP_TRANSLATE: x = subc(x, c[0]); y = subc(y, c[1]); z = subc(z, c[2]); break;
-        case OP_SCALE: x = divc(x, c[0]); y = divc(y, c[1]); z = divc(z, c[2]); break;
-        case OP_ROTATE: {
-            const Ival nx = dot3c(x, y, z, c[0], c[3], c[6]);
-            const Ival ny = dot3c(x, y, z, c[1], c[4], c[7]);
-            const Ival nz = dot3c(x, y, z, c[2], c[5], c[8]);
-            x = nx; y = ny; z = nz; break; }
-        case OP_ELONGATE: {
-            const Ival qx = subc(abs_(x), c[0]), qy = subc(abs_(y), c[1]), qz = subc(abs_(z), c[2]);
-            dsave(sa, minc(max_(qx, max_(qy, qz)), 0.0));
-            x = maxc(qx, 0.0); y = maxc(qy, 0.0); z = maxc(qz, 0.0); break; }
-        case OP_TRANSLATE2: x = subc(x, c[0]); y = subc(y, c[1]); break;
-        case OP_SCALE2: x = divc(x, c[0]); y = divc(y, c[1]); break;
-        case OP_ROTATE2: {
-            const Ival nx = dot2c(x, y, c[0], c[2]), ny = dot2c(x, y, c[1], c[3]);
-            x = nx; y = ny; break; }
-        case OP_ELONGATE2: {
-            const Ival qx = subc(abs_(x), c[0]), qy = subc(abs_(y), c[1]);
-            dsave(sa, minc(max_(qx, qy), 0.0));
-            x = maxc(qx, 0.0); y = maxc(qy, 0.0); break; }
-        case OP_REVOLVE: { const Ival nx = subc(len2(x, y), c[0]); y = z; x = nx; z = pt(0.0); break; }
-        case OP_SETZ0: z = pt(0.0); break;
+        case OP_TRANSLATE: SDF_IA_BOXES { x[b] = subc(x[b], c[0]); y[b] = subc(y[b], c[1]); z[b] = subc(z[b], c[2]); } break;
+        case OP_SCALE: SDF_IA_BOXES { x[b] = divc(x[b], c[0]); y[b] = divc(y[b], c[1]); z[b] = divc(z[b], c[2]); } break;
+        case OP_ROTATE:
+            SDF_IA_BOXES {
+                const Ival nx = dot3c(x[b], y[b], z[b], c[0], c[3], c[6]);
+                const Ival ny = dot3c(x[b], y[b], z[b], c[1], c[4], c[7]);
+                const Ival nz = dot3c(x[b], y[b], z[b], c[2], c[5], c[8]);
+                x[b] = nx; y[b] = ny; z[b] = nz;
+            }
+            break;
+        case OP_ELONGATE:
+            SDF_IA_BOXES {
+                const Ival qx = subc(abs_(x[b]), c[0]), qy = subc(abs_(y[b]), c[1]), qz = subc(abs_(z[b]), c[2]);
+                dsave(sa, b, minc(max_(qx, max_(qy, qz)), 0.0));
+                x[b] = maxc(qx, 0.0); y[b] = maxc(qy, 0.0); z[b] = maxc(qz, 0.0);
+            }
+            break;
+        case OP_TRANSLATE2: SDF_IA_BOXES { x[b] = subc(x[b], c[0]); y[b] = subc(y[b], c[1]); } break;
+        case OP_SCALE2: SDF_IA_BOXES { x[b] = divc(x[b], c[0]); y[b] = divc(y[b], c[1]); } break;
+        case OP_ROTATE2:
+            SDF_IA_BOXES {
+                const Ival nx = dot2c(x[b], y[b], c[0], c[2]), ny = dot2c(x[b], y[b], c[1], c[3]);
+                x[b] = nx; y[b] = ny;
+            }
+            break;
+        case OP_ELONGATE2:
+            SDF_IA_BOXES {
+                const Ival qx = subc(abs_(x[b]), c[0]), qy = subc(abs_(y[b]), c[1]);
+                dsave(sa, b, minc(max_(qx, qy), 0.0));
+                x[b] = maxc(qx, 0.0); y[b] = maxc(qy, 0.0);
+            }
+            break;
+        case OP_REVOLVE: SDF_IA_BOXES { const Ival nx = subc(len2(x[b], y[b]), c[0]); y[b] = z[b]; x[b] = nx; z[b] = pt(0.0); } break;
+        case OP_SETZ0: SDF_IA_BOXES z[b] = pt(0.0); break;
         case OP_SAVE_P: psave(sa); if constexpr (DECIDE) ia_keep_bit(keep, ip); break;
         case OP_LOAD_P: pload(sa); if constexpr (DECIDE) ia_keep_bit(keep, ip); break;
-        case OP_PUSH_D: dsave(sa, acc); break;
+        case OP_PUSH_D: SDF_IA_BOXES dsave(sa, b, acc[b]); break;
         case OP_NOP: break;
-        case OP_NEG: acc = neg(acc); break;
-        case OP_ADDC: acc = addc(acc, c[0]); break;
-        case OP_SUBC: acc = subc(acc, c[0]); break;
-        case OP_MULC: acc = mulc(acc, c[0]); break;
-        case OP_SHELL: acc = subc(abs_(acc), c[0]); break;
-        case OP_ADD_DS: acc = add(acc, dload(sa)); break;
-        case OP_EXT_PRE: dsave(sa, subc(abs_(z), c[0])); break;
-        case OP_EXT_POST: {
-            const Ival w = dload(sa);
-            acc = add(minc(max_(acc, w), 0.0), len2(maxc(acc, 0.0), maxc(w, 0.0))); break; }
-        case OP_BEND_LINEAR: {
-            const Ival tt = ease01((int)c[10], clip01(divc(dot3c(subc(x, c[0]), subc(y, c[1]), subc(z, c[2]), c[3], c[4], c[5]), c[6])));
-            x = add(x, mulc(tt, c[7])); y = add(y, mulc(tt, c[8])); z = add(z, mulc(tt, c[9])); break; }
+        case OP_NEG: SDF_IA_BOXES acc[b] = neg(acc[b]); break;
+        case OP_ADDC: SDF_IA_BOXES acc[b] = addc(acc[b], c[0]); break;
+        case OP_SUBC: SDF_IA_BOXES acc[b] = subc(acc[b], c[0]); break;
+        case OP_MULC: SDF_IA_BOXES acc[b] = mulc(acc[b], c[0]); break;
+        case OP_SHELL: SDF_IA_BOXES acc[b] = subc(abs_(acc[b]), c[0]); break;
+        case OP_ADD_DS: SDF_IA_BOXES acc[b] = add(acc[b], dload(sa, b)); break;
+        case OP_EXT_PRE: SDF_IA_BOXES dsave(sa, b, subc(abs_(z[b]), c[0])); break;
+        case OP_EXT_POST:
+            SDF_IA_BOXES {
+                const Ival w = dload(sa, b);
+                acc[b] = add(minc(max_(acc[b], w), 0.0), len2(maxc(acc[b], 0.0), maxc(w, 0.0)));
+            }
+            break;
+        case OP_BEND_LINEAR:
+            SDF_IA_BOXES {
+                const Ival tt = ease01((int)c[10], clip01(divc(dot3c(subc(x[b], c[0]), subc(y[b], c[1]), subc(z[b], c[2]), c[3], c[4], c[5]), c[6])));
+                x[b] = add(x[b], mulc(tt, c[7])); y[b] = add(y[b], mulc(tt, c[8])); z[b] = add(z[b], mulc(tt, c[9]));
+            }
+            break;
         case OP_REP_PREP: {
             const int dim = (int)c[0];
-            Ival idx[3] = {pt(0.0), pt(0.0), pt(0.0)};
-            const Ival pp[3] = {x, y, z};
-            for (int i = 0; i < 3; i++) {
-                if (i >= dim) continue;
-                const double s = c[1 + i];
-                Ival r = s != 0.0 ? rint_(divc(pp[i], s)) : pt(0.0);
-                if (c[4] != 0.0) r = clipc(r, -c[5 + i], c[5 + i]);
-                idx[i] = r;
-            }
-            sh.ps(sa, 0) = idx[0].lo; sh.ps(sa, 1) = idx[0].hi; sh.ps(sa, 2) = idx[1].lo; sh.ps(sa, 3) = idx[1].hi;
-            sh.ps(sa, 4) = idx[2].lo; sh.ps(sa, 5) = idx[2].hi; break; }
+            SDF_IA_BOXES {
+                Ival idx[3] = {pt(0.0), pt(0.0), pt(0.0)};
+                const Ival pp[3] = {x[b], y[b], z[b]};
+                for (int i = 0; i < 3; i++) {
+                    if (i >= dim) continue;
+                    const double s = c[1 + i];
+                    Ival r = s != 0.0 ? rint_(divc(pp[i], s)) : pt(0.0);
+                    if (c[4] != 0.0) r = clipc(r, -c[5 + i], c[5 + i]);
+                    idx[i] = r;
+                }
+                const int o = b * box_stride;
+                sh.ps(sa, 0, o) = idx[0].lo; sh.ps(sa, 1, o) = idx[0].hi; sh.ps(sa, 2, o) = idx[1].lo; sh.ps(sa, 3, o) = idx[1].hi;
+                sh.ps(sa, 4, o) = idx[2].lo; sh.ps(sa, 5, o) = idx[2].hi;
+            }
+            break; }
         case OP_REP_SET: {
             const uint32_t sb = (w1 >> 24) & 7u;
-            const Ival ax{sh.ps(sa, 0), sh.ps(sa, 1)}, ay{sh.ps(sa, 2), sh.ps(sa, 3)}, az{sh.ps(sa, 4), sh.ps(sa, 5)};
-            const Ival bx{sh.ps(sb, 0), sh.ps(sb, 1)}, by{sh.ps(sb, 2), sh.ps(sb, 3)}, bz{sh.ps(sb, 4), sh.ps(sb, 5)};
-            x = sub(ax, mulc(addc(bx, c[3]), c[0]));
-            y = sub(ay, mulc(addc(by, c[4]), c[1]));
-            z = sub(az, mulc(addc(bz, c[5]), c[2])); break; }
+            SDF_IA_BOXES {
+                const int o = b * box_stride;
+                const Ival ax{sh.ps(sa, 0, o), sh.ps(sa, 1, o)}, ay{sh.ps(sa, 2, o), sh.ps(sa, 3, o)}, az{sh.ps(sa, 4, o), sh.ps(sa, 5, o)};
+                const Ival bx{sh.ps(sb, 0, o), sh.ps(sb, 1, o)}, by{sh.ps(sb, 2, o), sh.ps(sb, 3, o)}, bz{sh.ps(sb, 4, o), sh.ps(sb, 5, o)};
+                x[b] = sub(ax, mulc(addc(bx, c[3]), c[0]));
+                y[b] = sub(ay, mulc(addc(by, c[4]), c[1]));
+                z[b] = sub(az, mulc(addc(bz, c[5]), c[2]));
+            }
+            break; }
         case OP_TRANS_LIN_PRE:
-            dsave(sa, ease01((int)c[7], clip01(divc(dot3c(subc(x, c[0]), subc(y, c[1]), subc(z, c[2]), c[3], c[4], c[5]), c[6])))); break;
+            SDF_IA_BOXES dsave(sa, b, ease01((int)c[7], clip01(divc(dot3c(subc(x[b], c[0]), subc(y[b], c[1]), subc(z[b], c[2]), c[3], c[4], c[5]), c[6]))));
+            break;
         case OP_TRANS_MIX: {
             const uint32_t sb = (w1 >> 24) & 7u;
-            const Ival tt = dload(sa), dd = dload(sb);
-            acc = add(mul(tt, acc), mul(csub(1.0, tt), dd)); break; }
+            SDF_IA_BOXES {
+                const Ival tt = dload(sa, b), dd = dload(sb, b);
+                acc[b] = add(mul(tt, acc[b]), mul(csub(1.0, tt), dd));
+            }
+            break; }
         case OP_EXTTO_PRE:
-            dsave(sa, ease01((int)c[1], addc(clipc(divc(z, c[0]), -0.5, 0.5), 0.5))); break;
+            SDF_IA_BOXES dsave(sa, b, ease01((int)c[1], addc(clipc(divc(z[b], c[0]), -0.5, 0.5), 0.5)));
+            break;
         case OP_EXTTO_MIX: {
             const uint32_t sb = (w1 >> 24) & 7u;
-            const Ival dd1 = dload(sb), tt = dload(sa);
-            acc = add(dd1, mul(sub(acc, dd1), tt)); break; }
-        case OP_SLICE_POST: {
-            const Ival A = dload(sa), B = neg(acc);
-            if (bad(A) || bad(B)) acc = top();
-            else if (A.hi <= 0.0) acc = B;
-            else if (A.lo > 0.0) acc = A;
-            else acc = Ival{fmin(A.lo, B.lo), fmax(A.hi, B.hi)};
+            SDF_IA_BOXES {
+                const Ival dd1 = dload(sb, b), tt = dload(sa, b);
+                acc[b] = add(dd1, mul(sub(acc[b], dd1), tt));
+            }
             break; }
+        case OP_SLICE_POST:
+            SDF_IA_BOXES {
+                const Ival A = dload(sa, b), B = neg(acc[b]);
+                if (bad(A) || bad(B)) acc[b] = top();
+                else if (A.hi <= 0.0) acc[b] = B;
+                else if (A.lo > 0.0) acc[b] = A;
+                else acc[b] = Ival{fmin(A.lo, B.lo), fmax(A.hi, B.hi)};
+            }
+            break;
         case OP_TWIST: case OP_BEND: case OP_BEND_RADIAL: case OP_TRANS_RAD_PRE: case OP_WRAP_AROUND:
             if constexpr (FULL) {
                 if (op == OP_WRAP_AROUND) {
                     const double pi = 3.141592653589793;
-                    Ival r = finite_(x) && finite_(y) ? pad(len2(x, y), 1e-12, 1e-300) : top();
-                    if (!bad(r)) r.lo = fmax(r.lo, 0.0);
-                    const Ival d = subc(r, c[9]);
-                    const Ival u = divc(addc(atan2_range(x, y), pi), 2.0 * pi);
-                    const Ival tt = bad(u) ? top() : ease01((int)c[10], Ival{fmax(u.lo, 0.0), fmin(u.hi, 1.0)});
-                    const Ival nx = add(addc(mulc(tt, c[3]), c[0]), mulc(d, c[6])), ny = add(addc(mulc(tt, c[4]), c[1]), mulc(d, c[7]));
-                    x = nx; y = ny;
+                    SDF_IA_BOXES {
+                        Ival r = finite_(x[b]) && finite_(y[b]) ? pad(len2(x[b], y[b]), 1e-12, 1e-300) : top();
+                        if (!bad(r)) r.lo = fmax(r.lo, 0.0);
+                        const Ival d = subc(r, c[9]);
+                        const Ival u = divc(addc(atan2_range(x[b], y[b]), pi), 2.0 * pi);
+                        const Ival tt = bad(u) ? top() : ease01((int)c[10], Ival{fmax(u.lo, 0.0), fmin(u.hi, 1.0)});
+                        const Ival nx = add(addc(mulc(tt, c[3]), c[0]), mulc(d, c[6])), ny = add(addc(mulc(tt, c[4]), c[1]), mulc(d, c[7]));
+                        x[b] = nx; y[b] = ny;
+                    }
                 } else
                 if (op == OP_TWIST || op == OP_BEND) {
-                    Ival sn, cs;
-                    sincos_range(mulc(op == OP_TWIST ? z : x, c[0]), sn, cs);
-                    const Ival nx = sub(mul(cs, x), mul(sn, y)), ny = add(mul(sn, x), mul(cs, y));
-                    x = nx; y = ny;
+                    SDF_IA_BOXES {
+                        Ival sn, cs;
+                        sincos_range(mulc(op == OP_TWIST ? z[b] : x[b], c[0]), sn, cs);
+                        const Ival nx = sub(mul(cs, x[b]), mul(sn, y[b])), ny = add(mul(sn, x[b]), mul(cs, y[b]));
+                        x[b] = nx; y[b] = ny;
+                    }
                 } else {
-                    Ival r = finite_(x) && finite_(y) ? pad(len2(x, y), 1e-12, 1e-300) : top();
-                    if (!bad(r)) r.lo = fmax(r.lo, 0.0);
-                    const Ival tt = clip01(divc(subc(r, c[0]), c[1]));
-                    if (op == OP_BEND_RADIAL) z = sub(z, mulc(ease01((int)c[3], tt), c[2]));
-                    else dsave(sa, ease01((int)c[2], tt));
+                    SDF_IA_BOXES {
+                        Ival r = finite_(x[b]) && finite_(y[b]) ? pad(len2(x[b], y[b]), 1e-12, 1e-300) : top();
+                        if (!bad(r)) r.lo = fmax(r.lo, 0.0);
+                        const Ival tt = clip01(divc(subc(r, c[0]), c[1]));
+                        if (op == OP_BEND_RADIAL) z[b] = sub(z[b], mulc(ease01((int)c[3], tt), c[2]));
+                        else dsave(sa, b, ease01((int)c[2], tt));
+                    }
                 }
                 break;
             }
@@ -736,28 +818,41 @@
         case OP_CIRC_PREP: case OP_CIRC_SET:
             if constexpr (FULL) {
                 if (op == OP_CIRC_PREP) {
-                    Ival d, a;
-                    circ_prep(x, y, c[0], d, a);
-                    sh.ps(sa, 0) = d.lo; sh.ps(sa, 1) = d.hi; sh.ps(sa, 2) = a.lo; sh.ps(sa, 3) = a.hi;
-                    sh.ps(sa, 4) = z.lo; sh.ps(sa, 5) = z.hi;
+                    SDF_IA_BOXES {
+                        Ival d, a;
+                        circ_prep(x[b], y[b], c[0], d, a);
+                        const int o = b * box_stride;
+                        sh.ps(sa, 0, o) = d.lo; sh.ps(sa, 1, o) = d.hi; sh.ps(sa, 2, o) = a.lo; sh.ps(sa, 3, o) = a.hi;
+                        sh.ps(sa, 4, o) = z[b].lo; sh.ps(sa, 5, o) = z[b].hi;
+                    }
                 } else {
-                    const Ival d{sh.ps(sa, 0), sh.ps(sa, 1)}, a{sh.ps(sa, 2), sh.ps(sa, 3)};
-                    circ_set(d, a, c[0], x, y);
-                    z = Ival{sh.ps(sa, 4), sh.ps(sa, 5)};
+                    SDF_IA_BOXES {
+                        const int o = b * box_stride;
+                        const Ival d{sh.ps(sa, 0, o), sh.ps(sa, 1, o)}, a{sh.ps(sa, 2, o), sh.ps(sa, 3, o)};
+                        circ_set(d, a, c[0], x[b], y[b]);
+                        z[b] = Ival{sh.ps(sa, 4, o), sh.ps(sa, 5, o)};
+                    }
                 }
                 break;
             }
             [[fallthrough]];
         default:
-            x = y = z = top(); acc = top();
-            for (int k = 0; k < n_d; k++) dsave(k, top());
+            SDF_IA_BOXES { x[b] = y[b] = z[b] = top(); acc[b] = top(); }
+            for (int k = 0; k < n_d; k++) { SDF_IA_BOXES dsave(k, b, top()); }
             if (op == OP_REP_PREP || op == OP_CIRC_PREP) psave(sa);
             break;
         }
     }
     if constexpr (DECIDE)
         for (int k = 0; k < 8; k++) masks[k] &= ~keep[k];
-    return acc;
+}
+template <bool DECIDE, bool FULL, bool RARE>
+SDF_IA Ival ia_run_tape(const uint32_t *__restrict__ code, const double *__restrict__ consts,
+                        const uint16_t *__restrict__ rstart, const uint16_t *__restrict__ lstart, int n_instr,
+                        Ival x, Ival y, Ival z, bool live, IaShared sh, int n_d, uint32_t *masks) {
+    Ival x1[1] = {x}, y1[1] = {y}, z1[1] = {z}, acc[1];
+    ia_run_tape_nb<DECIDE, FULL, RARE, 1>(code, consts, rstart, lstart, n_instr, x1, y1, z1, live, sh, 0, n_d, masks, acc);
+    return acc[0];
 }
 
 __device__ __forceinline__ int compact_tape(const unsigned long long *__restrict__ code64, int n_instr, const uint32_t *masks,
diff --git a/sdf_amd/engine.py b/sdf_amd/engine.py
--- a/sdf_amd/engine.py
+++ b/sdf_amd/engine.py
@@ -71,6 +71,7 @@
     'sdf_ctx_set_tail_order': (ctypes.c_int, [_vp, ctypes.c_int]),
     'sdf_ctx_set_defer': (ctypes.c_int, [_vp, ctypes.c_int]),
     'sdf_ctx_set_cull_levels': (ctypes.c_int, [_vp, ctypes.c_int]),
+    'sdf_ctx_set_cull_boxes': (ctypes.c_int, [_vp, ctypes.c_int]),
     'sdf_ctx_synchronize': (ctypes.c_int, [_vp]),
     'sdf_ctx_trim': (ctypes.c_int, [_vp]),
     'sdf_tape_create': (ctypes.c_int, [_vp, _u32p, ctypes.c_uint32, _f64p, ctypes.c_uint32,
@@ -153,7 +154,7 @@
     'sdf_mesh_prune_masks': (ctypes.c_int, [_vp, _u32p]),
     'sdf_mesh_destroy': (ctypes.c_int, [_vp]),
 }
-ABI_VERSION = 15
+ABI_VERSION = 16
 
 
 def build_info():
@@ -559,6 +560,9 @@
 
     def set_cull_levels(self, levels):
         _check(self.lib, self.lib.sdf_ctx_set_cull_levels(self.ctx, int(levels)))
+
+    def set_cull_boxes(self, boxes):
+        _check(self.lib, self.lib.sdf_ctx_set_cull_boxes(self.ctx, int(boxes)))
 
     def set_twopass(self, mode):
         _check(self.lib, self.lib.sdf_ctx_set_twopass(self.ctx, int(mode)))
```

Result: slower. 615.6 billion voxels/s (-1.5%).
